# pkorus/neural-imaging

Measured on AMD Instinct MI355X. Metric: patches/s (fwd+bwd) ISP->JPEG->FAN @256^2, higher is better.
Workload: dtype bf16; 1 GPU; c4 = train_manipulation UNet->[native,sharpen:1,resample:50,gaussian:0.83,jpeg:80]->dJPEG(QF80,soft)->FAN, ds none, trainable nip+fan, lambda_nip 0.1; raw_patch=128, batch_per_gpu=64, global_batch=64, parallelism=dp1, world_size=1, hip_graph=False

## Files before the change

include/nimg.h:

```cpp
#ifndef NIMG_H
#define NIMG_H

#include <stddef.h>
#include <stdint.h>

#ifdef __cplusplus
extern "C" {
#endif

#define NIMG_OK 0
#define NIMG_ERR_ARG (-1)
#define NIMG_ERR_LAUNCH (-2)
#define NIMG_ERR_WORKSPACE (-3)

#define NIMG_BF16_IN 1
#define NIMG_BF16_OUT 2
#define NIMG_BF16_MASK 4
#define NIMG_BF16_DZ 8
#define NIMG_D2S_OUT 16
#define NIMG_MASK_CONV 128
#define NIMG_COPY_LRELU 64
#define NIMG_S2D_OUT 32
#define NIMG_UNPOOL_OUT 512
#define NIMG_D2S_CONVT 1024
#define NIMG_POOL_ALSO 256

#define NIMG_ABI_VERSION 7
int nimg_abi_version(void);

#define NIMG_ROUND_ROUND 0
#define NIMG_ROUND_SOFT 1
#define NIMG_ROUND_SIN 2
#define NIMG_ROUND_HARMONIC 3
#define NIMG_ROUND_IDENTITY 4

int nimg_djpeg_fwd(const float* x, float* y, const float* qtab, uint8_t* mask, int16_t* idx, float* xdq,
                   int n, int h, int w, int rounding, void* stream);
int nimg_djpeg_bwd(const float* x, const float* gy, const uint8_t* mask, const float* qtab, float* gx,
                   int n, int h, int w, int rounding, void* stream);
size_t nimg_djpeg_dq_workspace_bytes(int n, int h, int w);
int nimg_djpeg_bwd_dq(const float* x, const float* gy, const uint8_t* mask, const float* qtab, float* gx, float* dq,
                      int n, int h, int w, int rounding, int accumulate, void* workspace, size_t workspace_bytes,
                      void* stream);
int nimg_jpeg_qtable(int quality, int channel, float* out64);

int nimg_conv2d_fwd(const float* in1, int c1, const float* in2, int c2, const float* w, const float* bias,
                    float* out1, int o1, float* out2, int o2, const float* act_mask, int n, int h, int wd, int ks,
                    int stride, int pad_t, int pad_l, int pad_mode, int hout, int wout, int act, float alpha,
                    void* stream);
int nimg_conv_flip_weights(const float* w, float* wt, int ks_h, int ks_w, int cin, int cout, void* stream);
size_t nimg_conv2d_wgrad_workspace_bytes(int cin, int cout, int ks_h, int ks_w, int n, int hout, int wout);
int nimg_conv2d_wgrad(const float* in1, int c1, const float* in2, int c2, const float* dz, int cout, float* dw,
                      float* db, int n, int h, int wd, int ks, int stride, int pad_t, int pad_l, int pad_mode, int hout,
                      int wout, int accumulate, void* workspace, size_t workspace_bytes, void* stream);
size_t nimg_bias_grad_workspace_bytes(long npix, int cout);
int nimg_bias_grad(const float* dz, float* db, long npix, int cout, int accumulate, void* workspace,
                   size_t workspace_bytes, void* stream);
int nimg_bias_grad_ex(const float* dz, float* db, long npix, int cout, int accumulate, void* workspace,
                      size_t workspace_bytes, int flags, void* stream);
int nimg_convt2x2_fwd(const float* x, const float* w, const float* bias, float* y, int n, int h, int wd, int cin,
                      int cout, void* stream);

int nimg_maxpool2_fwd(const float* x, float* y, int n, int h, int w, int c, void* stream);
int nimg_maxpool2_bwd(const float* dp, const float* yact, const float* add, float* dz, int n, int h, int w, int c,
                      int apply_lrelu_mask, float alpha, void* stream);
int nimg_maxpool2_fwd_bf16(const void* x, void* y, int n, int h, int w, int c, void* stream);
int nimg_maxpool2_bwd_bf16(const void* dp, const void* yact, const void* add, void* dz, int n, int h, int w, int c,
                           int apply_lrelu_mask, float alpha, void* stream);
int nimg_conv2d_pool_fwd(const float* in, int cin, const float* w, const float* bias, float* pool_out,
                         unsigned char* pool_idx, int cout, int n, int h, int wd, int ks, int act, float alpha,
                         void* stream);
int nimg_conv2d_pool_fwd_bf16(const float* in, int cin, const float* w, const void* wb, const float* bias,
                              float* pool_out, unsigned char* pool_idx, int cout, int n, int h, int wd, int ks, int act,
                              float alpha, void* stream);
int nimg_maxpool2_unpool(const float* dp, const unsigned char* idx, const float* pooled, float* dz, int n, int ho, int wo,
                         int c, int apply_lrelu_mask, float alpha, void* stream);
int nimg_d2s_clip_fwd(const float* x, float* y, int n, int h, int w, int cout, float scale, float shift, int clip,
                      void* stream);
int nimg_d2s_clip_bwd(const float* dy, float* dx, int n, int h, int w, int cout, float scale, void* stream);
int nimg_lrelu_bwd(const float* dy, const float* yact, float* dz, long count, float alpha, void* stream);
int nimg_add(const float* a, const float* b, float* out, long count, void* stream);
int nimg_add_n(const float* const* inputs, int n_inputs, float* out, long count, void* stream);
int nimg_avgpool_fwd(const float* x, float* y, int n, int h, int w, int c, int factor, void* stream);
int nimg_avgpool_bwd(const float* dy, float* dx, int n, int h, int w, int c, int factor, void* stream);

size_t nimg_mse255_workspace_bytes(void);
int nimg_mse255(const float* a, const float* b, float* loss, float* grad_a, long count, float grad_scale,
                int accumulate, void* workspace, size_t workspace_bytes, void* stream);
size_t nimg_mae255_workspace_bytes(void);
int nimg_mae255(const float* a, const float* b, float* loss, float* grad_a, long count, float grad_scale,
                int accumulate, void* workspace, size_t workspace_bytes, void* stream);
size_t nimg_ssim_loss_workspace_bytes(int n, int h, int w, int c, int with_grad);
int nimg_ssim_loss(const float* y, const float* t, float* loss, float* grad_y, int n, int h, int w, int c,
                   float max_val, const float* gauss_win, float grad_scale, int accumulate, void* workspace,
                   size_t workspace_bytes, void* stream);
int nimg_mse255_sum_s2d3(const float* const* parts, int n_parts, const float* y, const float* target, float* loss, float* dz,
                         int n, int h, int w, float grad_scale, void* workspace, size_t workspace_bytes, void* stream);
size_t nimg_ssim_workspace_bytes(int n);
int nimg_ssim(const float* a, const float* b, float* out, int n, int h, int w, int c, int mode, float max_val,
              const float* gauss_win, void* workspace, size_t workspace_bytes, void* stream);
int nimg_fan_head_fwd(const float* act, const float* w, const float* b, const int* labels, float* gap, float* probs,
                      float* loss_per, float* dlogits, int n, int hw, int c, int k, float loss_scale, void* stream);
int nimg_fan_head_bwd(const float* act, const float* gap, const float* w, const float* dlogits,
                      const float* loss_per, float* dact, float* dw, float* db, float* loss, int n, int hw, int c,
                      int k, float loss_scale, float alpha, void* stream);
int nimg_adam_step(float* params, const float* grads, float* m, float* v, long count, float lr, float beta1,
                   float beta2, float eps, int step, float grad_scale, const int* skip_flag, void* stream);
int nimg_adam_step_dev(float* params, const float* grads, float* m, float* v, long count, const float* lr_t, float beta1,
                       float beta2, float eps, float grad_scale, const int* skip_flag, void* stream);
int nimg_nan_flag(const float* g, long count, int* flag, void* stream);
int nimg_int_words(int* dst, const int* src, long n, int value, int mode, void* stream);
int nimg_float_fill(float* dst, long n, float value, void* stream);

#define NIMG_TICKET_BYTES (64 * 1024)
#define NIMG_TICKET_STREAMS 16
int nimg_bind_tickets(void* stream, void* buf, size_t bytes);

int nimg_stream_create_cu_mask(int n_cus, void** stream);
int nimg_stream_destroy(void* stream);

int nimg_head_fused_ok(int hw, int c);
int nimg_head_fwd(const void* x, const void* wimg, const float* bias, unsigned* mask, unsigned* mask_p, float* gap, int n, int hw,
                  int c, float alpha, void* stream);
size_t nimg_head_wgrad_workspace_bytes(int n, int c);
int nimg_head_wgrad(const void* x, const unsigned* mask_p, const float* dlogits, const float* wdense, int k, float* dw, float* db,
                    int n, int hw, int c, float alpha, int accumulate, void* workspace, size_t workspace_bytes, void* stream);
int nimg_head_dgrad(const unsigned* mask, const float* dlogits, const float* wdense, int k, const void* wimg_t,
                    const void* in_mask, void* dx, int n, int hw, int c, float alpha, void* stream);
int nimg_head_dact(const unsigned* mask, const float* dlogits, const float* wdense, int k, void* dact, int n, int hw, int c,
                   float alpha, void* stream);
int nimg_fan_dense_fwd(const float* gap, const float* w, const float* b, const int* labels, float* probs, float* loss_per,
                       float* dlogits, int n, int c, int k, float loss_scale, void* stream);
int nimg_fan_dense_bwd(const float* gap, const float* dlogits, const float* loss_per, float* dw, float* db, float* loss, int n,
                       int c, int k, float loss_scale, void* stream);

int nimg_constrained_kernel_fwd(const float* kernel, float* nf, int ks, int channels, float strength, void* stream);
int nimg_constrained_kernel_bwd(const float* kernel, const float* dnf, float* dkernel, int ks, int channels,
                                float strength, void* stream);
int nimg_fold_pad(const float* dpad, float* dx, int n, int h, int w, int c, int pad, int pad_mode, void* stream);

int nimg_gaussian_fwd(const float* x, float* y, uint8_t* mask, const float* gk25, int n, int h, int w, int clip,
                      void* stream);
int nimg_gaussian_bwd(const float* dy, const uint8_t* mask, float* dx, const float* gk25, int n, int h, int w,
                      void* stream);
int nimg_dwfilter_fwd(const float* x, float* y, uint8_t* mask, const float* taps, int k, int pad_mode, int n, int h, int w,
                      int clip, void* stream);
int nimg_dwfilter_bwd(const float* dy, const uint8_t* mask, float* dx, const float* taps, int k, int pad_mode, int n, int h,
                      int w, void* stream);
int nimg_sharpen_fwd(const float* x, float* y, float* aux_hsv, uint8_t* mask, const float* gk9, int n, int h, int w,
                     void* stream);
int nimg_sharpen_bwd(const float* x, const float* dy, float* aux_hsv, const uint8_t* mask, float* dx,
                     const float* gk9, int n, int h, int w, void* stream);
int nimg_sparse_axis_apply(const float* in, float* out, const int* rowptr, const int* col, const float* val, int n,
                           int hin, int win, int c, int axis, int out_size, void* stream);

size_t nimg_ssim_planes_workspace_bytes(int n, int c);
int nimg_ssim_planes(const float* y, const float* t, int n, int h, int w, int c, float max_val, const float* gauss_win,
                     float* mean_ssim, float* mean_cs, float* maps, int which_maps, void* workspace,
                     size_t workspace_bytes, void* stream);
int nimg_msssim_combine(const float* values, const float* items, int scales, int planes, float* loss, float* coef,
                        void* stream);
int nimg_ssim_maps_grad(const float* y, const float* t, const float* maps, const float* coef, float* grad_y, int n,
                        int h, int w, int c, const float* gauss_win, float grad_scale, int accumulate, void* stream);

int nimg_patch_stats(const uint8_t* rgb, int n_images, int h, int w, const int* image_idx, const int* cand_xy, int b,
                     int attempts, int patch, double* var_out, double* mean_out, void* stream);
int nimg_patch_select(const int* cand_xy, const float* uniforms, const double* var, const double* mean, int b,
                      int attempts, int max_attempts, int mode, int* chosen_xy, int* attempts_used, void* stream);
int nimg_patch_gather(const uint16_t* raw, const uint8_t* rgb, int n_images, int h, int w, const int* image_idx,
                      const int* xy, int b, int patch, float* x_out, float* y_out, void* stream);

int nimg_affine(const float* x, float* y, long count, float a, float b, void* stream);
int nimg_lrelu_fwd(const float* x, float* y, long count, float alpha, void* stream);
int nimg_tanh_fwd(const float* x, float* y, long count, void* stream);
int nimg_tanh_bwd(const float* dy, const float* y, float* dx, long count, void* stream);
int nimg_clip01(const float* x, float* y, long count, void* stream);
int nimg_pad2d(const float* x, float* y, int n, int h, int w, int c, int pad, int pad_mode, void* stream);
int nimg_isp_residual_fwd(const float* x, const float* f, const float* alpha, float* y, long count, int clip,
                          void* stream);
long nimg_isp_residual_workspace_bytes(void);
int nimg_isp_residual_bwd(const float* dy, const float* f, const float* alpha, float* df, float* dalpha,
                          float* workspace, long count, int accumulate, void* stream);
int nimg_mask_scale(const float* x, const uint8_t* keep, float* y, long count, float scale, void* stream);
size_t nimg_conv5_dgrad_sparse_image_bytes(int cin, int cout);
int nimg_conv5_dgrad_sparse_weights(const float* w, void* image, int cin, int cout, void* stream);
int nimg_conv5_dgrad_sparse(const void* g, const unsigned char* idx, int cout, const void* image, void* out, int cin,
                            const void* act_mask, int n, int h, int wd, float alpha, int flags, void* stream);
int nimg_conv2d_fwd_bf16_res(const float* in1, int c1, const void* wb, const float* bias, float* out1, int o1,
                             const float* act_mask, const float* residual, void* out_bf16_copy, int n, int h, int wd, int ks,
                             int stride, int pad_t, int pad_l, int pad_mode, int hout, int wout, int act, float alpha, int flags,
                             void* stream);
int nimg_conv2d_fwd_bf16_unpool(const void* in_pooled, const unsigned char* in_idx, int c1, const void* wb, const float* bias,
                                float* out1, int o1, const float* act_mask, int n, int h, int w_, int ks, int pad_t, int pad_l,
// ... 12 lines not shown
size_t nimg_reduce_entry_bytes(void);
int nimg_reduce_batch_max(void);
int nimg_reduce_slabs_batch(const void* entries, int n, void* stream);

int nimg_conv5c3_bf16(const float* in, const float* w, float* out, int n, int h, int wd, void* stream);
int nimg_cconv3(const float* in, const float* w, float* out_f32, void* out_c4, int n, int h, int w_, int pad_mode,
                void* stream);
int nimg_cconv3_dgrad_border(const float* dc, const float* nf, float* dx, int n, int h, int w_, void* stream);
int nimg_conv1_pool_fwd_c4(const void* c4, const float* w, const float* bias, void* pooled, unsigned char* pool_idx, int n,
                           int h, int w_, float alpha, int out_bf16, void* stream);
size_t nimg_conv1_wgrad_c4_workspace_bytes(void);
int nimg_conv1_wgrad_c4(const void* c4, const void* g, const unsigned char* pool_idx, float* dw, float* db, int n, int h, int w_,
                        int g_bf16, int accumulate, void* workspace, size_t workspace_bytes, void* stream);
int nimg_conv1_dgrad_pooled(const void* g, const unsigned char* pool_idx, const float* w, float* dc, int n, int h, int w_,
                            int g_bf16, void* stream);
int nimg_confusion_accumulate(const float* probs, const int* labels, int* pred, unsigned long long* conf, int n, int k,
                              void* stream);
int nimg_sigmoid_fwd(const float* x, float* y, long count, void* stream);
int nimg_sigmoid_bwd(const float* dy, const float* y, float* dx, long count, void* stream);
int nimg_activation_fwd(const float* x, float* y, long count, int kind, float alpha, void* stream);
int nimg_activation_bwd(const float* dy, const float* y, float* dx, long count, int kind, float alpha, void* stream);
int nimg_gamma_ste_fwd(const float* x, float* y, long count, float lo, float hi, float exponent, void* stream);
int nimg_gamma_ste_bwd(const float* x, const float* dy, float* dx, long count, float lo, float hi, float exponent,
                       void* stream);
int nimg_s2d2_affine_bf16(const float* x, void* y, int n, int h, int w, int c, int cp, float a, float b, void* stream);
int nimg_s2d_conv_weights(const float* w5, float* w3, int cin, int cp, int cout, void* stream);
int nimg_s2d_conv_weights_bwd(const float* dw3, float* dw5, int cin, int cp, int cout, int accumulate, void* stream);
int nimg_d2s2_scale(const float* xs, float* x, int n, int h, int w, int c, int cp, float scale, void* stream);
int nimg_zero_insert2(const float* in, float* out, int n, int h, int w, int c, void* stream);
size_t nimg_latent_workspace_bytes(int codebook_size);
int nimg_latent_fwd(const float* z, const float* scale, const float* codebook, int codebook_size, float v,
                    float gamma, int soft_codebook, float* latent, float* entropy, long count, long count_global,
                    void* workspace, size_t workspace_bytes, int finalize, void* stream);
int nimg_latent_entropy_finalize(int codebook_size, long count_global, float* entropy, void* workspace, void* stream);
int nimg_latent_bwd(const float* z, const float* scale, const float* latent, const float* dlatent,
                    float entropy_coef, const float* codebook, int codebook_size, float v, float gamma,
                    int soft_codebook, float* dz, float* dscale, int accumulate_dscale, long count, void* workspace,
                    size_t workspace_bytes, void* stream);
size_t nimg_l2_loss_workspace_bytes(void);
int nimg_l2_loss(const float* target, const float* y, float* loss, float* grad_y, long count, float grad_scale,
                 int accumulate, void* workspace, size_t workspace_bytes, void* stream);

size_t nimg_conv_weights_bf16_bytes(int ks_h, int ks_w, int cin, int cout, int mode);
int nimg_conv_weights_bf16(const float* w, void* wb, int ks_h, int ks_w, int cin, int cout, int mode, void* stream);
int nimg_conv2d_wgrad_pooled_bf16(const float* in, int cin, const float* g, const unsigned char* idx, int cout,
                                  float* dw, float* db, int n, int h, int wd, int ks, int accumulate, void* workspace,
                                  size_t workspace_bytes, void* stream);
int nimg_conv2d_dgrad_fewin_pooled_bf16(const float* g, const unsigned char* idx, const float* w, float* out, int ci,
                                        int cz, int n, int h, int wd, int ks, void* stream);
int nimg_conv2d_fwd_bf16_ex(const float* in1, int c1, const float* in2, int c2, const void* wb, const float* bias,
                            float* out1, int o1, float* out2, int o2, const float* act_mask, int n, int h, int wd,
                            int ks, int stride, int pad_t, int pad_l, int pad_mode, int hout, int wout, int act,
                            float alpha, int flags, void* stream);
int nimg_conv2d_wgrad_bf16_ex(const float* in1, int c1, const float* in2, int c2, const float* dz, int cout, float* dw,
                              float* db, int n, int h, int wd, int ks, int stride, int pad_t, int pad_l, int pad_mode,
                              int hout, int wout, int accumulate, void* workspace, size_t workspace_bytes, int flags,
                              void* stream);
int nimg_conv2d_pool_fwd_bf16_ex(const float* in, int cin, const float* w, const void* wb, const float* bias,
                                 float* pool_out, unsigned char* pool_idx, int cout, int n, int h, int wd, int ks,
                                 int act, float alpha, int flags, void* stream);
int nimg_conv2d_fwd_pool_also_bf16(const float* in, int cin, const void* wb, const float* bias, float* out, float* pool_out,
                                   unsigned char* pool_idx, int cout, int n, int h, int wd, int act, float alpha, void* stream);
#define NIMG_ROWS_F32_OUT 1
int nimg_conv3_rows_bf16(const void* in1, int c1, const void* in2, int c2, const void* wb, const float* bias, const void* mask,
                         void* out, void* out2, void* pool_out, int n, int h, int wd, int cout, int act, float alpha, int flags,
                         void* stream);
int nimg_conv3_rows_d2s_bf16(const void* in, int c1, const void* wb, const float* bias, float* y, int n, int h, int wd, void* stream);
int nimg_conv3_rows_c4_bf16(const float* in, const float* w, const float* bias, void* out, int n, int h, int wd, int act, float alpha,
                            void* stream);

int nimg_conv2d_dgrad_unpool_out_bf16(const float* dz, int c1, const void* wb, const float* act, const float* skip, float* out,
                                      int cout, int n, int h, int wd, int apply_mask, float alpha, void* stream);
int nimg_conv2d_wgrad_pooled_bf16_ex(const float* in, int cin, const float* g, const unsigned char* idx, int cout,
                                     float* dw, float* db, int n, int h, int wd, int ks, int accumulate, void* workspace,
                                     size_t workspace_bytes, int flags, void* stream);
int nimg_conv2d_dgrad_fewin_pooled_bf16_ex(const float* g, const unsigned char* idx, const float* w, float* out, int ci,
                                           int cz, int n, int h, int wd, int ks, int flags, void* stream);
int nimg_maxpool2_unpool_ex(const float* dp, const unsigned char* idx, const float* pooled, float* dz, int n, int ho,
                            int wo, int c, int apply_lrelu_mask, float alpha, int flags, void* stream);
int nimg_convt2x2_fwd_bf16(const float* x, const void* wb, const float* bias, float* y, int n, int h, int wd, int cin,
                           int cout, void* stream);
int nimg_convt2x2_fwd_bf16_ex(const float* x, const void* wb, const float* bias, float* y, int n, int h, int wd, int cin,
                              int cout, int flags, void* stream);
int nimg_conv_weights_bf16_batch(const void* table, int n_entries, void* stream);
int nimg_conv2d_fwd_bf16(const float* in1, int c1, const float* in2, int c2, const void* wb, const float* bias,
                         float* out1, int o1, float* out2, int o2, const float* act_mask, int n, int h, int wd,
                         int ks, int stride, int pad_t, int pad_l, int pad_mode, int hout, int wout, int act,
                         float alpha, void* stream);
size_t nimg_conv2d_wgrad_bf16_workspace_bytes(int cin, int cout, int ks_h, int ks_w, int n, int hout, int wout);
int nimg_conv2d_wgrad_bf16(const float* in1, int c1, const float* in2, int c2, const float* dz, int cout, float* dw,
                           float* db, int n, int h, int wd, int ks, int stride, int pad_t, int pad_l, int pad_mode,
                           int hout, int wout, int accumulate, void* workspace, size_t workspace_bytes, void* stream);

int nimg_conv2d_fwd_smallc_bf16(const float* in, int cin, const float* w, const float* bias, float* out, int cout,
                                int n, int h, int wd, int ks, int pad_mode, int act, float alpha, void* stream);
int nimg_conv2d_fwd_smallc_bf16_ex(const float* in, int cin, const float* w, const float* bias, float* out, int cout,
                                   int n, int h, int wd, int ks, int pad_mode, int act, float alpha, int flags, void* stream);
int nimg_conv2d_dgrad_fewin_bf16(const float* dz, const float* w, float* out, int ci, int cz, int n, int h, int wd,
                                 int ks, void* stream);

int nimg_awgn_fwd(const float* x, const float* noise, float* y, uint8_t* mask, long count, float strength,
                  void* stream);
int nimg_awgn_bwd(const float* x, const float* noise, const float* dy, const uint8_t* mask, float* dx, long count,
                  float strength, void* stream);
int nimg_gamma_fwd(const float* x, float* y, long count, float gamma, void* stream);
int nimg_gamma_bwd(const float* x, const float* dy, float* dx, long count, float gamma, void* stream);
int nimg_median_fwd(const float* x, float* y, uint8_t* sel, int n, int h, int w, int kernel, void* stream);
int nimg_median_bwd(const float* dy, const uint8_t* sel, float* dx, int n, int h, int w, int kernel, void* stream);

#define NIMG_L3IC_E_READ 1
#define NIMG_L3IC_E_LANES 2
#define NIMG_L3IC_E_RANGE 4
#define NIMG_L3IC_E_SYMBOL 8
#define NIMG_L3IC_E_FREQ 16
#define NIMG_L3IC_E_VARINT 32
#define NIMG_L3IC_E_ODD 64
#define NIMG_L3IC_E_UNUSED 128
#define NIMG_L3IC_E_STATE 256
#define NIMG_L3IC_E_RLE 512
size_t nimg_l3ic_workspace_bytes(int n_streams, int n_sym);
int nimg_l3ic_quantise(const float* z, const float* codebook, int codebook_size, uint8_t* idx, int* err, int n, int h,
                       int w, int c, void* stream);
int nimg_l3ic_encode(const uint8_t* idx, int n_streams, int n_sym, uint8_t* out, uint32_t* lengths, uint32_t* hist,
                     uint32_t* freq, void* workspace, size_t workspace_bytes, void* stream);
int nimg_l3ic_decode(const uint8_t* data, const uint32_t* offsets, const uint32_t* lengths, const float* codebook,
                     int codebook_size, float* z, uint32_t* err, int n, int h, int w, int c, void* stream);

size_t nimg_jpeg_workspace_bytes(int n, int h, int w, int hs, int vs);
int nimg_jpeg_transform(const void* x, int is_u8, int n, int h, int w, int hs, int vs, int quality, int16_t* coef, void* workspace,
                        size_t workspace_bytes, void* stream);
int nimg_jpeg_encode(const int16_t* coef, int n, int h, int w, int hs, int vs, uint8_t* out, size_t out_capacity, uint32_t* lengths,
                     void* workspace, size_t workspace_bytes, void* stream);
int nimg_jpeg_reconstruct(const int16_t* coef, int n, int h, int w, int hs, int vs, int quality, float* y, void* workspace,
                          size_t workspace_bytes, void* stream);

#ifdef __cplusplus
}
#endif
#endif
```

neural-imaging_amd/_lib.py:

```python
import ctypes
import os
from ctypes import c_float, c_int, c_long, c_size_t, c_void_p

_HERE = os.path.dirname(os.path.abspath(__file__))
LIB_PATH = os.environ.get('NIMG_LIBPATH') or os.path.join(_HERE, 'libnimg.so')

P = c_void_p

PROTOTYPES = {
    'nimg_abi_version': (c_int, []),
    'nimg_djpeg_fwd': (c_int, [P, P, P, P, P, P, c_int, c_int, c_int, c_int, P]),
    'nimg_djpeg_bwd': (c_int, [P, P, P, P, P, c_int, c_int, c_int, c_int, P]),
    'nimg_djpeg_dq_workspace_bytes': (c_size_t, [c_int, c_int, c_int]),
    'nimg_djpeg_bwd_dq': (c_int, [P, P, P, P, P, P, c_int, c_int, c_int, c_int, c_int, P, c_size_t, P]),
    'nimg_jpeg_qtable': (c_int, [c_int, c_int, P]),
    'nimg_conv2d_fwd': (c_int, [P, c_int, P, c_int, P, P, P, c_int, P, c_int, P, c_int, c_int, c_int, c_int, c_int,
                                c_int, c_int, c_int, c_int, c_int, c_int, c_float, P]),
    'nimg_conv_flip_weights': (c_int, [P, P, c_int, c_int, c_int, c_int, P]),
    'nimg_conv2d_wgrad_workspace_bytes': (c_size_t, [c_int, c_int, c_int, c_int, c_int, c_int, c_int]),
    'nimg_conv2d_wgrad': (c_int, [P, c_int, P, c_int, P, c_int, P, P, c_int, c_int, c_int, c_int, c_int, c_int, c_int,
                                  c_int, c_int, c_int, c_int, P, c_size_t, P]),
    'nimg_bias_grad_workspace_bytes': (c_size_t, [c_long, c_int]),
    'nimg_bias_grad': (c_int, [P, P, c_long, c_int, c_int, P, c_size_t, P]),
    'nimg_bias_grad_ex': (c_int, [P, P, c_long, c_int, c_int, P, c_size_t, c_int, P]),
    'nimg_convt2x2_fwd': (c_int, [P, P, P, P, c_int, c_int, c_int, c_int, c_int, P]),
    'nimg_maxpool2_fwd': (c_int, [P, P, c_int, c_int, c_int, c_int, P]),
    'nimg_maxpool2_bwd': (c_int, [P, P, P, P, c_int, c_int, c_int, c_int, c_int, c_float, P]),
    'nimg_maxpool2_fwd_bf16': (c_int, [P, P, c_int, c_int, c_int, c_int, P]),
    'nimg_maxpool2_bwd_bf16': (c_int, [P, P, P, P, c_int, c_int, c_int, c_int, c_int, c_float, P]),
    'nimg_conv2d_pool_fwd': (c_int, [P, c_int, P, P, P, P, c_int, c_int, c_int, c_int, c_int, c_int, c_float, P]),
    'nimg_conv2d_pool_fwd_bf16': (c_int, [P, c_int, P, P, P, P, P, c_int, c_int, c_int, c_int, c_int, c_int, c_float,
                                          P]),
    'nimg_maxpool2_unpool': (c_int, [P, P, P, P, c_int, c_int, c_int, c_int, c_int, c_float, P]),
    'nimg_d2s_clip_fwd': (c_int, [P, P, c_int, c_int, c_int, c_int, c_float, c_float, c_int, P]),
    'nimg_d2s_clip_bwd': (c_int, [P, P, c_int, c_int, c_int, c_int, c_float, P]),
    'nimg_lrelu_bwd': (c_int, [P, P, P, c_long, c_float, P]),
    'nimg_add': (c_int, [P, P, P, c_long, P]),
    'nimg_add_n': (c_int, [P, c_int, P, c_long, P]),
    'nimg_avgpool_fwd': (c_int, [P, P, c_int, c_int, c_int, c_int, c_int, P]),
    'nimg_avgpool_bwd': (c_int, [P, P, c_int, c_int, c_int, c_int, c_int, P]),
    'nimg_mse255_workspace_bytes': (c_size_t, []),
    'nimg_mse255': (c_int, [P, P, P, P, c_long, c_float, c_int, P, c_size_t, P]),
    'nimg_mse255_sum_s2d3': (c_int, [P, c_int, P, P, P, P, c_int, c_int, c_int, c_float, P, c_size_t, P]),
    'nimg_fan_head_fwd': (c_int, [P, P, P, P, P, P, P, P, c_int, c_int, c_int, c_int, c_float, P]),
    'nimg_fan_head_bwd': (c_int, [P, P, P, P, P, P, P, P, P, c_int, c_int, c_int, c_int, c_float, c_float, P]),
    'nimg_adam_step': (c_int, [P, P, P, P, c_long, c_float, c_float, c_float, c_float, c_int, c_float, P, P]),
    'nimg_adam_step_dev': (c_int, [P, P, P, P, c_long, P, c_float, c_float, c_float, c_float, P, P]),
    'nimg_conv3_rows_bf16': (c_int, [P, c_int, P, c_int, P, P, P, P, P, P, c_int, c_int, c_int, c_int, c_int, c_float, c_int, P]),
    'nimg_conv3_rows_d2s_bf16': (c_int, [P, c_int, P, P, P, c_int, c_int, c_int, P]),
    'nimg_conv2d_wgrad_bf16_deferred': (c_int, [P, c_int, P, c_int, P, P, c_int, P, P, c_int, c_int, c_int, c_int, c_int, c_int, c_int,
                                                c_int, c_int, c_int, P, c_size_t, c_int, P, P]),
    'nimg_conv2d_wgrad_bf16_chained': (c_int, [P, c_int, P, c_int, P, P, c_int, P, P, c_int, c_int, c_int, c_int, c_int, c_int, c_int,
                                               c_int, c_int, c_int, P, c_size_t, c_int, P, P, P]),
    'nimg_reduce_entry_bytes': (c_size_t, []),
    'nimg_reduce_batch_max': (c_int, []),
    'nimg_reduce_slabs_batch': (c_int, [P, c_int, P]),
    'nimg_conv3_rows_c4_bf16': (c_int, [P, P, P, P, c_int, c_int, c_int, c_int, c_float, P]),
    'nimg_nan_flag': (c_int, [P, c_long, P, P]),
    'nimg_int_words': (c_int, [P, P, c_long, c_int, c_int, P]),
    'nimg_float_fill': (c_int, [P, c_long, c_float, P]),
    'nimg_bind_tickets': (c_int, [P, P, c_size_t]),
    'nimg_stream_create_cu_mask': (c_int, [c_int, P]),
    'nimg_stream_destroy': (c_int, [P]),
    'nimg_head_fused_ok': (c_int, [c_int, c_int]),
    'nimg_head_fwd': (c_int, [P, P, P, P, P, P, c_int, c_int, c_int, c_float, P]),
    'nimg_head_wgrad_workspace_bytes': (c_size_t, [c_int, c_int]),
    'nimg_head_wgrad': (c_int, [P, P, P, P, c_int, P, P, c_int, c_int, c_int, c_float, c_int, P, c_size_t, P]),
    'nimg_head_dgrad': (c_int, [P, P, P, c_int, P, P, P, c_int, c_int, c_int, c_float, P]),
    'nimg_head_dact': (c_int, [P, P, P, c_int, P, c_int, c_int, c_int, c_float, P]),
    'nimg_fan_dense_fwd': (c_int, [P, P, P, P, P, P, P, c_int, c_int, c_int, c_float, P]),
    'nimg_fan_dense_bwd': (c_int, [P, P, P, P, P, P, c_int, c_int, c_int, c_float, P]),
    'nimg_constrained_kernel_fwd': (c_int, [P, P, c_int, c_int, c_float, P]),
    'nimg_constrained_kernel_bwd': (c_int, [P, P, P, c_int, c_int, c_float, P]),
    'nimg_fold_pad': (c_int, [P, P, c_int, c_int, c_int, c_int, c_int, c_int, P]),
    'nimg_gaussian_fwd': (c_int, [P, P, P, P, c_int, c_int, c_int, c_int, P]),
    'nimg_gaussian_bwd': (c_int, [P, P, P, P, c_int, c_int, c_int, P]),
    'nimg_dwfilter_fwd': (c_int, [P, P, P, P, c_int, c_int, c_int, c_int, c_int, c_int, P]),
    'nimg_dwfilter_bwd': (c_int, [P, P, P, P, c_int, c_int, c_int, c_int, c_int, P]),
    'nimg_sharpen_fwd': (c_int, [P, P, P, P, P, c_int, c_int, c_int, P]),
    'nimg_sharpen_bwd': (c_int, [P, P, P, P, P, P, c_int, c_int, c_int, P]),
    'nimg_affine': (c_int, [P, P, c_long, c_float, c_float, P]),
    'nimg_lrelu_fwd': (c_int, [P, P, c_long, c_float, P]),
    'nimg_zero_insert2': (c_int, [P, P, c_int, c_int, c_int, c_int, P]),
    'nimg_s2d2_affine_bf16': (c_int, [P, P, c_int, c_int, c_int, c_int, c_int, c_float, c_float, P]),
    'nimg_s2d_conv_weights': (c_int, [P, P, c_int, c_int, c_int, P]),
    'nimg_s2d_conv_weights_bwd': (c_int, [P, P, c_int, c_int, c_int, c_int, P]),
    'nimg_d2s2_scale': (c_int, [P, P, c_int, c_int, c_int, c_int, c_int, c_float, P]),
    'nimg_latent_workspace_bytes': (c_size_t, [c_int]),
    'nimg_latent_fwd': (c_int, [P, P, P, c_int, c_float, c_float, c_int, P, P, c_long, c_long, P, c_size_t, c_int, P]),
    'nimg_latent_entropy_finalize': (c_int, [c_int, c_long, P, P, P]),
    'nimg_latent_bwd': (c_int, [P, P, P, P, c_float, P, c_int, c_float, c_float, c_int, P, P, c_int, c_long, P,
                                c_size_t, P]),
    'nimg_l2_loss_workspace_bytes': (c_size_t, []),
    'nimg_l2_loss': (c_int, [P, P, P, P, c_long, c_float, c_int, P, c_size_t, P]),
    'nimg_conv_weights_bf16_bytes': (c_size_t, [c_int, c_int, c_int, c_int, c_int]),
    'nimg_conv_weights_bf16': (c_int, [P, P, c_int, c_int, c_int, c_int, c_int, P]),
    'nimg_conv2d_fwd_bf16': (c_int, [P, c_int, P, c_int, P, P, P, c_int, P, c_int, P, c_int, c_int, c_int, c_int,
                                     c_int, c_int, c_int, c_int, c_int, c_int, c_int, c_float, P]),
    'nimg_conv2d_wgrad_bf16_workspace_bytes': (c_size_t, [c_int, c_int, c_int, c_int, c_int, c_int, c_int]),
    'nimg_conv2d_wgrad_bf16': (c_int, [P, c_int, P, c_int, P, c_int, P, P, c_int, c_int, c_int, c_int, c_int, c_int,
                                       c_int, c_int, c_int, c_int, c_int, P, c_size_t, P]),
    'nimg_conv2d_wgrad_pooled_bf16': (c_int, [P, c_int, P, P, c_int, P, P, c_int, c_int, c_int, c_int, c_int, P, c_size_t,
                                              P]),
    'nimg_conv2d_dgrad_fewin_pooled_bf16': (c_int, [P, P, P, P, c_int, c_int, c_int, c_int, c_int, c_int, P]),
    'nimg_ssim_workspace_bytes': (c_size_t, [c_int]),
    'nimg_ssim': (c_int, [P, P, P, c_int, c_int, c_int, c_int, c_int, c_float, P, P, c_size_t, P]),
    'nimg_tanh_fwd': (c_int, [P, P, c_long, P]),
    'nimg_tanh_bwd': (c_int, [P, P, P, c_long, P]),
    'nimg_clip01': (c_int, [P, P, c_long, P]),
    'nimg_isp_residual_fwd': (c_int, [P, P, P, P, c_long, c_int, P]),
    'nimg_isp_residual_workspace_bytes': (c_long, []),
    'nimg_isp_residual_bwd': (c_int, [P, P, P, P, P, P, c_long, c_int, P]),
    'nimg_activation_fwd': (c_int, [P, P, c_long, c_int, c_float, P]),
    'nimg_activation_bwd': (c_int, [P, P, P, c_long, c_int, c_float, P]),
    'nimg_sigmoid_fwd': (c_int, [P, P, c_long, P]),
    'nimg_sigmoid_bwd': (c_int, [P, P, P, c_long, P]),
    'nimg_gamma_ste_fwd': (c_int, [P, P, c_long, c_float, c_float, c_float, P]),
    'nimg_gamma_ste_bwd': (c_int, [P, P, P, c_long, c_float, c_float, c_float, P]),
    'nimg_mae255_workspace_bytes': (c_size_t, []),
    'nimg_mae255': (c_int, [P, P, P, P, c_long, c_float, c_int, P, c_size_t, P]),
    'nimg_ssim_loss_workspace_bytes': (c_size_t, [c_int, c_int, c_int, c_int, c_int]),
    'nimg_ssim_loss': (c_int, [P, P, P, P, c_int, c_int, c_int, c_int, c_float, P, c_float, c_int, P, c_size_t, P]),
    'nimg_patch_stats': (c_int, [P, c_int, c_int, c_int, P, P, c_int, c_int, c_int, P, P, P]),
    'nimg_patch_select': (c_int, [P, P, P, P, c_int, c_int, c_int, c_int, P, P, P]),
    'nimg_patch_gather': (c_int, [P, P, c_int, c_int, c_int, P, P, c_int, c_int, P, P, P]),
    'nimg_mask_scale': (c_int, [P, P, P, c_long, c_float, P]),
    'nimg_conv5_dgrad_sparse_image_bytes': (c_size_t, [c_int, c_int]),
    'nimg_conv5_dgrad_sparse_weights': (c_int, [P, P, c_int, c_int, P]),
    'nimg_conv5_dgrad_sparse': (c_int, [P, P, c_int, P, P, c_int, P, c_int, c_int, c_int, c_float, c_int, P]),
    'nimg_conv2d_fwd_bf16_res': (c_int, [P, c_int, P, P, P, c_int, P, P, P, c_int, c_int, c_int, c_int, c_int, c_int, c_int, c_int, c_int,
                                 c_int, c_int, c_float, c_int, P]),
    'nimg_conv2d_fwd_bf16_unpool': (c_int, [P, P, c_int, P, P, P, c_int, P, c_int, c_int, c_int, c_int, c_int, c_int, c_int,
                                            c_int, c_int, c_float, c_int, P]),
    'nimg_conv2d_wgrad_bf16_unpool': (c_int, [P, c_int, P, P, c_int, P, P, c_int, c_int, c_int, c_int, c_int, P, c_size_t, P]),
    'nimg_cconv3': (c_int, [P, P, P, P, c_int, c_int, c_int, c_int, P]),
    'nimg_conv5c3_bf16': (c_int, [P, P, P, c_int, c_int, c_int, P]),
    'nimg_cconv3_dgrad_border': (c_int, [P, P, P, c_int, c_int, c_int, P]),
    'nimg_conv1_pool_fwd_c4': (c_int, [P, P, P, P, P, c_int, c_int, c_int, c_float, c_int, P]),
    'nimg_conv1_wgrad_c4_workspace_bytes': (c_size_t, []),
    'nimg_conv1_wgrad_c4': (c_int, [P, P, P, P, P, c_int, c_int, c_int, c_int, c_int, P, c_size_t, P]),
    'nimg_conv1_dgrad_pooled': (c_int, [P, P, P, P, c_int, c_int, c_int, c_int, P]),
    'nimg_confusion_accumulate': (c_int, [P, P, P, P, c_int, c_int, P]),
    'nimg_ssim_planes_workspace_bytes': (c_size_t, [c_int, c_int]),
    'nimg_ssim_planes': (c_int, [P, P, c_int, c_int, c_int, c_int, c_float, P, P, P, P, c_int, P, c_size_t, P]),
    'nimg_msssim_combine': (c_int, [P, P, c_int, c_int, P, P, P]),
    'nimg_ssim_maps_grad': (c_int, [P, P, P, P, P, c_int, c_int, c_int, c_int, P, c_float, c_int, P]),
    'nimg_pad2d': (c_int, [P, P, c_int, c_int, c_int, c_int, c_int, c_int, P]),
    'nimg_conv2d_fwd_bf16_ex': (c_int, [P, c_int, P, c_int, P, P, P, c_int, P, c_int, P, c_int, c_int, c_int, c_int, c_int,
                                        c_int, c_int, c_int, c_int, c_int, c_int, c_float, c_int, P]),
    'nimg_conv2d_wgrad_bf16_ex': (c_int, [P, c_int, P, c_int, P, c_int, P, P, c_int, c_int, c_int, c_int, c_int, c_int,
                                          c_int, c_int, c_int, c_int, c_int, P, c_size_t, c_int, P]),
    'nimg_conv2d_pool_fwd_bf16_ex': (c_int, [P, c_int, P, P, P, P, P, c_int, c_int, c_int, c_int, c_int, c_int, c_float,
                                             c_int, P]),
    'nimg_conv2d_dgrad_unpool_out_bf16': (c_int, [P, c_int, P, P, P, P, c_int, c_int, c_int, c_int, c_int, c_float, P]),
    'nimg_conv2d_fwd_pool_also_bf16': (c_int, [P, c_int, P, P, P, P, P, c_int, c_int, c_int, c_int, c_int, c_float, P]),
    'nimg_conv2d_wgrad_pooled_bf16_ex': (c_int, [P, c_int, P, P, c_int, P, P, c_int, c_int, c_int, c_int, c_int, P,
                                                 c_size_t, c_int, P]),
    'nimg_conv2d_dgrad_fewin_pooled_bf16_ex': (c_int, [P, P, P, P, c_int, c_int, c_int, c_int, c_int, c_int, c_int, P]),
    'nimg_maxpool2_unpool_ex': (c_int, [P, P, P, P, c_int, c_int, c_int, c_int, c_int, c_float, c_int, P]),
    'nimg_conv_weights_bf16_batch': (c_int, [P, c_int, P]),
    'nimg_convt2x2_fwd_bf16': (c_int, [P, P, P, P, c_int, c_int, c_int, c_int, c_int, P]),
    'nimg_convt2x2_fwd_bf16_ex': (c_int, [P, P, P, P, c_int, c_int, c_int, c_int, c_int, c_int, P]),
    'nimg_conv2d_fwd_smallc_bf16': (c_int, [P, c_int, P, P, P, c_int, c_int, c_int, c_int, c_int, c_int, c_int,
                                            c_float, P]),
    'nimg_conv2d_fwd_smallc_bf16_ex': (c_int, [P, c_int, P, P, P, c_int, c_int, c_int, c_int, c_int, c_int, c_int,
                                               c_float, c_int, P]),
    'nimg_conv2d_dgrad_fewin_bf16': (c_int, [P, P, P, c_int, c_int, c_int, c_int, c_int, c_int, P]),
    'nimg_awgn_fwd': (c_int, [P, P, P, P, c_long, c_float, P]),
    'nimg_awgn_bwd': (c_int, [P, P, P, P, P, c_long, c_float, P]),
    'nimg_gamma_fwd': (c_int, [P, P, c_long, c_float, P]),
    'nimg_gamma_bwd': (c_int, [P, P, P, c_long, c_float, P]),
    'nimg_median_fwd': (c_int, [P, P, P, c_int, c_int, c_int, c_int, P]),
    'nimg_median_bwd': (c_int, [P, P, P, c_int, c_int, c_int, c_int, P]),
    'nimg_sparse_axis_apply': (c_int, [P, P, P, P, P, c_int, c_int, c_int, c_int, c_int, c_int, P]),
    'nimg_l3ic_workspace_bytes': (c_size_t, [c_int, c_int]),
    'nimg_l3ic_quantise': (c_int, [P, P, c_int, P, P, c_int, c_int, c_int, c_int, P]),
    'nimg_l3ic_encode': (c_int, [P, c_int, c_int, P, P, P, P, P, c_size_t, P]),
    'nimg_l3ic_decode': (c_int, [P, P, P, P, c_int, P, P, c_int, c_int, c_int, c_int, P]),
    'nimg_jpeg_workspace_bytes': (c_size_t, [c_int, c_int, c_int, c_int, c_int]),
    'nimg_jpeg_transform': (c_int, [P, c_int, c_int, c_int, c_int, c_int, c_int, c_int, P, P, c_size_t, P]),
    'nimg_jpeg_encode': (c_int, [P, c_int, c_int, c_int, c_int, c_int, P, c_size_t, P, P, c_size_t, P]),
    'nimg_jpeg_reconstruct': (c_int, [P, c_int, c_int, c_int, c_int, c_int, c_int, P, P, c_size_t, P]),
}

ERRORS = {-1: 'NIMG_ERR_ARG (invalid argument / unsupported configuration)',
          -2: 'NIMG_ERR_LAUNCH (HIP kernel launch failed)',
          -3: 'NIMG_ERR_WORKSPACE (workspace too small)'}

_lib = None


ABI_VERSION = 7
TICKET_BYTES = 64 * 1024


def load():
    global _lib
    if _lib is not None:
        return _lib
    if not os.path.isfile(LIB_PATH):
        raise RuntimeError('libnimg.so not found at {} - build it with neural-imaging_amd/csrc/build.sh '
                           '(or __graft_entry__.build()); there is no CPU fallback'.format(LIB_PATH))
    import torch
    lib = ctypes.CDLL(LIB_PATH)
    for name, (res, args) in PROTOTYPES.items():
        fn = getattr(lib, name)
        fn.restype = res
        fn.argtypes = args
    if lib.nimg_abi_version() != ABI_VERSION:
        raise RuntimeError('libnimg.so at {} has ABI version {}, this binding was written against {} - rebuild it '
                           '(neural-imaging_amd/csrc/build.sh)'.format(LIB_PATH, lib.nimg_abi_version(), ABI_VERSION))
    _lib = lib
    return lib


def call(name, *args):
    rc = getattr(load(), name)(*args)
    if rc != 0:
        raise RuntimeError('{} failed: {}'.format(name, ERRORS.get(rc, rc)))
    return rc
```

neural-imaging_amd/csrc/common.h:

```cpp
#pragma once
#include <hip/hip_runtime.h>
#include <stdint.h>
#include "../../include/nimg.h"

#define NIMG_CHECK_LAUNCH()                                   \
    do {                                                      \
        hipError_t e__ = hipGetLastError();                   \
        if (e__ != hipSuccess) return NIMG_ERR_LAUNCH;        \
    } while (0)

namespace nimg {

constexpr int WAVE = 64;

__device__ __forceinline__ float lrelu(float v, float alpha) { return v > 0.0f ? v : alpha * v; }

__device__ __forceinline__ float wave_sum(float v) {
#pragma unroll
    for (int o = 32; o > 0; o >>= 1) v += __shfl_xor(v, o, 64);
    return v;
}

__device__ __forceinline__ double wave_sum_d(double v) {
#pragma unroll
// ... 324 lines not shown
    e.blocks1 = 0;
    return e;
}

struct TicketJob {
    unsigned* cnt;
    float* slab[2];
    long stride[2];
    float* dst[2];
    int splits, group, accumulate;
};
struct TicketItem { int which; long off; };

__device__ __forceinline__ bool ticket_arrive(unsigned* cnt, unsigned expected, unsigned* flag_word) {
    asm volatile("s_waitcnt vmcnt(0)" ::: "memory");
    __syncthreads();
    if (threadIdx.x == 0) {
        __builtin_amdgcn_fence(__ATOMIC_RELEASE, "agent");
        asm volatile("s_waitcnt vmcnt(0)" ::: "memory");
        const unsigned t = __hip_atomic_fetch_add(cnt, 1u, __ATOMIC_RELAXED, __HIP_MEMORY_SCOPE_AGENT);
        const bool last = t + 1 == expected;
        if (last) {
            __hip_atomic_store(cnt, 0u, __ATOMIC_RELAXED, __HIP_MEMORY_SCOPE_AGENT);
            __builtin_amdgcn_fence(__ATOMIC_ACQUIRE, "agent");
        }
        *reinterpret_cast<volatile unsigned*>(flag_word) = last ? 1u : 0u;
    }
    __syncthreads();
    return *reinterpret_cast<volatile unsigned*>(flag_word) != 0u;
}

template <int NT, typename Map>
__device__ __forceinline__ void ticket_sum(const TicketJob& j, int k0, int kstep, int n, bool final, int items, Map map) {
    for (int it = threadIdx.x; it < items; it += NT) {
        const TicketItem m = map(it);
        const long stride = m.which ? j.stride[1] : j.stride[0];
        const long st = stride * kstep;
        float* src = (m.which ? j.slab[1] : j.slab[0]) + (long)k0 * stride + m.off;
        float4 a = *reinterpret_cast<const float4*>(src);
        int k = 1;
        for (; k + 8 <= n; k += 8) {
            float4 v[8];
#pragma unroll
            for (int u = 0; u < 8; ++u) v[u] = *reinterpret_cast<const float4*>(src + (long)(k + u) * st);
#pragma unroll
            for (int u = 0; u < 8; ++u) { a.x += v[u].x; a.y += v[u].y; a.z += v[u].z; a.w += v[u].w; }
        }
        for (; k < n; ++k) {
            const float4 v = *reinterpret_cast<const float4*>(src + (long)k * st);
            a.x += v.x; a.y += v.y; a.z += v.z; a.w += v.w;
        }
        if (final) {
            float4* d = reinterpret_cast<float4*>((m.which ? j.dst[1] : j.dst[0]) + m.off);
            if (j.accumulate) { const float4 o = *d; a.x += o.x; a.y += o.y; a.z += o.z; a.w += o.w; }
            *d = a;
        } else {
            *reinterpret_cast<float4*>(src) = a;
        }
    }
}

template <int NT, typename Map>
__device__ __forceinline__ void ticket_finish(const TicketJob& j, int split, int items, Map map, unsigned* flag_word) {
    const int G = j.group, NG = (j.splits + G - 1) / G, g = split / G;
    const int members = j.splits - g * G < G ? j.splits - g * G : G;
    if (!ticket_arrive(j.cnt + 1 + g, (unsigned)members, flag_word)) return;
    ticket_sum<NT>(j, g * G, 1, members, NG == 1, items, map);
    if (NG == 1) return;
    if (!ticket_arrive(j.cnt, (unsigned)NG, flag_word)) return;
    ticket_sum<NT>(j, 0, G, NG, true, items, map);
}

static inline int ticket_group(int splits) {
    if (splits <= 24) return splits < 1 ? 1 : splits;
    int g = 1;
    while (g * g < splits) ++g;
    return g;
}
__device__ __forceinline__ int ticket_words_per_tile_dev(int splits, int group) { return 1 + (splits + group - 1) / group; }
static inline int ticket_words_per_tile(int splits) { const int g = ticket_group(splits); return 1 + (splits + g - 1) / g; }

static inline int cdiv(long a, long b) { return (int)((a + b - 1) / b); }

}

extern "C" unsigned* nimg_internal_tickets(hipStream_t stream, size_t words);
int nimg_internal_wgrad5_alltaps(const void* in, int cin, const void* g, const unsigned char* idx, int cout, float* partial,
                                 float* db_partial, int n, int h, int wd, int max_slabs, hipStream_t stream);
int nimg_internal_wgrad3_alltaps(const void* in1, int c1, const void* in2, int c2, const void* dz, int cout, float* partial,
                                 float* db_partial, int n, int h, int wd, int max_slabs, hipStream_t stream, float* dw, float* db,
                                 int accumulate, const void* pre);
struct WgradArgsB;
int nimg_internal_wgrad_packed_splits(int cout, int n, int hout, int wout);
int nimg_internal_wgrad_packed(WgradArgsB* a, int ks, bool want_db, hipStream_t stream);
size_t nimg_internal_wgrad_tiny_bytes(int ks, int cin, int cout);
int nimg_internal_conv_wgrad_tiny(const float* in, const float* dz, float* dw, int cin, int cout, int n, int h, int wd,
                                  int ks, int pad, int pad_mode, int accumulate, void* workspace, hipStream_t s, bool bf16_ok);
int nimg_internal_conv_fewout(const float* in, int cin, const float* w, const float* bias, float* out, int cout, int n,
                              int h, int wd, int ks, int pad_t, int pad_l, int pad_mode, int hout, int wout,
                              hipStream_t s);
```

neural-imaging_amd/csrc/constrained.hip:

```cpp
#include "common.h"

namespace {

__device__ __forceinline__ bool centre_mask(int e, int ks, int c) {
    const int co = e % c, ci = (e / c) % c, kw = (e / (c * c)) % ks, kh = e / (c * c * ks);
    return kh == ks / 2 && kw == ks / 2 && ci == co;
}

__global__ __launch_bounds__(256) void constrained_fwd_kernel(const float* __restrict__ k, float* __restrict__ nf,
                                                              int ks, int c, float strength) {
    __shared__ float df[16];
    const int total = ks * ks * c * c, tid = threadIdx.x;
    if (tid < c) {
        float s = 0.f;
        for (int e = tid; e < total; e += c)
            if (!centre_mask(e, ks, c)) s += k[e];
        df[tid] = s;
    }
    __syncthreads();
    for (int e = tid; e < total; e += blockDim.x) {
        const bool m = centre_mask(e, ks, c);
        nf[e] = m ? -strength : strength * k[e] / df[e % c];
    }
}

__global__ __launch_bounds__(256) void constrained_bwd_kernel(const float* __restrict__ k,
                                                              const float* __restrict__ dnf, float* __restrict__ dk,
                                                              int ks, int c, float strength) {
    __shared__ float df[16], dot[16];
    const int total = ks * ks * c * c, tid = threadIdx.x;
    if (tid < c) {
        float s = 0.f, d = 0.f;
        for (int e = tid; e < total; e += c)
            if (!centre_mask(e, ks, c)) { s += k[e]; d += dnf[e] * k[e]; }
        df[tid] = s;
        dot[tid] = d;
    }
    __syncthreads();
    for (int e = tid; e < total; e += blockDim.x) {
        const int co = e % c;
        dk[e] = centre_mask(e, ks, c) ? 0.f : strength * (dnf[e] / df[co] - dot[co] / (df[co] * df[co]));
    }
}

}

extern "C" {

int nimg_constrained_kernel_fwd(const float* kernel, float* nf, int ks, int channels, float strength, void* stream) {
    if (!kernel || !nf || ks <= 0 || channels <= 0 || channels > 16) return NIMG_ERR_ARG;
    hipLaunchKernelGGL(constrained_fwd_kernel, dim3(1), dim3(256), 0, (hipStream_t)stream, kernel, nf, ks, channels,
                       strength);
    NIMG_CHECK_LAUNCH();
    return NIMG_OK;
}

int nimg_constrained_kernel_bwd(const float* kernel, const float* dnf, float* dkernel, int ks, int channels,
                                float strength, void* stream) {
    if (!kernel || !dnf || !dkernel || ks <= 0 || channels <= 0 || channels > 16) return NIMG_ERR_ARG;
    hipLaunchKernelGGL(constrained_bwd_kernel, dim3(1), dim3(256), 0, (hipStream_t)stream, kernel, dnf, dkernel, ks,
                       channels, strength);
    NIMG_CHECK_LAUNCH();
    return NIMG_OK;
}

}
```

neural-imaging_amd/csrc/conv_bf16.hip:

```cpp
#include "conv_bf16.h"

namespace {

__global__ void weights_bf16_kernel(const float* __restrict__ w, __bf16* __restrict__ wb, int taps, int cin, int cout,
                                    int mode) {
    const int rows = mode == 0 ? cout : cin, cols = mode == 0 ? cin : cout;
    const int cpad = (cols + 15) / 16 * 16;
    const long total = (long)taps * rows * cpad;
    for (long i = (long)blockIdx.x * blockDim.x + threadIdx.x; i < total; i += (long)gridDim.x * blockDim.x) {
        const int c = (int)(i % 16) + 16 * (int)(i / (16L * rows * taps)), r = (int)((i / 16) % rows);
        const int t = (int)((i / (16L * rows)) % taps);
        float v = 0.f;
        if (c < cols) v = mode == 0 ? w[((long)t * cin + c) * cout + r] : w[((long)(taps - 1 - t) * cin + r) * cout + c];
        wb[i] = (__bf16)v;
    }
}

__global__ __launch_bounds__(256) void weights_bf16_batch_kernel(const long long* __restrict__ table) {
    const long long* e = table + 4 * blockIdx.y;
    const float* w = reinterpret_cast<const float*>(e[0]);
    __bf16* wb = reinterpret_cast<__bf16*>(e[1]);
    const int taps = (int)(e[2] >> 32), mode = (int)(e[2] & 0xffffffffll);
    const int cin = (int)(e[3] >> 32), cout = (int)(e[3] & 0xffffffffll);
    const int rows = mode == 0 ? cout : cin, cols = mode == 0 ? cin : cout;
    const int chunks = (cols + 15) / 16, rblocks = (rows + 63) / 64;
    const int ntiles = chunks * taps * rblocks;
    __shared__ float tile[16][65];
    const int tid = threadIdx.x;
    for (int tl = blockIdx.x; tl < ntiles; tl += gridDim.x) {
        const int rb = tl % rblocks, ct = tl / rblocks, t = ct % taps, chunk = ct / taps;
        const int r0 = rb * 64, c0 = chunk * 16;
        __syncthreads();
        if (mode == 0) {
            const int cl = tid >> 4, rq = (tid & 15) * 4;
#pragma unroll
            for (int k = 0; k < 4; ++k) {
                const int c = c0 + cl, r = r0 + rq + k;
                tile[cl][rq + k] = (c < cols && r < rows) ? w[((long)t * cin + c) * cout + r] : 0.f;
            }
        } else {
            const int rl = tid >> 2, cq = (tid & 3) * 4;
#pragma unroll
            for (int k = 0; k < 4; ++k) {
                const int c = c0 + cq + k, r = r0 + rl;
                tile[cq + k][rl] = (c < cols && r < rows) ? w[((long)(taps - 1 - t) * cin + r) * cout + c] : 0.f;
            }
        }
        __syncthreads();
        const int rl = tid >> 2, kq = (tid & 3) * 4;
        if (r0 + rl < rows) {
            bf16x4 o;
#pragma unroll
            for (int k = 0; k < 4; ++k) o[k] = (__bf16)tile[kq + k][rl];
            *reinterpret_cast<bf16x4*>(wb + ((long)ct * rows + r0 + rl) * 16 + kq) = o;
        }
    }
}

template <int KS, int STRIDE>
int dispatch_b(const ConvParamsB& p, hipStream_t s) {
    if constexpr (STRIDE == 1) {
        if (p.flags & NIMG_BF16_IN) return conv_bf16_dispatch<KS, STRIDE, true>(p, s);
    } else if constexpr (KS == 2) {
        if (p.flags & NIMG_BF16_IN) return conv_bf16_dispatch<KS, STRIDE, true>(p, s);
    } else {
        if (p.flags & NIMG_BF16_IN) return NIMG_ERR_ARG;
    }
    return conv_bf16_dispatch<KS, STRIDE, false>(p, s);
}

}

extern "C" {

size_t nimg_conv_weights_bf16_bytes(int ks_h, int ks_w, int cin, int cout, int mode) {
    const long rows = mode == 0 ? cout : cin, cols = mode == 0 ? cin : cout;
    return (size_t)ks_h * ks_w * rows * ((cols + 15) / 16 * 16) * 2;
}

int nimg_conv_weights_bf16(const float* w, void* wb, int ks_h, int ks_w, int cin, int cout, int mode, void* stream) {
    if (!w || !wb || ks_h <= 0 || ks_w <= 0 || cin <= 0 || cout <= 0 || mode < 0 || mode > 1) return NIMG_ERR_ARG;
    const long total = (long)nimg_conv_weights_bf16_bytes(ks_h, ks_w, cin, cout, mode) / 2;
    const int grid = (int)((total + 255) / 256 > 2048 ? 2048 : (total + 255) / 256);
    hipLaunchKernelGGL(weights_bf16_kernel, dim3(grid), dim3(256), 0, (hipStream_t)stream, w, (__bf16*)wb,
                       ks_h * ks_w, cin, cout, mode);
    NIMG_CHECK_LAUNCH();
    return NIMG_OK;
}

int nimg_conv_weights_bf16_batch(const void* table, int n_entries, void* stream) {
    if (n_entries == 0) return NIMG_OK;
    if (!table || n_entries < 0) return NIMG_ERR_ARG;
    hipLaunchKernelGGL(weights_bf16_batch_kernel, dim3(384, (unsigned)n_entries), dim3(256), 0, (hipStream_t)stream,
                       (const long long*)table);
    NIMG_CHECK_LAUNCH();
    return NIMG_OK;
}

static int conv2d_fwd_bf16_impl(const float* in1, int c1, const float* in2, int c2, const void* wb, const float* bias,
                         float* out1, int o1, float* out2, int o2, const float* act_mask, int n, int h, int wd,
                         int ks, int stride, int pad_t, int pad_l, int pad_mode, int hout, int wout, int act,
                         float alpha, int flags, void* stream, const unsigned char* in_idx = nullptr,
                         const float* res = nullptr, void* out1b = nullptr, float* pool_out = nullptr,
                         unsigned char* pool_idx = nullptr) {
    if (n == 0) return NIMG_OK;
// ... 124 lines not shown
```

neural-imaging_amd/csrc/conv_bf16_wgrad.h:

```cpp
#pragma once
#include "conv_bf16.h"

struct WgradArgsB {
    const float* in1;
    const float* in2;
    const float* dz;
    const unsigned char* dz_idx;
    float* partial;
    float* db_partial;
    int C1, C2, Cout;
    int N, H, W, Hout, Wout, pad_t, pad_l;
    int tiles_y, tiles_x, splits, work_per_split, pad_mode;
    int flags;
    unsigned* tickets;
    float* dw;
    float* db;
    int group, accumulate;
    nimg::ReduceEntry pre;
};

namespace {

struct WgradParamsB : WgradArgsB {};

constexpr int B_TH = 8, B_TW = 16, B_CI = 32, B_CO = 64;

}
```

neural-imaging_amd/csrc/conv_bf16_wgrad.hip:

```cpp
#include "conv_bf16_wgrad.h"

namespace {

typedef short s16x4 __attribute__((ext_vector_type(4)));
typedef short s16x8 __attribute__((ext_vector_type(8)));

__device__ __forceinline__ bf16x8 tr_read8(const unsigned char* p0, const unsigned char* p1) {
    const s16x4 lo = __builtin_amdgcn_ds_read_tr16_b64_v4i16((s16x4 __attribute__((address_space(3)))*)p0);
    const s16x4 hi = __builtin_amdgcn_ds_read_tr16_b64_v4i16((s16x4 __attribute__((address_space(3)))*)p1);
    s16x8 r;
    r[0] = lo[0]; r[1] = lo[1]; r[2] = lo[2]; r[3] = lo[3]; r[4] = hi[0]; r[5] = hi[1]; r[6] = hi[2]; r[7] = hi[3];
    return *reinterpret_cast<bf16x8*>(&r);
}

constexpr int B_ZS = 192;

template <int KS, int STRIDE, int NW, bool INB, bool DZB, int TH, bool UNP = false, int NCO = 2, bool PAIR = false>
__global__ __launch_bounds__(NW * 64, 2) void conv_wgrad_bf16_kernel(const WgradParamsB p) {
    nimg::reduce_entry_inline(p.pre);
    constexpr int TCO = 32 * NCO, ZS = NCO == 2 ? B_ZS : 64, ZI = 4 * NCO;
    static_assert(NCO == 1 || NCO == 2, "one or two output fragments");
    static_assert(!UNP || NCO == 2, "un-pooling dz: 64-wide tile");
    static_assert(!UNP || (DZB && STRIDE == 1), "un-pooling dz: bf16-stored pooled gradient, stride 1");
    constexpr int TAPS = KS * KS, NT = (TAPS + NW - 1) / NW, NTHR = NW * 64;
    static_assert(!PAIR || (KS == 3 && STRIDE == 1 && TH == 8 && INB && DZB && !UNP), "image pairs: the 3x3 layers over 8 x 8 bf16 images");
    constexpr int THH = (TH - 1) * STRIDE + KS, TWH = PAIR ? 20 : (B_TW - 1) * STRIDE + KS;
    constexpr int NPIXH = THH * TWH, NPIX = TH * B_TW;
    static_assert(STRIDE == 1 || STRIDE == 2, "stride");
    extern __shared__ __attribute__((aligned(16))) unsigned char smem_raw[];
    unsigned char* sI = smem_raw;
    unsigned char* sZ = smem_raw + NPIXH * 64;
    const int tid = threadIdx.x, lane = tid & 63;
    const int wave = __builtin_amdgcn_readfirstlane(tid >> 6);
    const int Cin = p.C1 + p.C2;
    const int cib = (Cin + B_CI - 1) / B_CI, cob = (p.Cout + TCO - 1) / TCO;
    int bid = xcd_order(blockIdx.x);
    const int ci0 = (bid % cib) * B_CI;
    bid /= cib;
    const int co0 = (bid % cob) * TCO;
    const int split = bid / cob;
    const int half = lane >> 5, g = lane & 15, sub = (lane >> 4) & 1;

    f32x16 acc[NT][NCO];
#pragma unroll
    for (int t = 0; t < NT; ++t)
#pragma unroll
        for (int ni = 0; ni < NCO; ++ni)
#pragma unroll
            for (int j = 0; j < 16; ++j) acc[t][ni][j] = 0.0f;
    const int tiles = p.tiles_y * p.tiles_x;
    const int work_total = PAIR ? (p.N + 1) / 2 : p.N * tiles;
    const int w_begin = split * p.work_per_split;
    const int w_end = min(work_total, w_begin + p.work_per_split);
    const bool do_bias = p.db_partial && ci0 == 0;
    float bacc[8] = {0.f, 0.f, 0.f, 0.f, 0.f, 0.f, 0.f, 0.f};
    const int a_lane = ((half * (PAIR ? 10 : 8) + (g >> 2)) * STRIDE) * 64 + (sub * 16 + (g & 3) * 4) * 2;
    const int z_lane = (half * 8 + (g >> 2)) * ZS + (sub * 16 + (g & 3) * 4) * 2;
    constexpr int IP = (NPIXH * 4 + NTHR - 1) / NTHR, ZP = (NPIX * ZI) / NTHR;
    static_assert((NPIX * ZI) % NTHR == 0 && NTHR % ZI == 0, "dz tile must divide over the threads");
    float4 preI[IP][2], preZ[ZP][2];
    uint2 preZK[UNP ? ZP : 1];
    auto fetch = [&](int wk_) {
        const int n_ = (int)(wk_ / tiles), tile_ = (int)(wk_ % tiles);
        const int ty_ = (tile_ / p.tiles_x) * TH, tx_ = (tile_ % p.tiles_x) * B_TW;
        const int iy_ = ty_ * STRIDE - p.pad_t, ix_ = tx_ * STRIDE - p.pad_l;
#pragma unroll
        for (int q = 0; q < IP; ++q) {
            const int item = tid + q * NTHR;
            const int pix = item >> 2, c = ci0 + (item & 3) * 8;
            int gy = iy_ + pix / TWH, gx = ix_ + pix % TWH;
            int ni_ = n_;
            if constexpr (PAIR) {
                const int hx = pix % TWH;
                ni_ = 2 * wk_ + (hx >= 10 ? 1 : 0);
                gx = (hx >= 10 ? hx - 10 : hx) - 1;
                gy = pix / TWH - 1;
            }
            preI[q][0] = preI[q][1] = make_float4(0.f, 0.f, 0.f, 0.f);
            if (item < NPIXH * 4 && c < Cin && (!PAIR || ni_ < p.N) && map_coord(gy, p.H, p.pad_mode) && map_coord(gx, p.W, p.pad_mode)) {
                const long pixoff = ((long)ni_ * p.H + gy) * p.W + gx;
                if constexpr (INB) {
                    const __bf16* src = c < p.C1 ? reinterpret_cast<const __bf16*>(p.in1) + pixoff * p.C1 + c
                                                 : reinterpret_cast<const __bf16*>(p.in2) + pixoff * p.C2 + (c - p.C1);
                    preI[q][0] = *reinterpret_cast<const float4*>(src);
                } else {
                    const float* src = c < p.C1 ? p.in1 + pixoff * p.C1 + c : p.in2 + pixoff * p.C2 + (c - p.C1);
                    preI[q][0] = *reinterpret_cast<const float4*>(src);
                    if (c + 4 < Cin) preI[q][1] = *reinterpret_cast<const float4*>(src + 4);
                }
            }
        }
#pragma unroll
        for (int q = 0; q < ZP; ++q) {
            const int item = tid + q * NTHR;
            const int pix = item / ZI, c = co0 + (item % ZI) * 8;
            int oy = ty_ + pix / B_TW, ox = tx_ + pix % B_TW, nz_ = n_;
            if constexpr (PAIR) {
                nz_ = 2 * wk_ + ((pix % B_TW) >> 3);
                ox = pix & 7;
                oy = pix / B_TW;
            }
            preZ[q][0] = preZ[q][1] = make_float4(0.f, 0.f, 0.f, 0.f);
            if constexpr (UNP) preZK[q] = make_uint2(0xffffffffu, 0xffffffffu);
            if (oy < p.Hout && ox < p.Wout && c < p.Cout && (!PAIR || nz_ < p.N)) {
                const long zo = UNP ? (((long)n_ * (p.Hout >> 1) + (oy >> 1)) * (p.Wout >> 1) + (ox >> 1)) * p.Cout + c
                                    : (((long)nz_ * p.Hout + oy) * p.Wout + ox) * p.Cout + c;
                if constexpr (UNP) preZK[q] = *reinterpret_cast<const uint2*>(p.dz_idx + zo);
                if constexpr (DZB) {
                    preZ[q][0] = *reinterpret_cast<const float4*>(reinterpret_cast<const __bf16*>(p.dz) + zo);
                } else {
                    preZ[q][0] = *reinterpret_cast<const float4*>(p.dz + zo);
                    if (c + 4 < p.Cout) preZ[q][1] = *reinterpret_cast<const float4*>(p.dz + zo + 4);
                }
            }
        }
    };
    if (w_begin < w_end) fetch(w_begin);
    for (int wk = w_begin; wk < w_end; ++wk) {
        __syncthreads();
#pragma unroll
        for (int q = 0; q < IP; ++q) {
            const int item = tid + q * NTHR;
            if (item < NPIXH * 4) {
                uint4 packed;
                if constexpr (INB) {
                    packed = *reinterpret_cast<const uint4*>(&preI[q][0]);
                } else {
                    const float f[8] = {preI[q][0].x, preI[q][0].y, preI[q][0].z, preI[q][0].w,
                                        preI[q][1].x, preI[q][1].y, preI[q][1].z, preI[q][1].w};
                    const bf16x8 b = pack8(f);
                    packed = *reinterpret_cast<const uint4*>(&b);
                }
                *reinterpret_cast<uint4*>(sI + (item >> 2) * 64 + (item & 3) * 16) = packed;
            }
        }
#pragma unroll
        for (int q = 0; q < ZP; ++q) {
            const int item = tid + q * NTHR;
            float f[8];
            bf16x8 b;
            if constexpr (DZB) {
                if constexpr (UNP) {
                    const int pix_ = item / ZI;
                    const unsigned pos = (unsigned)((((pix_ / B_TW) & 1) << 1) | ((pix_ % B_TW) & 1));
                    const uint4 routed = unp_route(*reinterpret_cast<const uint4*>(&preZ[q][0]), preZK[q].x, preZK[q].y, pos);
                    b = *reinterpret_cast<const bf16x8*>(&routed);
                } else {
                    b = *reinterpret_cast<const bf16x8*>(&preZ[q][0]);
                }
#pragma unroll
                for (int e = 0; e < 8; ++e) f[e] = (float)b[e];
            } else {
                f[0] = preZ[q][0].x; f[1] = preZ[q][0].y; f[2] = preZ[q][0].z; f[3] = preZ[q][0].w;
                f[4] = preZ[q][1].x; f[5] = preZ[q][1].y; f[6] = preZ[q][1].z; f[7] = preZ[q][1].w;
                b = pack8(f);
            }
            if (do_bias) {
#pragma unroll
                for (int e = 0; e < 8; ++e) bacc[e] += f[e];
            }
            *reinterpret_cast<uint4*>(sZ + (item / ZI) * ZS + (item % ZI) * 16) = *reinterpret_cast<const uint4*>(&b);
        }
        __syncthreads();
        if (wk + 1 < w_end) fetch(wk + 1);
#pragma unroll 1
        for (int r = (KS == 1 ? wave : 0); r < TH; r += (KS == 1 ? NW : 1)) {
            const unsigned char* zr = sZ + (r * B_TW) * ZS + z_lane;
            bf16x8 bfr[NCO];
#pragma unroll
            for (int ni = 0; ni < NCO; ++ni) bfr[ni] = tr_read8(zr + 64 * ni, zr + 4 * ZS + 64 * ni);
#pragma unroll
            for (int t = 0; t < NT; ++t) {
                const int tap = KS == 1 ? 0 : wave + NW * t;
                if (tap < TAPS) {
                    const unsigned char* ir = sI + ((r * STRIDE + tap / KS) * TWH + (tap % KS)) * 64 + a_lane;
                    const bf16x8 a = tr_read8(ir, ir + 4 * STRIDE * 64);
#pragma unroll
                    for (int ni = 0; ni < NCO; ++ni)
                        acc[t][ni] = __builtin_amdgcn_mfma_f32_32x32x16_bf16(a, bfr[ni], acc[t][ni], 0, 0, 0);
                }
            }
        }
    }
    if (do_bias) {
        __syncthreads();
        float* red = reinterpret_cast<float*>(smem_raw);
#pragma unroll
        for (int e = 0; e < 8; ++e) red[tid * 8 + e] = bacc[e];
        __syncthreads();
        if (tid < TCO && co0 + tid < p.Cout) {
            float sum = 0.f;
            for (int o = 0; o < NTHR / ZI; ++o) sum += red[(o * ZI + (tid >> 3)) * 8 + (tid & 7)];
            p.db_partial[(long)split * p.Cout + co0 + tid] = sum;
        }
    }
    if constexpr (KS == 1) {
        static_assert(NCO == 2 && (NW - 1) * 2 * 16 * 64 * 4 <= NPIXH * 64 + NPIX * B_ZS, "fold scratch fits the tiles");
        __syncthreads();
        float* red = reinterpret_cast<float*>(smem_raw);
        if (wave > 0) {
#pragma unroll
            for (int ni = 0; ni < 2; ++ni)
#pragma unroll
                for (int j = 0; j < 16; ++j) red[(((wave - 1) * 2 + ni) * 16 + j) * 64 + lane] = acc[0][ni][j];
        }
        __syncthreads();
        if (wave == 0) {
#pragma unroll
            for (int w = 1; w < NW; ++w)
#pragma unroll
                for (int ni = 0; ni < 2; ++ni)
#pragma unroll
                    for (int j = 0; j < 16; ++j) acc[0][ni][j] += red[(((w - 1) * 2 + ni) * 16 + j) * 64 + lane];
        }
    }
    float* slab = p.partial + (long)split * TAPS * Cin * p.Cout;
#pragma unroll
    for (int t = 0; t < NT; ++t) {
        const int tap = KS == 1 ? 0 : wave + NW * t;
        if (tap >= TAPS || (KS == 1 && wave > 0)) continue;
#pragma unroll
        for (int ni = 0; ni < NCO; ++ni) {
            const int co = co0 + ni * 32 + (lane & 31);
            if (co >= p.Cout) continue;
#pragma unroll
            for (int j = 0; j < 16; ++j) {
                const int ci = ci0 + (j & 3) + 8 * (j >> 2) + 4 * half;
                if (ci < Cin) slab[((long)tap * Cin + ci) * p.Cout + co] = acc[t][ni][j];
            }
        }
    }
    if (p.tickets == nullptr) return;
    TicketJob job;
    job.cnt = p.tickets + (long)(xcd_order(blockIdx.x) % (cib * cob)) * ticket_words_per_tile_dev(p.splits, p.group);
    job.slab[0] = p.partial; job.stride[0] = (long)TAPS * Cin * p.Cout; job.dst[0] = p.dw;
    job.slab[1] = p.db_partial; job.stride[1] = p.Cout; job.dst[1] = p.db;
    job.splits = p.splits; job.group = p.group; job.accumulate = p.accumulate;
    const int rows = min(B_CI, Cin - ci0), c4n = min(TCO, p.Cout - co0) >> 2, Cout = p.Cout;
    const int witems = TAPS * rows * c4n;
    const int items = witems + ((p.db_partial && ci0 == 0) ? c4n : 0);
    ticket_finish<NTHR>(job, split, items, [=](int it) {
        TicketItem m;
        if (it >= witems) { m.which = 1; m.off = co0 + (it - witems) * 4; return m; }
        const int c4 = it % c4n, row = it / c4n;
        m.which = 0;
        m.off = ((long)(row / rows) * Cin + ci0 + row % rows) * Cout + co0 + c4 * 4;
        return m;
    }, reinterpret_cast<unsigned*>(smem_raw));
}

int splits_for(int cin, int cout, int n, int hout, int wout, int th = B_TH, int target_blocks = 512) {
    const long blocks_io = (long)cdiv(cin, B_CI) * cdiv(cout, B_CO);
    const long work = (long)n * cdiv(hout, th) * cdiv(wout, B_TW);
    long splits = (target_blocks + blocks_io - 1) / blocks_io;
    if (splits > work) splits = work;
    if (splits < 1) splits = 1;
    const long wps = (work + splits - 1) / splits;
    return (int)((work + wps - 1) / wps);
}

}

extern "C" {

size_t nimg_conv2d_wgrad_bf16_workspace_bytes(int cin, int cout, int ks_h, int ks_w, int n, int hout, int wout) {
    if (cin <= 0 || cout <= 0 || n <= 0) return 0;
    const size_t slab = (size_t)ks_h * ks_w * cin * cout * sizeof(float);
    const size_t generic = (slab + cout * sizeof(float)) * splits_for(cin, cout, n, hout, wout);
    const size_t packed = cin <= 4 ? (4 * slab + cout * sizeof(float)) * nimg_internal_wgrad_packed_splits(cout, n, hout, wout) : 0;
    const size_t tiny = (cin <= 4 && cout <= 4) ? nimg_internal_wgrad_tiny_bytes(ks_h, cin, cout) : 0;
    const size_t m = generic > packed ? generic : packed;
    return m > tiny ? m : tiny;
}

struct ReducePlan {
    nimg::ReduceEntry* defer = nullptr;
    const nimg::ReduceEntry* pre = nullptr;
};
static inline void finish_reduce2(const ReducePlan& plan, const float* p1, float* d1, long n1, int splits1, const float* p2,
                                  float* d2, long n2, int splits2, int accumulate, hipStream_t s) {
    if (plan.defer) nimg::fill_reduce_entry(plan.defer, p1, d1, n1, splits1, p2, d2, n2, splits2, accumulate);
    else launch_reduce2(p1, d1, n1, splits1, p2, d2, n2, splits2, accumulate, s);
}
struct OwedReduction {
    const nimg::ReduceEntry* e;
    hipStream_t s;
    void ran_in_kernel() { e = nullptr; }
    void now() {
        if (e && e->n1 > 0 && e->p1 && e->d1)
            launch_reduce2(e->p1, e->d1, e->n1, e->splits1, e->p2, e->d2, e->n2, e->splits2, e->accumulate, s);
        e = nullptr;
    }
    ~OwedReduction() { now(); }
};

static int wgrad_bf16_impl(const float* in1, int c1, const float* in2, int c2, const float* dz,
                           const unsigned char* dz_idx, int cout, float* dw, float* db, int n, int h, int wd, int ks,
                           int stride, int pad_t, int pad_l, int pad_mode, int hout, int wout, int accumulate,
                           void* workspace, size_t workspace_bytes, int flags, void* stream, const ReducePlan& plan) {
    OwedReduction owed{plan.pre, (hipStream_t)stream};
    if ((flags & NIMG_BF16_IN) && ((c1 & 7) || (c2 & 7))) return NIMG_ERR_ARG;
    if ((flags & NIMG_BF16_DZ) && (cout & 7)) return NIMG_ERR_ARG;
    if (flags && !dz_idx && c2 == 0 && c1 <= 4) return NIMG_ERR_ARG;
    if (dz_idx && c1 <= 4 && (flags & ~NIMG_BF16_DZ)) return NIMG_ERR_ARG;
    if (dz_idx && c1 > 4 && (flags != (NIMG_BF16_IN | NIMG_BF16_DZ) || stride != 1 || ks != 5 || (hout & 1) || (wout & 1)))
        return NIMG_ERR_ARG;
    if (!in1 || !dz || !dw || c1 <= 0 || c2 < 0 || cout <= 0 || n <= 0 || h <= 0 || wd <= 0) return NIMG_ERR_ARG;
    if ((c2 > 0 && !in2) || hout <= 0 || wout <= 0 || !workspace || pad_mode < 0 || pad_mode > 2) return NIMG_ERR_ARG;
    const int cin = c1 + c2;
    if (workspace_bytes < nimg_conv2d_wgrad_bf16_workspace_bytes(cin, cout, ks, ks, n, hout, wout)) return NIMG_ERR_WORKSPACE;
    WgradParamsB p;
    p.pre = nimg::empty_reduce_entry();
    p.in1 = in1; p.in2 = in2; p.dz = dz; p.dz_idx = dz_idx; p.partial = (float*)workspace; p.db_partial = nullptr;
    p.flags = flags;
    p.tickets = nullptr; p.dw = dw; p.db = db; p.group = 1; p.accumulate = accumulate;
    p.C1 = c1; p.C2 = c2; p.Cout = cout; p.N = n; p.H = h; p.W = wd; p.Hout = hout; p.Wout = wout;
    p.pad_t = pad_t; p.pad_l = pad_l; p.pad_mode = pad_mode;
    const long count = (long)ks * ks * cin * cout;
    hipStream_t s = (hipStream_t)stream;
    const bool tiny = c2 == 0 && c1 == 3 && cout == 3 && stride == 1 && (ks == 3 || ks == 5) && hout == h && wout == wd &&
                      pad_t == (ks - 1) / 2 && pad_l == pad_t && !db;
    const bool packed = c2 == 0 && (c1 == 3 || c1 == 4) && stride == 1 && (ks == 3 || ks == 5);
    const bool fan5 = dz_idx && ks == 5 && stride == 1 && c2 == 0 && pad_t == 2 && pad_l == 2 && hout == h && wout == wd && pad_mode == 0;
    if (tiny || packed || fan5) owed.now();
    if (tiny)
        return nimg_internal_conv_wgrad_tiny(in1, dz, dw, c1, cout, n, h, wd, ks, pad_t, pad_mode, accumulate, workspace, s,
                                             true);
    if (packed) {
        p.in2 = nullptr; p.dw = nullptr; p.db = nullptr;
        const int slabs = nimg_internal_wgrad_packed(&p, ks, db != nullptr, s);
        if (slabs < 0) return NIMG_ERR_LAUNCH;
        finish_reduce2(plan, (const float*)workspace, dw, count, slabs, p.db_partial, db, (long)cout, p.splits, accumulate, s);
        NIMG_CHECK_LAUNCH();
        return NIMG_OK;
    }
    if ((c1 % 4) || (c2 % 4) || (cout % 4) || (c2 > 0 && (c1 % 8))) return NIMG_ERR_ARG;
    auto want_tickets = [&](WgradParamsB& w) {
        if (plan.defer || (((uintptr_t)dw | (uintptr_t)db) & 15)) return;
        w.group = ticket_group(w.splits);
        w.tickets = nimg_internal_tickets((hipStream_t)stream, (size_t)cdiv(cin, B_CI) * cdiv(cout, B_CO) * ticket_words_per_tile(w.splits));
    };
    const int th = (stride == 1 && ks == 5) ? 16 : B_TH;
    p.tiles_y = cdiv(hout, th); p.tiles_x = cdiv(wout, B_TW);
    static const int wg5_env = getenv("NIMG_WGRAD5_BLOCKS") ? atoi(getenv("NIMG_WGRAD5_BLOCKS")) : 256;
    const int wg5 = wg5_env < 32 ? 32 : (wg5_env > 512 ? 512 : wg5_env);
    p.splits = splits_for(cin, cout, n, hout, wout, th, (stride == 1 && ks == 5) ? wg5 : 512);
    const long work = (long)n * p.tiles_y * p.tiles_x;
    p.work_per_split = (int)((work + p.splits - 1) / p.splits);
    if (fan5) {
        const int max_slabs = splits_for(cin, cout, n, hout, wout);
        float* dbp = db ? (float*)workspace + (size_t)max_slabs * count : nullptr;
        const int slabs = nimg_internal_wgrad5_alltaps(in1, cin, dz, dz_idx, cout, (float*)workspace, dbp, n, h, wd, max_slabs, s);
        if (slabs < 0) return NIMG_ERR_LAUNCH;
        if (slabs > 0) {
            finish_reduce2(plan, (const float*)workspace, dw, count, slabs, dbp, db, (long)cout, slabs, accumulate, s);
            NIMG_CHECK_LAUNCH();
            return NIMG_OK;
        }
    }
    if (!dz_idx && ks == 3 && stride == 1 && pad_t == 1 && pad_l == 1 && hout == h && wout == wd && pad_mode == 0 &&
        flags == (NIMG_BF16_IN | NIMG_BF16_DZ)) {
        const int max_slabs = splits_for(cin, cout, n, hout, wout);
        float* dbp = db ? (float*)workspace + (size_t)max_slabs * count : nullptr;
        const int slabs = nimg_internal_wgrad3_alltaps(in1, c1, in2, c2, dz, cout, (float*)workspace, dbp, n, h, wd, max_slabs, s,
                                                       plan.defer ? nullptr : dw, db, accumulate, owed.e);
        if (slabs != 0) owed.ran_in_kernel();
        if (slabs == -1) return NIMG_ERR_LAUNCH;
        if (slabs < -1) return NIMG_OK;
        if (slabs > 0) {
            finish_reduce2(plan, (const float*)workspace, dw, count, slabs, dbp, db, (long)cout, slabs, accumulate, s);
            NIMG_CHECK_LAUNCH();
            return NIMG_OK;
        }
    }
    static const bool no_pair = getenv("NIMG_NO_WGRAD_PAIR8") != nullptr;
    if (!no_pair && !dz_idx && ks == 3 && stride == 1 && h == 8 && wd == 8 && hout == 8 && wout == 8 && pad_t == 1 && pad_l == 1 &&
        pad_mode == 0 && flags == (NIMG_BF16_IN | NIMG_BF16_DZ) && n >= 2) {
        const long pairs = (n + 1) / 2;
        long sp = p.splits < pairs ? p.splits : pairs;
        const long wps = (pairs + sp - 1) / sp;
        sp = (pairs + wps - 1) / wps;
        p.splits = (int)sp; p.work_per_split = (int)wps; p.tiles_y = p.tiles_x = 1;
        if (db) p.db_partial = p.partial + (size_t)p.splits * count;
        const long pblocks = (long)cdiv(cin, B_CI) * cdiv(cout, B_CO) * p.splits;
        constexpr size_t lds = (size_t)10 * 20 * 64 + (size_t)B_TH * B_TW * B_ZS;
        auto k = conv_wgrad_bf16_kernel<3, 1, 4, true, true, B_TH, false, 2, true>;
        (void)hipFuncSetAttribute((const void*)k, hipFuncAttributeMaxDynamicSharedMemorySize, (int)lds);
        want_tickets(p);
        if (owed.e) p.pre = *owed.e;
        hipLaunchKernelGGL(k, dim3((unsigned)pblocks), dim3(256), lds, s, p);
        NIMG_CHECK_LAUNCH();
        owed.ran_in_kernel();
        if (p.tickets) return NIMG_OK;
        finish_reduce2(plan, (const float*)workspace, dw, count, p.splits, db ? (const float*)p.db_partial : nullptr, db, (long)cout,
                       p.splits, accumulate, s);
        NIMG_CHECK_LAUNCH();
        return NIMG_OK;
    }
    if (db) p.db_partial = p.partial + (size_t)p.splits * count;
    const long blocks = (long)cdiv(cin, B_CI) * cdiv(cout, B_CO) * p.splits;
    want_tickets(p);
    if (owed.e) p.pre = *owed.e;
#define NIMG_WGB1(KS_, ST_, NW_, INB_, DZB_, TH_)                                                               \
    do {                                                                                                      \
        constexpr int THH = (TH_ - 1) * ST_ + KS_, TWH = (B_TW - 1) * ST_ + KS_;                              \
        constexpr size_t lds_t = (size_t)THH * TWH * 64 + (size_t)TH_ * B_TW * B_ZS;                          \
        constexpr size_t lds = lds_t > (size_t)NW_ * 64 * 8 * 4 ? lds_t : (size_t)NW_ * 64 * 8 * 4;          \
        auto k = conv_wgrad_bf16_kernel<KS_, ST_, NW_, INB_, DZB_, TH_>;                                      \
        if constexpr (KS_ == 3 && ST_ == 1) {                              \
            static const bool no_narrow = getenv("NIMG_NO_NARROW_WGRAD") != nullptr;                          \
            if (!no_narrow && p.Cout <= 32 && !p.dz_idx) k = conv_wgrad_bf16_kernel<KS_, ST_, NW_, INB_, DZB_, TH_, false, 1>;  \
        }                                                                                                     \
        if (p.dz_idx) {                                                                                       \
            if constexpr (DZB_ && ST_ == 1 && KS_ == 5) k = conv_wgrad_bf16_kernel<KS_, ST_, NW_, INB_, true, TH_, true>;    \
            else return NIMG_ERR_ARG;                                                                         \
        }                                                                                                     \
        (void)hipFuncSetAttribute((const void*)k, hipFuncAttributeMaxDynamicSharedMemorySize, (int)lds);      \
        hipLaunchKernelGGL(k, dim3((unsigned)blocks), dim3(NW_ * 64), lds, s, p);                             \
    } while (0)
#define NIMG_WGB(KS_, ST_)                                                                                     \
    do {                                                                                                      \
        constexpr int NW = KS_ == 5 ? 8 : 4;                                                                  \
        constexpr int TH_ = (KS_ == 5 && ST_ == 1) ? 16 : B_TH;                                               \
         \
        constexpr bool BFOK = ST_ == 1 || KS_ == 2;                                                           \
        constexpr int S1 = BFOK ? ST_ : 1;                                                                    \
        constexpr int T1 = BFOK ? TH_ : B_TH;                                                                 \
        if (BFOK && (p.flags & NIMG_BF16_IN) && (p.flags & NIMG_BF16_DZ)) NIMG_WGB1(KS_, S1, NW, true, true, T1);    \
        else if (BFOK && (p.flags & NIMG_BF16_IN)) NIMG_WGB1(KS_, S1, NW, true, false, T1);                   \
        else if (BFOK && (p.flags & NIMG_BF16_DZ)) NIMG_WGB1(KS_, S1, NW, false, true, T1);                   \
        else if (p.flags) return NIMG_ERR_ARG;                                                                \
        else NIMG_WGB1(KS_, ST_, NW, false, false, TH_);                                                      \
    } while (0)
    if (stride == 1 && ks == 1) NIMG_WGB(1, 1);
    else if (stride == 1 && ks == 3) NIMG_WGB(3, 1);
    else if (stride == 1 && ks == 5) NIMG_WGB(5, 1);
    else if (stride == 2 && ks == 2) NIMG_WGB(2, 2);
    else if (stride == 2 && ks == 5) NIMG_WGB(5, 2);
    else return NIMG_ERR_ARG;
#undef NIMG_WGB
#undef NIMG_WGB1
    NIMG_CHECK_LAUNCH();
    owed.ran_in_kernel();
    if (p.tickets) return NIMG_OK;
    finish_reduce2(plan, (const float*)workspace, dw, count, p.splits, db ? (const float*)p.db_partial : nullptr, db, (long)cout,
                   p.splits, accumulate, s);
    NIMG_CHECK_LAUNCH();
    return NIMG_OK;
}

int nimg_conv2d_wgrad_bf16(const float* in1, int c1, const float* in2, int c2, const float* dz, int cout, float* dw,
                           float* db, int n, int h, int wd, int ks, int stride, int pad_t, int pad_l, int pad_mode,
                           int hout, int wout, int accumulate, void* workspace, size_t workspace_bytes, void* stream) {
    return wgrad_bf16_impl(in1, c1, in2, c2, dz, nullptr, cout, dw, db, n, h, wd, ks, stride, pad_t, pad_l, pad_mode, hout,
                           wout, accumulate, workspace, workspace_bytes, 0, stream, ReducePlan{});
}

int nimg_conv2d_wgrad_bf16_ex(const float* in1, int c1, const float* in2, int c2, const float* dz, int cout, float* dw,
                              float* db, int n, int h, int wd, int ks, int stride, int pad_t, int pad_l, int pad_mode,
                              int hout, int wout, int accumulate, void* workspace, size_t workspace_bytes, int flags,
                              void* stream) {
    return wgrad_bf16_impl(in1, c1, in2, c2, dz, nullptr, cout, dw, db, n, h, wd, ks, stride, pad_t, pad_l, pad_mode, hout,
                           wout, accumulate, workspace, workspace_bytes, flags, stream, ReducePlan{});
}

int nimg_conv2d_wgrad_bf16_unpool(const void* in, int cin, const void* g, const unsigned char* idx, int cout, float* dw, float* db,
                                  int n, int h, int wd, int ks, int accumulate, void* workspace, size_t workspace_bytes,
                                  void* stream) {
    if (!idx || ks != 5 || (h & 1) || (wd & 1)) return NIMG_ERR_ARG;
    return wgrad_bf16_impl((const float*)in, cin, nullptr, 0, (const float*)g, idx, cout, dw, db, n, h, wd, ks, 1, 2, 2, 0, h, wd,
                           accumulate, workspace, workspace_bytes, NIMG_BF16_IN | NIMG_BF16_DZ, stream, ReducePlan{});
}

int nimg_conv2d_wgrad_bf16_deferred(const void* in1, int c1, const void* in2, int c2, const void* dz, const unsigned char* idx,
                                    int cout, float* dw, float* db, int n, int h, int wd, int ks, int stride, int pad_t, int pad_l,
                                    int pad_mode, int hout, int wout, void* workspace, size_t workspace_bytes, int flags,
                                    void* entry, void* stream) {
    if (!entry) return NIMG_ERR_ARG;
    nimg::ReduceEntry* e = reinterpret_cast<nimg::ReduceEntry*>(entry);
    nimg::fill_reduce_entry(e, nullptr, nullptr, 0, 0, nullptr, nullptr, 0, 0, 0);
    e->blocks1 = 0;
    return wgrad_bf16_impl((const float*)in1, c1, (const float*)in2, c2, (const float*)dz, idx, cout, dw, db, n, h, wd, ks, stride,
                           pad_t, pad_l, pad_mode, hout, wout, 0, workspace, workspace_bytes, flags, stream, ReducePlan{e, nullptr});
}

int nimg_conv2d_wgrad_bf16_chained(const void* in1, int c1, const void* in2, int c2, const void* dz, const unsigned char* idx,
                                   int cout, float* dw, float* db, int n, int h, int wd, int ks, int stride, int pad_t, int pad_l,
                                   int pad_mode, int hout, int wout, void* workspace, size_t workspace_bytes, int flags,
                                   const void* pre_entry, void* entry, void* stream) {
    if (!entry) return NIMG_ERR_ARG;
    nimg::ReduceEntry pre_copy;
    if (pre_entry) pre_copy = *reinterpret_cast<const nimg::ReduceEntry*>(pre_entry);
    nimg::ReduceEntry* e = reinterpret_cast<nimg::ReduceEntry*>(entry);
    *e = nimg::empty_reduce_entry();
    return wgrad_bf16_impl((const float*)in1, c1, (const float*)in2, c2, (const float*)dz, idx, cout, dw, db, n, h, wd, ks, stride,
                           pad_t, pad_l, pad_mode, hout, wout, 0, workspace, workspace_bytes, flags, stream,
                           ReducePlan{e, pre_entry ? &pre_copy : nullptr});
}

size_t nimg_reduce_entry_bytes(void) { return sizeof(nimg::ReduceEntry); }
int nimg_reduce_batch_max(void) { return nimg::REDUCE_BATCH_MAX; }

int nimg_reduce_slabs_batch(const void* entries, int n, void* stream) {
    if (n == 0) return NIMG_OK;
    if (!entries || n < 0 || n > nimg::REDUCE_BATCH_MAX) return NIMG_ERR_ARG;
    const nimg::ReduceEntry* src = reinterpret_cast<const nimg::ReduceEntry*>(entries);
    nimg::ReduceBatch b;
    b.n = 0;
    int blocks = 0;
    for (int i = 0; i < n; ++i) {
        if (src[i].n1 <= 0 || !src[i].p1 || !src[i].d1) continue;
        b.e[b.n] = src[i];
        b.first_block[b.n] = blocks;
        blocks += src[i].blocks1 + ((src[i].p2 && src[i].d2) ? nimg::reduce_grid(src[i].n2) : 0);
        ++b.n;
    }
    b.first_block[b.n] = blocks;
    if (b.n == 0) return NIMG_OK;
    hipLaunchKernelGGL(nimg::reduce_slabs_batch_kernel, dim3((unsigned)blocks), dim3(256), 0, (hipStream_t)stream, b);
    NIMG_CHECK_LAUNCH();
    return NIMG_OK;
}

int nimg_conv2d_wgrad_pooled_bf16(const float* in, int cin, const float* g, const unsigned char* idx, int cout,
                                  float* dw, float* db, int n, int h, int wd, int ks, int accumulate, void* workspace,
                                  size_t workspace_bytes, void* stream) {
    return nimg_conv2d_wgrad_pooled_bf16_ex(in, cin, g, idx, cout, dw, db, n, h, wd, ks, accumulate, workspace,
                                            workspace_bytes, 0, stream);
}

int nimg_conv2d_wgrad_pooled_bf16_ex(const float* in, int cin, const float* g, const unsigned char* idx, int cout,
// ... 9 lines not shown
```

neural-imaging_amd/csrc/pointwise.hip:

```cpp
#include <stdlib.h>
#include <mutex>

#include "common.h"

namespace {

using namespace nimg;

inline int grid_for(long items) {
    long g = (items + 255) / 256;
    return (int)(g > 2048 ? 2048 : (g < 1 ? 1 : g));
}

template <int V>
__global__ void maxpool2_fwd_kernel(const float* __restrict__ x, float* __restrict__ y, int n, int h, int w, int c) {
    const int ho = h / 2, wo = w / 2, cv = c / V;
    const long total = (long)n * ho * wo * cv;
    for (long i = (long)blockIdx.x * blockDim.x + threadIdx.x; i < total; i += (long)gridDim.x * blockDim.x) {
        const int cc = (int)(i % cv) * V;
        long r = i / cv;
        const int ox = (int)(r % wo);
        r /= wo;
        const int oy = (int)(r % ho), im = (int)(r / ho);
        const float* p00 = x + (((long)im * h + 2 * oy) * w + 2 * ox) * c + cc;
// ... 802 lines not shown
#pragma unroll
    for (int k = 0; k < WIN; ++k) wsum += wt1[k];
    const double wnorm = mode == 0 ? 1.0 : 1.0 / wsum;
    double wt[WIN];
#pragma unroll
    for (int k = 0; k < WIN; ++k) wt[k] = wt1[k] * wnorm;
    double sum = 0.0;
    for (int t = blk; t < ntiles; t += blocks_per_image) {
        const int ch = t % c, tile = t / c, ty0 = (tile / tiles_x) * T, tx0 = (tile % tiles_x) * T;
        __syncthreads();
        for (int i = tid; i < HT * HT; i += 256) {
            const int gy = ty0 + i / HT, gx = tx0 + i % HT;
            const bool ok = gy < h && gx < w;
            const long o = (((long)n * h + (ok ? gy : 0)) * w + (ok ? gx : 0)) * c + ch;
            sa[i] = ok ? a[o] : 0.f;
            sb[i] = ok ? b[o] : 0.f;
        }
        __syncthreads();
        for (int i = tid; i < HT * T; i += 256) {
            const int r = i / T, cc = i % T;
            double ux = 0, uy = 0, uxx = 0, uyy = 0, uxy = 0;
#pragma unroll
            for (int dx = 0; dx < WIN; ++dx) {
                const double va = sa[r * HT + cc + dx], vb = sb[r * HT + cc + dx], wv = wt[dx];
                const double wa = wv * va, wb = wv * vb;
                ux += wa; uy += wb; uxx += wa * va; uyy += wb * vb; uxy += wa * vb;
            }
            hm[0][i] = ux; hm[1][i] = uy; hm[2][i] = uxx; hm[3][i] = uyy; hm[4][i] = uxy;
        }
        __syncthreads();
        const int oy = tid / T, ox = tid % T;
        if (ty0 + oy < ho && tx0 + ox < wo) {
            double ux = 0, uy = 0, uxx = 0, uyy = 0, uxy = 0;
#pragma unroll
            for (int dy = 0; dy < WIN; ++dy) {
                const int i = (oy + dy) * T + ox;
                const double wv = wt[dy];
                ux += wv * hm[0][i]; uy += wv * hm[1][i]; uxx += wv * hm[2][i]; uyy += wv * hm[3][i]; uxy += wv * hm[4][i];
            }
            const double vx = covn * (uxx - ux * ux), vy = covn * (uyy - uy * uy), vxy = covn * (uxy - ux * uy);
            sum += ((2 * ux * uy + c1) * (2 * vxy + c2)) / ((ux * ux + uy * uy + c1) * (vx + vy + c2));
        }
    }
    red[tid] = sum;
    __syncthreads();
    for (int st = 128; st > 0; st >>= 1) {
        if (tid < st) red[tid] += red[tid + st];
        __syncthreads();
    }
    if (tid == 0) partial[blockIdx.x] = red[0];
}

__global__ void ssim_final_kernel(const double* __restrict__ partial, float* __restrict__ out, int blocks_per_image,
                                  double inv_items) {
    const int n = blockIdx.x;
    double s = 0.0;
    for (int k = threadIdx.x; k < blocks_per_image; k += 64) s += partial[(long)n * blocks_per_image + k];
    s = wave_sum_d(s);
    if (threadIdx.x == 0) out[n] = (float)(s * inv_items);
}

__global__ void adam_kernel(float* __restrict__ p, const float* __restrict__ g, float* __restrict__ m,
                            float* __restrict__ v, long count, float lr_t, float b1, float b2, float eps,
                            float gscale, const int* __restrict__ skip_flag, const float* __restrict__ lr_t_dev) {
    if (skip_flag && skip_flag[0]) return;
    if (lr_t_dev) lr_t = lr_t_dev[0];
    for (long i = (long)blockIdx.x * blockDim.x + threadIdx.x; i < count; i += (long)gridDim.x * blockDim.x) {
        const float gi = gscale * g[i];
        const float mi = b1 * m[i] + (1.0f - b1) * gi;
        const float vi = b2 * v[i] + (1.0f - b2) * gi * gi;
        m[i] = mi;
        v[i] = vi;
        p[i] -= lr_t * mi / (sqrtf(vi) + eps);
    }
}

__global__ void nan_flag_kernel(const float* __restrict__ g, long count, int* flag) {
    bool bad = false;
    for (long i = (long)blockIdx.x * blockDim.x + threadIdx.x; i < count; i += (long)gridDim.x * blockDim.x)
        bad |= (g[i] != g[i]);
    if (__any(bad) && (threadIdx.x & 63) == 0) atomicOr(flag, 1);
}

}

extern "C" {

int nimg_maxpool2_fwd(const float* x, float* y, int n, int h, int w, int c, void* stream) {
    if (n == 0) return NIMG_OK;
    if (!x || !y || n < 0 || h < 2 || w < 2 || c <= 0) return NIMG_ERR_ARG;
    if (n == 0) return NIMG_OK;
    hipStream_t s = (hipStream_t)stream;
    if (c % 4 == 0)
        hipLaunchKernelGGL(maxpool2_fwd_kernel<4>, dim3(grid_for((long)n * (h / 2) * (w / 2) * (c / 4))), dim3(256),
                           0, s, x, y, n, h, w, c);
    else
        hipLaunchKernelGGL(maxpool2_fwd_kernel<1>, dim3(grid_for((long)n * (h / 2) * (w / 2) * c)), dim3(256), 0, s,
                           x, y, n, h, w, c);
    NIMG_CHECK_LAUNCH();
    return NIMG_OK;
}

int nimg_maxpool2_bwd(const float* dp, const float* yact, const float* add, float* dz, int n, int h, int w, int c,
                      int apply_lrelu_mask, float alpha, void* stream) {
    if (n == 0) return NIMG_OK;
    if (!dp || !yact || !dz || n < 0 || h < 2 || w < 2 || c <= 0) return NIMG_ERR_ARG;
    if (n == 0) return NIMG_OK;
    hipStream_t s = (hipStream_t)stream;
    if ((h & 1) || (w & 1)) {
        if (add && add != dz) return NIMG_ERR_ARG;
        if (!add && hipMemsetAsync(dz, 0, (size_t)n * h * w * c * sizeof(float), s) != hipSuccess) return NIMG_ERR_LAUNCH;
        if (add && apply_lrelu_mask) {
            const long border = (long)n * (((h & 1) ? (long)w * c : 0) + ((w & 1) ? (long)(h & ~1) * c : 0));
            hipLaunchKernelGGL(maxpool2_bwd_border_kernel, dim3(grid_for(border)), dim3(256), 0, s, yact, dz, n, h, w, c, alpha);
            NIMG_CHECK_LAUNCH();
        }
    }
    if (c % 4 == 0)
        hipLaunchKernelGGL(maxpool2_bwd_kernel<4>, dim3(grid_for((long)n * (h / 2) * (w / 2) * (c / 4))), dim3(256),
                           0, s, dp, yact, add, dz, n, h, w, c, apply_lrelu_mask, alpha);
    else
        hipLaunchKernelGGL(maxpool2_bwd_kernel<1>, dim3(grid_for((long)n * (h / 2) * (w / 2) * c)), dim3(256), 0, s,
                           dp, yact, add, dz, n, h, w, c, apply_lrelu_mask, alpha);
    NIMG_CHECK_LAUNCH();
    return NIMG_OK;
}

int nimg_maxpool2_fwd_bf16(const void* x, void* y, int n, int h, int w, int c, void* stream) {
    if (n == 0) return NIMG_OK;
    if (!x || !y || n < 0 || h < 2 || w < 2 || c <= 0 || (h & 1) || (w & 1) || (c & 7)) return NIMG_ERR_ARG;
    hipLaunchKernelGGL(maxpool2_fwd_bf16_kernel, dim3(grid_for((long)n * (h / 2) * (w / 2) * (c / 8))), dim3(256), 0,
                       (hipStream_t)stream, (const __bf16*)x, (__bf16*)y, n, h, w, c);
    NIMG_CHECK_LAUNCH();
    return NIMG_OK;
}

int nimg_maxpool2_bwd_bf16(const void* dp, const void* yact, const void* add, void* dz, int n, int h, int w, int c,
                           int apply_lrelu_mask, float alpha, void* stream) {
    if (n == 0) return NIMG_OK;
    if (!dp || !yact || !dz || n < 0 || h < 2 || w < 2 || c <= 0 || (h & 1) || (w & 1) || (c & 7)) return NIMG_ERR_ARG;
    hipLaunchKernelGGL(maxpool2_bwd_bf16_kernel, dim3(grid_for((long)n * (h / 2) * (w / 2) * (c / 8))), dim3(256), 0,
                       (hipStream_t)stream, (const __bf16*)dp, (const __bf16*)yact, (const __bf16*)add, (__bf16*)dz, n, h, w, c,
                       apply_lrelu_mask, alpha);
    NIMG_CHECK_LAUNCH();
    return NIMG_OK;
}

int nimg_maxpool2_unpool(const float* dp, const unsigned char* idx, const float* pooled, float* dz, int n, int ho, int wo,
                         int c, int apply_lrelu_mask, float alpha, void* stream) {
    if (n == 0) return NIMG_OK;
    if (!dp || !idx || !dz || n < 0 || ho <= 0 || wo <= 0 || c <= 0 || (c & 3)) return NIMG_ERR_ARG;
    if (apply_lrelu_mask && !pooled) return NIMG_ERR_ARG;
    if (n == 0) return NIMG_OK;
    return nimg_maxpool2_unpool_ex(dp, idx, pooled, dz, n, ho, wo, c, apply_lrelu_mask, alpha, 0, stream);
}

int nimg_maxpool2_unpool_ex(const float* dp, const unsigned char* idx, const float* pooled, float* dz, int n, int ho,
                            int wo, int c, int apply_lrelu_mask, float alpha, int flags, void* stream) {
    if (n == 0) return NIMG_OK;
    if (!dp || !idx || !dz || n < 0 || ho <= 0 || wo <= 0 || c <= 0 || (c & 3)) return NIMG_ERR_ARG;
    if (apply_lrelu_mask && !pooled) return NIMG_ERR_ARG;
    const dim3 grid(grid_for((long)n * ho * wo * (c / 4)));
    hipStream_t s = (hipStream_t)stream;
    if ((flags & NIMG_BF16_IN) && (flags & NIMG_BF16_OUT) && !apply_lrelu_mask && (c & 7) == 0) {
        hipLaunchKernelGGL(maxpool2_unpool_bf16x8_kernel, dim3(grid_for((long)n * ho * wo * (c / 8))), dim3(256), 0, s,
                           (const uint4*)dp, (const uint2*)idx, (uint4*)dz, n, ho, wo, c / 8);
// ... 185 lines not shown
    NIMG_CHECK_LAUNCH();
    if (k > 16)
        hipLaunchKernelGGL(dense_softmax_ce_wide_kernel, dim3(n), dim3(64), 0, s, gap, w, b, labels, probs, loss_per, dlogits, n,
                           c, k, loss_scale);
    else
    hipLaunchKernelGGL(dense_softmax_ce_kernel, dim3(n), dim3(64), 0, s, gap, w, b, labels, probs, loss_per, dlogits, n, c,
                       k, loss_scale);
    NIMG_CHECK_LAUNCH();
    return NIMG_OK;
}

int nimg_fan_head_bwd(const float* act, const float* gap, const float* w, const float* dlogits,
                      const float* loss_per, float* dact, float* dw, float* db, float* loss, int n, int hw, int c,
                      int k, float loss_scale, float alpha, void* stream) {
    if (!act || !gap || !w || !dlogits || !loss_per || !dact || !dw || !db || !loss) return NIMG_ERR_ARG;
    if (n <= 0 || hw <= 0 || c <= 0 || k <= 0 || k > 256) return NIMG_ERR_ARG;
    hipStream_t s = (hipStream_t)stream;
    if (k > 16)
        hipLaunchKernelGGL(dense_bwd_params_wide_kernel, dim3(c + 2), dim3(64), 0, s, gap, dlogits, loss_per, dw, db, loss, n, c,
                           k, loss_scale);
    else
    hipLaunchKernelGGL(dense_bwd_params_kernel, dim3(c + 2), dim3(64), 0, s, gap, dlogits, loss_per, dw, db, loss, n, c, k,
                       loss_scale);
    NIMG_CHECK_LAUNCH();
    const int parts = n >= 1024 ? 1 : (n >= 256 ? 4 : 16);
    hipLaunchKernelGGL(gap_bwd_kernel, dim3((unsigned)(n * parts)), dim3(256), 0, s, dlogits, w, act, dact, hw, c, k, alpha,
                       parts);
    NIMG_CHECK_LAUNCH();
    return NIMG_OK;
}

int nimg_fan_dense_fwd(const float* gap, const float* w, const float* b, const int* labels, float* probs, float* loss_per,
                       float* dlogits, int n, int c, int k, float loss_scale, void* stream) {
    if (n == 0) return NIMG_OK;
    if (!gap || !w || !b || !probs || n < 0 || c <= 0 || k <= 0 || k > 256) return NIMG_ERR_ARG;
    if (labels && (!loss_per || !dlogits)) return NIMG_ERR_ARG;
    hipStream_t s = (hipStream_t)stream;
    if (k > 16)
        hipLaunchKernelGGL(dense_softmax_ce_wide_kernel, dim3(n), dim3(64), 0, s, gap, w, b, labels, probs, loss_per, dlogits, n,
                           c, k, loss_scale);
    else
        hipLaunchKernelGGL(dense_softmax_ce_kernel, dim3(n), dim3(64), 0, s, gap, w, b, labels, probs, loss_per, dlogits, n, c,
                           k, loss_scale);
    NIMG_CHECK_LAUNCH();
    return NIMG_OK;
}

int nimg_fan_dense_bwd(const float* gap, const float* dlogits, const float* loss_per, float* dw, float* db, float* loss, int n,
                       int c, int k, float loss_scale, void* stream) {
    if (!gap || !dlogits || !loss_per || !dw || !db || !loss || n <= 0 || c <= 0 || k <= 0 || k > 256) return NIMG_ERR_ARG;
    hipStream_t s = (hipStream_t)stream;
    if (k > 16)
        hipLaunchKernelGGL(dense_bwd_params_wide_kernel, dim3(c + 2), dim3(64), 0, s, gap, dlogits, loss_per, dw, db, loss, n, c,
                           k, loss_scale);
    else
        hipLaunchKernelGGL(dense_bwd_params_kernel, dim3(c + 2), dim3(64), 0, s, gap, dlogits, loss_per, dw, db, loss, n, c, k,
                           loss_scale);
    NIMG_CHECK_LAUNCH();
    return NIMG_OK;
}

int nimg_adam_step(float* params, const float* grads, float* m, float* v, long count, float lr, float beta1,
                   float beta2, float eps, int step, float grad_scale, const int* skip_flag, void* stream) {
    if (!params || !grads || !m || !v || count < 0 || step < 1) return NIMG_ERR_ARG;
    if (count == 0) return NIMG_OK;
    const double lr_t = (double)lr * __builtin_sqrt(1.0 - __builtin_pow((double)beta2, (double)step)) /
                        (1.0 - __builtin_pow((double)beta1, (double)step));
    hipLaunchKernelGGL(adam_kernel, dim3(grid_for(count)), dim3(256), 0, (hipStream_t)stream, params, grads, m, v,
                       count, (float)lr_t, beta1, beta2, eps, grad_scale, skip_flag, (const float*)nullptr);
    NIMG_CHECK_LAUNCH();
    return NIMG_OK;
}

int nimg_adam_step_dev(float* params, const float* grads, float* m, float* v, long count, const float* lr_t, float beta1,
                       float beta2, float eps, float grad_scale, const int* skip_flag, void* stream) {
    if (!params || !grads || !m || !v || !lr_t || count < 0) return NIMG_ERR_ARG;
    if (count == 0) return NIMG_OK;
    hipLaunchKernelGGL(adam_kernel, dim3(grid_for(count)), dim3(256), 0, (hipStream_t)stream, params, grads, m, v,
                       count, 0.f, beta1, beta2, eps, grad_scale, skip_flag, lr_t);
    NIMG_CHECK_LAUNCH();
    return NIMG_OK;
}

int nimg_int_words(int* dst, const int* src, long n, int value, int mode, void* stream) {
    if (n == 0) return NIMG_OK;
    if (!dst || n < 0 || mode < 0 || mode > 1 || (mode == 1 && !src)) return NIMG_ERR_ARG;
    hipLaunchKernelGGL(int_words_kernel, dim3(grid_for(n)), dim3(256), 0, (hipStream_t)stream, dst, src, n, value, mode);
    NIMG_CHECK_LAUNCH();
    return NIMG_OK;
}

namespace {
struct TicketBinding { hipStream_t stream; unsigned* buf; size_t words; bool used; };
TicketBinding g_tickets[NIMG_TICKET_STREAMS];
std::mutex g_tickets_mutex;
}

int nimg_bind_tickets(void* stream, void* buf, size_t bytes) {
    if ((buf && (bytes < 4 || (bytes & 3))) || ((uintptr_t)buf & 3)) return NIMG_ERR_ARG;
    std::lock_guard<std::mutex> lock(g_tickets_mutex);
    int free_slot = -1;
    for (int i = 0; i < NIMG_TICKET_STREAMS; ++i) {
        if (g_tickets[i].used && g_tickets[i].stream == (hipStream_t)stream) {
            if (buf) { g_tickets[i].buf = (unsigned*)buf; g_tickets[i].words = bytes / 4; }
            else g_tickets[i].used = false;
            return NIMG_OK;
        }
        if (!g_tickets[i].used && free_slot < 0) free_slot = i;
    }
    if (!buf) return NIMG_OK;
    if (free_slot < 0) return NIMG_ERR_ARG;
    g_tickets[free_slot] = TicketBinding{(hipStream_t)stream, (unsigned*)buf, bytes / 4, true};
    return NIMG_OK;
}

int nimg_stream_create_cu_mask(int n_cus, void** stream) {
    if (!stream || n_cus < 1 || n_cus > 1024) return NIMG_ERR_ARG;
    uint32_t mask[32] = {0};
    for (int i = 0; i < n_cus; ++i) mask[i >> 5] |= 1u << (i & 31);
    hipStream_t s = nullptr;
    if (hipExtStreamCreateWithCUMask(&s, (uint32_t)((n_cus + 31) / 32), mask) != hipSuccess) return NIMG_ERR_LAUNCH;
    *stream = (void*)s;
    return NIMG_OK;
}

int nimg_stream_destroy(void* stream) {
    if (!stream) return NIMG_ERR_ARG;
    return hipStreamDestroy((hipStream_t)stream) == hipSuccess ? NIMG_OK : NIMG_ERR_LAUNCH;
}

unsigned* nimg_internal_tickets(hipStream_t stream, size_t words) {
    static const bool off = getenv("NIMG_NO_TICKETS") != nullptr;
    if (off) return nullptr;
    std::lock_guard<std::mutex> lock(g_tickets_mutex);
    for (int i = 0; i < NIMG_TICKET_STREAMS; ++i)
        if (g_tickets[i].used && g_tickets[i].stream == stream) return g_tickets[i].words >= words ? g_tickets[i].buf : nullptr;
    return nullptr;
}

int nimg_float_fill(float* dst, long n, float value, void* stream) {
    if (n == 0) return NIMG_OK;
    if (!dst || n < 0) return NIMG_ERR_ARG;
    hipLaunchKernelGGL(float_fill_kernel, dim3(grid_for(n)), dim3(256), 0, (hipStream_t)stream, dst, n, value);
    NIMG_CHECK_LAUNCH();
    return NIMG_OK;
}

int nimg_nan_flag(const float* g, long count, int* flag, void* stream) {
    if (!g || !flag || count < 0) return NIMG_ERR_ARG;
    if (count == 0) return NIMG_OK;
    hipLaunchKernelGGL(nan_flag_kernel, dim3(grid_for(count)), dim3(256), 0, (hipStream_t)stream, g, count, flag);
    NIMG_CHECK_LAUNCH();
    return NIMG_OK;
}

}
```

neural-imaging_amd/models/forensics.py:

```python
import os
from collections import OrderedDict

import numpy as np

import torch

from .. import ops, parallel
from ..device import DeviceArray, to_device
from ..helpers import paramspec
from .layers import ConstrainedConv2D, Conv2D
from .tfmodel import ParamStore, TFModel, glorot_uniform_


LATE_PARAMS = os.environ.get('NIMG_NO_LATE_PARAMS') is None
LATE_MIN_IMAGES = int(os.environ.get('NIMG_LATE_MIN_IMAGES', '160'))
DEFER_MASK = int(os.environ.get('NIMG_PIPELINE_FAN_MASK', '255'))
LATE_MASK = int(os.environ.get('NIMG_LATE_MASK', '255'))


class FAN(TFModel):

    def __init__(self, n_classes, patch_size=None, n_filters=32, n_fscale=2, n_convolutions=4, kernel=5, dropout=0.0,
                 use_gap=True, n_dense=0, activation='leaky_relu', device=None, seed=4321):
        super().__init__(device=device)
        self._h = paramspec.ParamSpec({
            'n_classes': (7, int, (2, 256)),
            'n_filters': (32, int, (4, 128)),
            'n_fscale': (2, float, (0.25, 4)),
            'n_convolutions': (4, int, (1, 32)),
            'kernel': (5, int, (3, 11)),
            'dropout': (0, float, (0, 1)),
            'use_gap': (False, bool, None),
            'n_dense': (2, int, (0, 16)),
            'activation': ('leaky_relu', str, set(ops.ACTIVATIONS)),
        })
        params = locals()
        self._h.update(**{k: params[k] for k in self._h.keys()})
        if not 0 <= float(dropout) < 1:
            raise ValueError('dropout rate must be in [0, 1)')
        self._dropout_gen, self._dropout_seed = None, int(seed) + 17
        self.dropout_masks = None
        if not use_gap and patch_size is None:
            raise ValueError('the Flatten head (use_gap=False) needs a fixed patch_size')
        self.patch_size = patch_size
        self.x = _Shape((None, patch_size, patch_size, 3))
        self.y = _Shape((None, n_classes))

        self._constrained = ConstrainedConv2D('constrained')
        self._convs = []
        cin, nf = 3, n_filters
        for i in range(self._h.n_convolutions):
            self._convs.append(Conv2D('conv{}'.format(i + 1), self._h.kernel, cin, nf, self._h.activation,
                                      mask_activation=self._h.activation))
            cin, nf = nf, int(nf * self._h.n_fscale)
        nf = int(nf // self._h.n_fscale)
        self._conv1x1 = Conv2D('conv1x1', 1, cin, nf, self._h.activation, mask_activation=self._h.activation)
        self._generic_act = self._h.activation != 'leaky_relu'
        self._use_gap = bool(use_gap)
        feat = nf if use_gap else nf * (patch_size // 2 ** self._h.n_convolutions) ** 2
        self._hidden = []
        for i in range(self._h.n_dense):
            nf = int(nf // self._h.n_fscale)
            self._hidden.append(Conv2D('dense' if i == 0 else 'dense_{}'.format(i), 1, feat, nf, self._h.activation))
            feat = nf
        self._cls = 'dense' if self._h.n_dense == 0 else 'dense_{}'.format(self._h.n_dense)
        self._n_features = feat
        specs = self._constrained.specs()
        for c in self._convs:
            specs += c.specs()
        specs += self._conv1x1.specs()
        for d in self._hidden:
            specs += [(d.name + '/kernel', (d.cin, d.cout)), (d.name + '/bias', (d.cout,))]
        specs += [(self._cls + '/kernel', (feat, n_classes)), (self._cls + '/bias', (n_classes,))]
        self._model = ParamStore(specs, self.device)
        gen = torch.Generator().manual_seed(seed)
        self._constrained.init(self._model)
        for c in self._convs:
            c.init(self._model, gen)
        self._conv1x1.init(self._model, gen)
        for d in self._hidden + [None]:
            name, fi, fo = (d.name, d.cin, d.cout) if d is not None else (self._cls, feat, n_classes)
            k = torch.empty((fi, fo), dtype=torch.float32)
            glorot_uniform_(k, fi, fo, gen)
            self._model.p[name + '/kernel'].copy_(k)
            self._model.p[name + '/bias'].zero_()
        self.learning_rate = 1e-3
        self.loss = self._loss

    def reset_performance_stats(self):
        self.performance = {'loss': {'training': [], 'validation': []}, 'accuracy': {'validation': []},
                            'confusion': []}

    def forward(self, x, labels=None, training=False, loss_scale=None):
        self._model.refresh_images()
        P = self._model
        t = OrderedDict()
        t['x'] = x
        c1 = self._convs[0]
        front = ops.front_end_ok(c1.cin, c1.cout, c1.ks, x.shape[1], x.shape[2], n=x.shape[0] if training else None) and \
            c1.activation == 'leaky_relu'
        net, nf = self._constrained.forward(P, x, c4_only=front)
        t['constrained'], t['nf'] = net, nf
        for i, c in enumerate(self._convs):
            if i == 0 and front:
                nxt = self._convs[1] if len(self._convs) > 1 else self._conv1x1
                as_bf16 = ops.STORE_BF16 and nxt.cout >= 8
                net, idx = ops.conv1_pool_c4(net, P.p[c.name + '/kernel'], P.p[c.name + '/bias'], want_idx=training,
                                             out_bf16=as_bf16)
                t['idx1'], t['front'] = idx, True
            elif c.can_pool(net):
                nxt = self._convs[i + 1] if i + 1 < len(self._convs) else self._conv1x1
                as_bf16 = ops.COMPUTE == 'bf16' and ops.STORE_BF16 and c.cout % 8 == 0 and nxt.cout >= 8
                net, idx = c.forward_pool(P, net, want_idx=training, out_bf16=as_bf16)
                t['idx{}'.format(i + 1)] = idx
            else:
                a = c.forward(P, net)
                t['conv{}'.format(i + 1)] = a
                net = ops.maxpool2(a)
            t['pool{}'.format(i + 1)] = net
        n = x.shape[0]
        ls = (1.0 / n) if loss_scale is None else loss_scale
        c5 = self._conv1x1
        if self._use_gap and not self._hidden and not self._generic_act and c5.cin == c5.cout and ops.head_fused_ok(net, c5.cout):
            gap, mask, mask_p = ops.head_fwd(net, P.p[c5.name + '/kernel'], P.p[c5.name + '/bias'], want_mask=training)
            t['head_mask_p'] = mask_p
            probs, loss_per, dlogits = ops.fan_dense_fwd(gap, P.p[self._cls + '/kernel'], P.p[self._cls + '/bias'], labels, ls)
            t['head_mask'], t['gap'], t['probs'], t['loss_per'], t['dlogits'], t['loss_scale'] = mask, gap, probs, loss_per, dlogits, ls
            return probs, (t if training else None)
        a = self._conv1x1.forward(P, net)
        t['conv1x1'] = a
        head_in = a
        if self._hidden or not self._use_gap:
            if self._use_gap:
                if a.shape[1] != a.shape[2]:
                    raise ValueError('the hidden-Dense head pools square feature maps')
                head_in = ops.avgpool(a, a.shape[1])
            else:
                head_in = a.reshape(n, 1, 1, -1)
            t['feat'] = head_in
            rate = float(self._h.dropout)
            for li, d in enumerate(self._hidden):
                w4 = P.p[d.name + '/kernel'].view(1, 1, d.cin, d.cout)
                if self._generic_act:
                    head_in = ops.conv2d(head_in, w4, P.p[d.name + '/bias'])
                    ops.activation(head_in, self._h.activation, out=head_in)
                else:
                    head_in = ops.conv2d(head_in, w4, P.p[d.name + '/bias'], act='leaky_relu')
                t[d.name] = head_in
                if training and rate > 0:
                    if self.dropout_masks is not None:
                        keep = self.dropout_masks[li].to(device=x.device, dtype=torch.uint8).reshape(head_in.shape).contiguous()
                    else:
                        if self._dropout_gen is None:
                            self._dropout_gen = parallel.rank_generator(self._dropout_seed, x.device)
                        keep = (torch.rand(head_in.shape, device=x.device, generator=self._dropout_gen) >= rate).to(torch.uint8)
                    head_in = ops.mask_scale(head_in, keep, 1.0 / (1.0 - rate))
                    t[d.name + '/keep'], t[d.name + '/dropped'] = keep, head_in
            if training:
                self.dropout_masks = None
# ... 166 lines not shown
```

neural-imaging_amd/models/layers.py:

```python
import numpy as np
import torch

from .. import ops
from ..helpers import kernels as hk


FUSED_ACTIVATIONS = (None, 'leaky_relu')


def act_forward(y, activation):
    if isinstance(y, tuple):
        raise RuntimeError('a bf16 copy cannot be combined with activation {}'.format(activation))
    return ops.activation(y, activation, out=y)


class Conv2D(object):

    def __init__(self, name, ks, cin, cout, activation=None, stride=1, cin2=0, mask_activation='leaky_relu'):
        self.name, self.ks, self.cin, self.cin2, self.cout = name, ks, cin, cin2, cout
        self.activation, self.stride = activation, stride
        self.mask_activation = mask_activation

    def specs(self):
        return [(self.name + '/kernel', (self.ks, self.ks, self.cin + self.cin2, self.cout)),
# ... 42 lines not shown
    def forward_s2d(self, store, xs, bf16_copy=False, copy_lrelu=False):
        w3 = ops.s2d_conv_weights(store.p[self.name + '/kernel'])
        fused = self.activation in FUSED_ACTIVATIONS
        y = ops.conv2d(xs, w3, store.p[self.name + '/bias'], act=self.activation if fused else None, bf16_copy=bf16_copy,
                       copy_lrelu=copy_lrelu)
        return y if fused else act_forward(y, self.activation)

    def backward_params_s2d(self, store, xs, dz):
        with ops.side_stream(xs, dz, key=store.g[self.name + '/kernel'].data_ptr()):
            dw3 = ops.conv2d_wgrad(xs, dz, 3, db=store.g[self.name + '/bias'])
            ops.s2d_conv_weights_bwd(dw3, store.g[self.name + '/kernel'])

    def backward_input(self, store, dz, in_hw, act_mask=None, out=None, out2=None, out_bf16=False, residual=None,
                       bf16_copy=False, s2d_out=False, mask_s2d=False, mask_activation=None):
        kind = mask_activation or self.mask_activation
        if act_mask is not None and kind not in FUSED_ACTIVATIONS:
            if out2 is not None or mask_s2d:
                raise NotImplementedError('split / space-to-depth-stored masks with activation {}'.format(kind))
            d = self.backward_input(store, dz, in_hw, out=out)
            ops.activation_bwd(d, act_mask, kind, out=d)
            if residual is not None:
                ops.add(residual, d, out=d)
            if s2d_out:
                d = ops.d2s_clip_bwd(d, 1.0)
            return (d, None) if bf16_copy else d
        if self.stride == 2:
            d = ops.conv2d_dgrad_strided2(dz, store.p[self.name + '/kernel'], in_hw, act_mask=act_mask, out_bf16=out_bf16,
                                          mask_s2d=mask_s2d)
            d = d if residual is None else ops.add(residual, d, out=d)
            return (d, None) if bf16_copy else d
        return ops.conv2d_dgrad(dz, store.p[self.name + '/kernel'], in_hw, stride=self.stride, act_mask=act_mask,
                                out=out, out2=out2, out_bf16=out_bf16, residual=residual, bf16_copy=bf16_copy,
                                s2d_out=s2d_out)


class Conv5x5Stride2Image(Conv2D):

    def s2d_ok(self, x):
        return ops.s2d_conv_ok(self.ks, self.stride, x.shape[1], x.shape[2], self.cin) and self.cin2 == 0 and 4 * self.cin <= 16

    def forward_image(self, store, x, a, b, s2d_out=False):
        if not self.s2d_ok(x):
            if s2d_out:
                raise RuntimeError('s2d_out needs the space-to-depth form of the layer')
            x0 = ops.affine(x, a, b)
            return self.forward(store, x0), x0
        xs = ops.s2d2_affine(x, a, b, cp=16)
        w3 = ops.s2d_conv_weights(store.p[self.name + '/kernel'], cp=16)
        fused = self.activation in FUSED_ACTIVATIONS
        y = ops.conv2d(xs, w3, store.p[self.name + '/bias'], act=self.activation if fused else None, s2d_out=s2d_out,
                       out_bf16=s2d_out)
        return (y if fused else act_forward(y, self.activation)), xs

    def backward_params_image(self, store, ctx, dz):
        if ctx.dtype != torch.bfloat16:
            return self.backward_params(store, ctx, dz)
        with ops.side_stream(ctx, dz, key=store.g[self.name + '/kernel'].data_ptr()):
            dw3 = ops.conv2d_wgrad(ctx, dz, 3, db=store.g[self.name + '/bias'])
            ops.s2d_conv_weights_bwd(dw3, store.g[self.name + '/kernel'])

    def backward_input_image(self, store, dz, in_hw, a):
        return ops.conv2d_dgrad_strided2(dz, store.p[self.name + '/kernel'], in_hw, scale=a)


class Conv2DTranspose2x2(object):

    def __init__(self, name, cin, cout):
        self.name, self.cin, self.cout = name, cin, cout

    def specs(self):
        return [(self.name + '/kernel', (2, 2, self.cout, self.cin)), (self.name + '/bias', (self.cout,))]

    def init(self, store, gen):
        from .tfmodel import glorot_uniform_
        k = torch.empty((2, 2, self.cout, self.cin), dtype=torch.float32)
        glorot_uniform_(k, self.cin * 4, self.cout * 4, gen)
        store.p[self.name + '/kernel'].copy_(k)
        store.p[self.name + '/bias'].zero_()

    def forward(self, store, x, out_bf16=False):
        return ops.convt2x2(x, store.p[self.name + '/kernel'], store.p[self.name + '/bias'], out_bf16=out_bf16)

    def backward_params(self, store, x, dy):
        ops.convt2x2_wgrad(x, dy, dw=store.g[self.name + '/kernel'], side=True)
        ops.bias_grad(dy, db=store.g[self.name + '/bias'], side=True)

    def backward_input(self, store, dy, act_mask=None, out_bf16=False, mask_activation='leaky_relu'):
        if act_mask is not None and mask_activation not in FUSED_ACTIVATIONS:
            d = ops.convt2x2_dgrad(dy, store.p[self.name + '/kernel'])
            return ops.activation_bwd(d, act_mask, mask_activation, out=d)
        return ops.convt2x2_dgrad(dy, store.p[self.name + '/kernel'], act_mask=act_mask, out_bf16=out_bf16)


class ConstrainedConv2D(object):

    def __init__(self, name='constrained', filter_strength=100.0):
        self.name, self.strength = name, float(filter_strength)

    def specs(self):
        return [(self.name + '/kernel', (5, 5, 3, 3))]

    def init(self, store, gen=None):
        store.p[self.name + '/kernel'].copy_(torch.from_numpy(hk.residual_init_filter().astype(np.float32)))

    def forward(self, store, x, c4_only=False):
        nf = ops.constrained_kernel(store.p[self.name + '/kernel'], self.strength)
        y, c4 = ops.cconv3(x, nf, pad_mode=1, want_f32=not c4_only, want_c4=c4_only)
        return (c4 if c4_only else y), nf

    def backward_params(self, store, x, dy):
        with ops.side_stream(x, dy, key=store.g[self.name + '/kernel'].data_ptr()):
            dnf = ops.conv2d_wgrad(x, dy, 5, pads=(2, 2), pad_mode=1)
            ops.constrained_kernel_bwd(store.p[self.name + '/kernel'], dnf, store.g[self.name + '/kernel'], self.strength)

    def backward_input(self, nf, dy):
        n, h, w, _ = dy.shape
        if h < 4 or w < 4:
            dpad = ops.conv2d(dy, ops.flip_weights(nf), None, pads=(4, 4), out_hw=(h + 4, w + 4))
            return ops.fold_pad(dpad, 2, 1)
        return ops.cconv3_dgrad(dy, nf)
```

neural-imaging_amd/models/tfmodel.py:

```python
import json
import os
from collections import OrderedDict
from pathlib import Path

import numpy as np
import torch

from ..device import DeviceArray, default_device
from ..helpers import utils
from .. import ops


class ParamStore(object):

    def __init__(self, specs, device):
        self.specs = OrderedDict(specs)
        self.device = device
        align = 64
        sizes = [int(np.prod(s)) if len(s) else 1 for s in self.specs.values()]
        total = int(sum(-(-n // align) * align for n in sizes))
        self.flat = torch.zeros(total, dtype=torch.float32, device=device)
        self.flat_grad = torch.zeros(total, dtype=torch.float32, device=device)
        self.p, self.g, self.offsets = OrderedDict(), OrderedDict(), OrderedDict()
        off = 0
        for (name, shape), n in zip(self.specs.items(), sizes):
            self.p[name] = self.flat[off:off + n].view(shape)
            self.g[name] = self.flat_grad[off:off + n].view(shape)
            self.offsets[name] = off
            off += -(-n // align) * align
        self.m = self.v = None
        self.step = 0
        self.lr_t_dev = None
        self.images = ops.WeightImages([t for t in self.p.values() if t.dim() == 4 and min(t.shape) > 0], device) \
            if torch.device(device).type == 'cuda' else None

    def grad_range(self, first=None, before=None):
        lo = 0 if first is None else self.offsets[first]
        hi = self.flat_grad.numel() if before is None else self.offsets[before]
        return self.flat_grad[lo:hi]

    def refresh_images(self):
        if self.images is not None:
            self.images.refresh()

    def ensure_adam(self):
        if self.m is None:
            self.m = torch.zeros_like(self.flat)
            self.v = torch.zeros_like(self.flat)

    def adam(self, lr, step=None, grad_scale=1.0, skip_flag=None, lr_t_dev=None):
        self.ensure_adam()
        ops.join_side_stream()
        self.grads_pending = False
        if step is None:
            self.step += 1
            step = self.step
        ops.adam_step(self.flat, self.flat_grad, self.m, self.v, lr, step, grad_scale=grad_scale, skip_flag=skip_flag,
                      lr_t_dev=lr_t_dev if lr_t_dev is not None else self.lr_t_dev)


def glorot_uniform_(t, fan_in, fan_out, gen):
    limit = float(np.sqrt(6.0 / (fan_in + fan_out)))
    vals = (torch.rand(t.shape, generator=gen, dtype=torch.float64) * 2 - 1) * limit
    t.copy_(vals.to(torch.float32))


class TFModel(object):

    def __init__(self, device=None, **kwargs):
        self.device = torch.device(device) if device is not None else default_device()
        self._model = None
        self.reset_performance_stats()

    @staticmethod
    def _reset_performance(metrics):
        return {k: {'training': [], 'validation': []} for k in metrics}

    def reset_performance_stats(self):
        self.performance = self._reset_performance(['loss'])

    def log_metric(self, metric, scope, value, raw=False):
        if not raw:
            if isinstance(value, DeviceArray):
                value = float(np.mean(value.numpy()))
            elif utils.is_number(value):
                value = float(value)
            else:
                value = float(np.mean([float(v) for v in value]))
        self.performance[metric][scope].append(value)

    def pop_metric(self, metric, scope):
        return self.performance[metric][scope][-1]

    @property
    def parameters(self):
        return [] if self._model is None else list(self._model.p.values())

    @property
    def variables(self):
        return self.parameters

    @property
    def parameter_names(self):
        return [] if self._model is None else list(self._model.p.keys())

    def count_parameters(self):
        return int(sum(int(p.numel()) for p in self.parameters))

    def count_parameters_breakdown(self):
        import pandas as pd
        total = max(self.count_parameters(), 1)
        rows = [(k, tuple(v.shape), int(v.numel()), round(100 * int(v.numel()) / total, 1)) for k, v in self._model.p.items()]
        return pd.DataFrame(rows, columns=['name', 'shape', 'parameters', 'total'])

    def state_dict(self):
        return OrderedDict((k, v.detach().cpu().numpy()) for k, v in self._model.p.items())

    def load_state_dict(self, state):
        for k, v in self._model.p.items():
            if k not in state:
                raise KeyError('missing parameter {} in checkpoint'.format(k))
            a = np.asarray(state[k], np.float32)
            if tuple(a.shape) != tuple(v.shape):
                raise ValueError('shape mismatch for {}: {} vs {}'.format(k, a.shape, tuple(v.shape)))
            v.copy_(torch.from_numpy(a))

    _h5_skip = ()

    def keras_layers(self):
        layers = []
        for k, v in self.state_dict().items():
            if k in self._h5_skip:
                continue
            prefix, _, leaf = k.rpartition('/')
            lname = (prefix or leaf).replace('/', '_')
            if not layers or layers[-1][0] != lname:
                layers.append((lname, []))
            layers[-1][1].append(('{}/{}:0'.format(lname, leaf), v))
        return layers

    def load_keras_weights(self, filename):
# ... 108 lines not shown
```

neural-imaging_amd/ops.py:

```python
import math
import os

import numpy as np
import torch

from . import _lib

LRELU_ALPHA = 0.2

COMPUTE = 'f32'


STORE_BF16 = True


def set_compute(mode):
    global COMPUTE
    if mode not in ('f32', 'bf16'):
        raise ValueError('compute mode must be f32 or bf16')
    COMPUTE = mode


_WB_REGISTRY = {}


class WeightImages(object):

    def __init__(self, weights, device):
        lib = _lib.load()
        self.entries, sizes = [], []
        for w in weights:
            kh, kw, cin, cout = w.shape
            for mode in (0, 1):
                sizes.append(int(lib.nimg_conv_weights_bf16_bytes(kh, kw, cin, cout, mode)))
                self.entries.append((w, mode))
        offs = np.concatenate([[0], np.cumsum([-(-s // 256) * 256 for s in sizes])]).astype(np.int64)
        self.buf = torch.empty(int(offs[-1]) or 256, dtype=torch.uint8, device=device)
        table = np.zeros((len(self.entries), 4), np.int64)
        for i, (w, mode) in enumerate(self.entries):
            kh, kw, cin, cout = w.shape
            view = self.buf[int(offs[i]):int(offs[i]) + sizes[i]]
            table[i] = (w.data_ptr(), view.data_ptr(), ((kh * kw) << 32) | mode, (cin << 32) | cout)
            if _WB_REGISTRY.get(w.data_ptr(), {}).get('shape') != tuple(w.shape):
                _WB_REGISTRY[w.data_ptr()] = {'shape': tuple(w.shape)}
            _WB_REGISTRY[w.data_ptr()][mode] = view
        self.table = torch.from_numpy(table).to(device)
        import weakref
        keys = [(w.data_ptr(), tuple(w.shape)) for w in weights]
        weakref.finalize(self, WeightImages._forget, keys, self.buf.data_ptr(), self.buf.numel())

    @staticmethod
    def _forget(keys, base, size):
        for ptr, shape in keys:
            reg = _WB_REGISTRY.get(ptr)
            if reg is not None and reg['shape'] == shape and \
                    all(base <= reg[m].data_ptr() < base + size for m in (0, 1) if m in reg):
                del _WB_REGISTRY[ptr]

    def refresh(self):
        if COMPUTE == 'bf16' and len(self.entries):
            _lib.call('nimg_conv_weights_bf16_batch', _p(self.table), len(self.entries), _stream())


def weights_bf16(w, mode):
    reg = _WB_REGISTRY.get(w.data_ptr())
    if reg is not None and reg['shape'] == tuple(w.shape) and mode in reg:
        return reg[mode]
    kh, kw, cin, cout = w.shape
    nbytes = int(_lib.load().nimg_conv_weights_bf16_bytes(kh, kw, cin, cout, mode))
    wb = torch.empty(nbytes, dtype=torch.uint8, device=w.device)
    _lib.call('nimg_conv_weights_bf16', _p(w), _p(wb), kh, kw, cin, cout, mode, _stream())
    return wb


_raw_stream = getattr(torch._C, '_cuda_getCurrentRawStream', None)
_raw_device = getattr(torch._C, '_cuda_getDevice', None)


def _stream():
    if _raw_stream is not None and _raw_device is not None:
        return _raw_stream(_raw_device())
    return torch.cuda.current_stream().cuda_stream


def _p(t):
    return None if t is None else t.data_ptr()


def _chk(*ts):
    for t in ts:
        if t is None:
            continue
        if not (t.is_cuda and t.is_contiguous()):
            raise RuntimeError('nimg ops need contiguous device tensors (got device={}, contiguous={})'.format(
                t.device, t.is_contiguous()))


def _f32(*ts):
    for t in ts:
        if t is not None and t.dtype != torch.float32:
            raise RuntimeError('nimg ops need float32 tensors, got {}'.format(t.dtype))
    _chk(*ts)


D2S_EPILOGUE = os.environ.get('NIMG_NO_D2S_OUT') is None
BF16_IN, BF16_OUT, BF16_MASK, BF16_DZ, D2S_OUT, S2D_OUT, COPY_LRELU, MASK_CONV = 1, 2, 4, 8, 16, 32, 64, 128


def _fb(*ts):
    for t in ts:
        if t is not None and t.dtype not in (torch.float32, torch.bfloat16):
            raise RuntimeError('nimg ops need float32 / bfloat16 tensors, got {}'.format(t.dtype))
    _chk(*ts)


def _is_bf16(t):
    return t is not None and t.dtype == torch.bfloat16


def same_pads(size, k, s):
    out = -(-size // s)
    total = max((out - 1) * s + k - size, 0)
    return out, total // 2


_PIN_LOG = None


def begin_pin_log():
    global _PIN_LOG
    _PIN_LOG = []


def end_pin_log():
    global _PIN_LOG
    log, _PIN_LOG = _PIN_LOG or [], None
    seen, out = set(), []
    for t in log:
        if id(t) not in seen:
            seen.add(id(t))
            out.append(t)
    return out


# ... 553 lines not shown
            return dw
        if _defer_k is not None and CHAIN_REDUCE:
            _flush_chain_here(_defer_k)
        if _defer_k is not None:
            _flush_deferred(_defer_k, on_its_stream=False)
        ws = _ws_current(x.device).get(need, x.device)
        _lib.call('nimg_conv2d_wgrad_bf16_ex', _p(x), c1, _p(x2), c2, _p(dz), cout, _p(dw), _p(db), n, h, wd, ks, stride,
                  pt, pl, pad_mode, ho, wo, 1 if accumulate else 0, _p(ws), ws.numel(), flags, _stream())
        return dw
    if _is_bf16(x) or _is_bf16(dz):
        raise RuntimeError('bf16-stored tensor reached a float32 weight-gradient path')
    need = _lib.load().nimg_conv2d_wgrad_workspace_bytes(c1 + c2, cout, ks, ks, n, ho, wo)
    ws = _ws_current(x.device).get(need, x.device)
    _lib.call('nimg_conv2d_wgrad', _p(x), c1, _p(x2), c2, _p(dz), cout, _p(dw), _p(db), n, h, wd, ks, stride, pt, pl,
              pad_mode, ho, wo, 1 if accumulate else 0, _p(ws), ws.numel(), _stream())
    return dw


def _flush_chain_here(k):
    entry = _CHAIN.pop(k, None)
    if entry is not None:
        _lib.call('nimg_reduce_slabs_batch', entry, 1, _stream())


def _wgrad_carried(k, carrier, device, need, flags, *operands):
    import ctypes
    if carrier == 'defer':
        st = _defer_state(k)
        if st['n'] == st['cap']:
            _flush_deferred(k, on_its_stream=False)
        entry = ctypes.byref(st['buf'], st['n'] * st['nb'])
    else:
        entry = (ctypes.c_char * int(_lib.load().nimg_reduce_entry_bytes()))()
    ws = _SIDE['ws'][k].claim(need, device)
    name, pre = ('nimg_conv2d_wgrad_bf16_chained', (_CHAIN.get(k),)) if carrier == 'chain' else ('nimg_conv2d_wgrad_bf16_deferred', ())
    _lib.call(name, *operands, _p(ws), ws.numel(), flags, *pre, entry, _stream())
    if carrier == 'defer':
        st['n'] += 1
    elif carrier == 'chain':
        _CHAIN[k] = entry
    else:
        _reduce_behind(k, entry, device)


def bias_grad(dz, db=None, accumulate=False, side=False):
    if side and _SIDE['enabled'] and db is not None:
        with _on_side_stream(dz, key=db.data_ptr()):
            return bias_grad(dz, db=db, accumulate=accumulate, side=False)
    _f32(db)
    _fb(dz)
    cout = dz.shape[-1]
    npix = dz.numel() // cout
    if db is None:
        db = torch.empty((cout,), dtype=torch.float32, device=dz.device)
    need = _lib.load().nimg_bias_grad_workspace_bytes(npix, cout)
    ws = _ws_current(dz.device).get(need, dz.device)
    _lib.call('nimg_bias_grad_ex', _p(dz), _p(db), npix, cout, 1 if accumulate else 0, _p(ws), ws.numel(),
              BF16_DZ if _is_bf16(dz) else 0, _stream())
    return db


def convt2x2(x, w, bias, out_bf16=False):
    _f32(w, bias)
    _fb(x)
    n, h, wd, cin = x.shape
    cout = w.shape[2]
    y = torch.empty((n, 2 * h, 2 * wd, cout), dtype=torch.bfloat16 if out_bf16 else torch.float32, device=x.device)
    if COMPUTE == 'bf16' and cin % 8 == 0 and cout >= 8:
        wb = weights_bf16(w, 1)
        _lib.call('nimg_convt2x2_fwd_bf16_ex', _p(x), _p(wb), _p(bias), _p(y), n, h, wd, cin, cout,
                  (BF16_IN if _is_bf16(x) else 0) | (BF16_OUT if out_bf16 else 0), _stream())
        return y
    if _is_bf16(x) or out_bf16:
        raise RuntimeError('bf16-stored tensor reached a float32 transposed-convolution path')
    _lib.call('nimg_convt2x2_fwd', _p(x), _p(w), _p(bias), _p(y), n, h, wd, cin, cout, _stream())
    return y


def convt2x2_dgrad(dy, w, act_mask=None, out_bf16=False):
    n, h2, w2, _ = dy.shape
    return conv2d(dy, w, None, stride=2, pads=(0, 0), out_hw=(h2 // 2, w2 // 2), act_mask=act_mask, out_bf16=out_bf16)


def convt2x2_wgrad(x, dy, dw=None, side=False):
    return conv2d_wgrad(dy, x, 2, stride=2, pads=(0, 0), dw=dw, side=side)


def maxpool2(x):
    _fb(x)
    n, h, w, c = x.shape
    y = torch.empty((n, h // 2, w // 2, c), dtype=x.dtype, device=x.device)
    if _is_bf16(x):
        _lib.call('nimg_maxpool2_fwd_bf16', _p(x), _p(y), n, h, w, c, _stream())
        return y
    _lib.call('nimg_maxpool2_fwd', _p(x), _p(y), n, h, w, c, _stream())
    return y


def maxpool2_bwd(dp, yact, add=None, apply_mask=True, out=None, alpha=None):
    a = LRELU_ALPHA if alpha is None else float(alpha)
    _fb(dp, yact, add, out)
    n, h, w, c = yact.shape
    dz = torch.empty_like(yact) if out is None else out
    if _is_bf16(yact):
        if any(t is not None and not _is_bf16(t) for t in (dp, add, dz)):
            raise RuntimeError('maxpool2_bwd on a bf16-stored activation needs bf16-stored gradients')
        _lib.call('nimg_maxpool2_bwd_bf16', _p(dp), _p(yact), _p(add), _p(dz), n, h, w, c, 1 if apply_mask else 0,
                  a, _stream())
        return dz
    _f32(dp, add, dz)
    _lib.call('nimg_maxpool2_bwd', _p(dp), _p(yact), _p(add), _p(dz), n, h, w, c, 1 if apply_mask else 0,
              a, _stream())
    return dz


def conv2d_pool(x, w, bias=None, act='leaky_relu', want_idx=True, out_bf16=False):
    _f32(w, bias)
    _fb(x)
    n, h, wd, cin = x.shape
    ks, cout = w.shape[0], w.shape[3]
    if w.shape[2] != cin or (h & 1) or (wd & 1) or (cout & 3) or ks not in (3, 5):
        raise ValueError('conv2d_pool: unsupported shape')
    bf16_path = COMPUTE == 'bf16' and (cin in (3, 4) or cin % 8 == 0)
    if (out_bf16 or _is_bf16(x)) and not bf16_path:
        raise RuntimeError('bf16 storage needs the throughput-mode convolution path')
    pooled = torch.empty((n, h // 2, wd // 2, cout), dtype=torch.bfloat16 if out_bf16 else torch.float32, device=x.device)
    idx = torch.empty((n, h // 2, wd // 2, cout), dtype=torch.uint8, device=x.device) if want_idx else None
    a = 1 if act == 'leaky_relu' else 0
    if bf16_path:
        wb = None if cin in (3, 4) else weights_bf16(w, 0)
        flags = (BF16_IN if _is_bf16(x) else 0) | (BF16_OUT if out_bf16 else 0)
        _lib.call('nimg_conv2d_pool_fwd_bf16_ex', _p(x), cin, _p(w), _p(wb), _p(bias), _p(pooled), _p(idx), cout, n, h, wd,
                  ks, a, LRELU_ALPHA, flags, _stream())
    else:
        _lib.call('nimg_conv2d_pool_fwd', _p(x), cin, _p(w), _p(bias), _p(pooled), _p(idx), cout, n, h, wd, ks, a,
                  LRELU_ALPHA, _stream())
    return pooled, idx


POOL_ALSO = _os.environ.get('NIMG_NO_POOL_ALSO') is None


_EPI8 = {}


def _epi8_built(entry):
    if entry not in _EPI8:
        lib = _lib.load()
        if entry == 'nimg_conv2d_fwd_pool_also_bf16':
            rc = lib.nimg_conv2d_fwd_pool_also_bf16(None, 8, None, None, None, None, None, 8, 0, 16, 16, 1, LRELU_ALPHA, None)
        else:
            rc = lib.nimg_conv2d_dgrad_unpool_out_bf16(None, 8, None, None, None, None, 8, 0, 16, 16, 1, LRELU_ALPHA, None)
        _EPI8[entry] = rc == 0
    return _EPI8[entry]


def conv2d_and_pool_ok(x, w):
    n, h, wd, cin = x.shape
    return POOL_ALSO and _epi8_built('nimg_conv2d_fwd_pool_also_bf16') and COMPUTE == 'bf16' and _is_bf16(x) and w.shape[0] == 3 and w.shape[1] == 3 and cin % 8 == 0 and \
        w.shape[3] % 8 == 0 and h % 2 == 0 and wd % 2 == 0 and h > 8 and wd > 8


def conv2d_and_pool(x, w, bias=None, act='leaky_relu'):
    _f32(w, bias)
    if not conv2d_and_pool_ok(x, w):
        raise ValueError('conv2d_and_pool: unsupported shape / mode')
    n, h, wd, cin = x.shape
    cout = w.shape[3]
# ... 309 lines not shown
        if labels.dtype != torch.int32:
            raise RuntimeError('labels must be int32')
        loss_per = torch.empty((n,), dtype=torch.float32, device=gap.device)
        dlogits = torch.empty((n, k), dtype=torch.float32, device=gap.device)
    _lib.call('nimg_fan_dense_fwd', _p(gap), _p(w), _p(b), _p(labels), _p(probs), _p(loss_per), _p(dlogits), n, c, k,
              float(loss_scale), _stream())
    return probs, loss_per, dlogits


def fan_dense_bwd(gap, dlogits, loss_per, loss_scale, dw, db):
    _f32(gap, dlogits, loss_per, dw, db)
    n, c = gap.shape
    loss = torch.empty((1,), dtype=torch.float32, device=gap.device)
    _lib.call('nimg_fan_dense_bwd', _p(gap), _p(dlogits), _p(loss_per), _p(dw), _p(db), _p(loss), n, c, dlogits.shape[1],
              float(loss_scale), _stream())
    return loss


def head_dgrad(mask, dlogits, wdense, w, in_mask, shape, alpha=None):
    _chk(mask, dlogits, wdense, w, in_mask)
    n, h, wd, c = shape
    dx = torch.empty((n, h, wd, c), dtype=torch.bfloat16, device=mask.device)
    if in_mask is not None and (not _is_bf16(in_mask) or tuple(in_mask.shape) != tuple(shape)):
        raise RuntimeError('head_dgrad: the mask tensor is the bf16-stored input of the 1x1 layer')
    _lib.call('nimg_head_dgrad', _p(mask), _p(dlogits), _p(wdense), dlogits.shape[1], _p(weights_bf16(w, 1)), _p(in_mask), _p(dx),
              n, h * wd, c, LRELU_ALPHA if alpha is None else float(alpha), _stream())
    return dx


def head_dact(mask, dlogits, wdense, shape, alpha=None):
    _chk(mask, dlogits, wdense)
    n, h, wd, c = shape
    dact = torch.empty((n, h, wd, c), dtype=torch.bfloat16, device=mask.device)
    _lib.call('nimg_head_dact', _p(mask), _p(dlogits), _p(wdense), dlogits.shape[1], _p(dact), n, h * wd, c,
              LRELU_ALPHA if alpha is None else float(alpha), _stream())
    return dact


def adam_lr_t(lr, step, beta1=0.9, beta2=0.999):
    lr, beta1, beta2 = (float(np.float32(v)) for v in (lr, beta1, beta2))
    return lr * math.sqrt(1.0 - math.pow(beta2, float(int(step)))) / (1.0 - math.pow(beta1, float(int(step))))


def adam_step(params, grads, m, v, lr, step, beta1=0.9, beta2=0.999, eps=1e-7, grad_scale=1.0, skip_flag=None,
              lr_t_dev=None):
    join_side_stream()
    _f32(params, grads, m, v, lr_t_dev)
    if lr_t_dev is not None:
        _lib.call('nimg_adam_step_dev', _p(params), _p(grads), _p(m), _p(v), params.numel(), _p(lr_t_dev), float(beta1),
                  float(beta2), float(eps), float(grad_scale), _p(skip_flag), _stream())
        return
    _lib.call('nimg_adam_step', _p(params), _p(grads), _p(m), _p(v), params.numel(), float(lr), float(beta1),
              float(beta2), float(eps), int(step), float(grad_scale), _p(skip_flag), _stream())


def int_fill(t, value=0):
    _chk(t)
    if t.dtype != torch.int32 or not t.is_contiguous():
        raise ValueError('int_fill: contiguous int32 tensor expected')
    _lib.call('nimg_int_words', _p(t), None, t.numel(), int(value), 0, _stream())
    return t


def int_max_(dst, src):
    _chk(dst, src)
    if dst.dtype != torch.int32 or src.dtype != torch.int32 or dst.numel() != src.numel():
        raise ValueError('int_max_: two int32 tensors of one size expected')
    _lib.call('nimg_int_words', _p(dst), _p(src), dst.numel(), 0, 1, _stream())
    return dst


def float_fill(t, value):
    _f32(t)
    _lib.call('nimg_float_fill', _p(t), t.numel(), float(value), _stream())
    return t


def nan_flag(g, flag):
    join_side_stream()
    _f32(g)
    _lib.call('nimg_nan_flag', _p(g), g.numel(), _p(flag), _stream())


def constrained_kernel(kernel, strength=100.0):
    _f32(kernel)
    nf = torch.empty_like(kernel)
    _lib.call('nimg_constrained_kernel_fwd', _p(kernel), _p(nf), kernel.shape[0], kernel.shape[2], float(strength),
              _stream())
    return nf


def constrained_kernel_bwd(kernel, dnf, dk, strength=100.0):
    _f32(kernel, dnf, dk)
    _lib.call('nimg_constrained_kernel_bwd', _p(kernel), _p(dnf), _p(dk), kernel.shape[0], kernel.shape[2],
              float(strength), _stream())
    return dk


def cconv3(x, w, pad_mode=1, out=None, want_f32=True, want_c4=False):
    _f32(x, w, out)
    n, h, wd, c = x.shape
    if c != 3 or tuple(w.shape) != (5, 5, 3, 3):
        raise ValueError('cconv3: (N,H,W,3) input and a (5,5,3,3) kernel expected')
    y = (torch.empty_like(x) if out is None else out) if want_f32 else None
    c4 = torch.empty((n, h, wd, 4), dtype=torch.bfloat16, device=x.device) if want_c4 else None
    _lib.call('nimg_cconv3', _p(x), _p(w), _p(y), _p(c4), n, h, wd, int(pad_mode), _stream())
    return y, c4


FRONT_END = _os.environ.get('NIMG_OLD_FRONTEND') is None
CCONV_DGRAD_MFMA = _os.environ.get('NIMG_NO_CCONV_DGRAD_MFMA') is None
S2D_CONV = _os.environ.get('NIMG_NO_S2D_CONV') is None
SPARSE_DGRAD = _os.environ.get('NIMG_SPARSE_DGRAD') is not None


def front_end_ok(cin, cout, ks, h, w, n=None):
    small = n is None or n * h * w * 16 < (1 << 31) - 65536
    return FRONT_END and COMPUTE == 'bf16' and cin == 3 and cout == 32 and ks == 5 and h % 2 == 0 and w % 2 == 0 and \
        h >= 4 and w >= 4 and small


def conv1_pool_c4(c4, w, bias, act='leaky_relu', want_idx=True, out_bf16=True):
    _f32(w, bias)
    _chk(c4)
    n, h, wd, c = c4.shape
    if c4.dtype != torch.bfloat16 or c != 4 or tuple(w.shape) != (5, 5, 3, 32) or (h & 1) or (wd & 1):
        raise ValueError('conv1_pool_c4: (N,H,W,4) bf16 pixels, a (5,5,3,32) kernel and even sizes expected')
    pooled = torch.empty((n, h // 2, wd // 2, 32), dtype=torch.bfloat16 if out_bf16 else torch.float32, device=c4.device)
    idx = torch.empty((n, h // 2, wd // 2, 8), dtype=torch.uint8, device=c4.device) if want_idx else None
    _lib.call('nimg_conv1_pool_fwd_c4', _p(c4), _p(w), _p(bias), _p(pooled), _p(idx), n, h, wd,
              LRELU_ALPHA if act == 'leaky_relu' else 1.0, 1 if out_bf16 else 0, _stream())
    return pooled, idx


def conv1_wgrad_c4(c4, g, idx, dw=None, db=None, accumulate=False, side=False):
    if side and _SIDE['enabled'] and dw is not None:
        with _on_side_stream(c4, g, idx, key=dw.data_ptr()):
            return conv1_wgrad_c4(c4, g, idx, dw=dw, db=db, accumulate=accumulate, side=False)
    _f32(dw, db)
    _fb(g)
    _chk(c4, idx)
    n, h, wd, _ = c4.shape
    if c4.dtype != torch.bfloat16 or tuple(g.shape) != (n, h // 2, wd // 2, 32) or tuple(idx.shape) != (n, h // 2, wd // 2, 8) or \
            idx.dtype != torch.uint8:
        raise ValueError('conv1_wgrad_c4: (N,H,W,4) bf16 pixels, a (N,H/2,W/2,32) gradient and (N,H/2,W/2,8) arg-max codes expected')
    if dw is None:
        dw = torch.empty((5, 5, 3, 32), dtype=torch.float32, device=c4.device)
    need = _lib.load().nimg_conv1_wgrad_c4_workspace_bytes()
    ws = _ws_current(c4.device).get(need, c4.device)
    _lib.call('nimg_conv1_wgrad_c4', _p(c4), _p(g), _p(idx), _p(dw), _p(db), n, h, wd, 1 if _is_bf16(g) else 0,
              1 if accumulate else 0, _p(ws), ws.numel(), _stream())
    return dw


def conv1_dgrad_pooled(g, idx, w, out=None):
    _f32(w, out)
    _fb(g)
    _chk(idx)
    n, hp, wp, c = g.shape
    if c != 32 or tuple(w.shape) != (5, 5, 3, 32) or tuple(idx.shape) != (n, hp, wp, 8) or idx.dtype != torch.uint8:
        raise ValueError('conv1_dgrad_pooled: a (N,H/2,W/2,32) gradient, (N,H/2,W/2,8) arg-max codes and a (5,5,3,32) kernel expected')
    if out is None:
        out = torch.empty((n, 2 * hp, 2 * wp, 3), dtype=torch.float32, device=g.device)
    _lib.call('nimg_conv1_dgrad_pooled', _p(g), _p(idx), _p(w), _p(out), n, 2 * hp, 2 * wp, 1 if _is_bf16(g) else 0, _stream())
    return out


def cconv3_dgrad(dy, nf):
    _f32(dy, nf)
    n, h, wd, _ = dy.shape
    if COMPUTE == 'bf16' and wd % 64 == 0 and CCONV_DGRAD_MFMA:
        dx = torch.empty_like(dy)
        _lib.call('nimg_conv5c3_bf16', _p(dy), _p(flip_weights(nf)), _p(dx), n, h, wd, _stream())
    else:
        dx, _ = cconv3(dy, flip_weights(nf), pad_mode=0)
    _lib.call('nimg_cconv3_dgrad_border', _p(dy), _p(nf), _p(dx), n, h, wd, _stream())
    return dx


def fold_pad(dpad, pad, pad_mode):
    _f32(dpad)
    n, hp, wp, c = dpad.shape
    dx = torch.empty((n, hp - 2 * pad, wp - 2 * pad, c), dtype=torch.float32, device=dpad.device)
    _lib.call('nimg_fold_pad', _p(dpad), _p(dx), n, hp - 2 * pad, wp - 2 * pad, c, pad, pad_mode, _stream())
    return dx


def gaussian_fwd(x, gk25, out=None, clip=True, want_mask=True):
    _f32(x, gk25, out)
    n, h, w, _ = x.shape
    y = torch.empty_like(x) if out is None else out
    mask = torch.empty((n, h, w), dtype=torch.uint8, device=x.device) if want_mask else None
    _lib.call('nimg_gaussian_fwd', _p(x), _p(y), _p(mask), _p(gk25), n, h, w, 1 if clip else 0, _stream())
    return y, mask


def gaussian_bwd(dy, mask, gk25):
    _f32(dy, gk25)
    n, h, w, _ = dy.shape
    dx = torch.empty_like(dy)
    _lib.call('nimg_gaussian_bwd', _p(dy), _p(mask), _p(dx), _p(gk25), n, h, w, _stream())
    return dx


def dwfilter_fwd(x, taps, k, pad_mode, out=None, clip=True, want_mask=True):
    _f32(x, taps, out)
    n, h, w, _ = x.shape
    if taps.numel() != k * k:
        raise ValueError('taps: k*k floats')
    y = torch.empty_like(x) if out is None else out
    mask = torch.empty((n, h, w), dtype=torch.uint8, device=x.device) if want_mask else None
    _lib.call('nimg_dwfilter_fwd', _p(x), _p(y), _p(mask), _p(taps), int(k), PAD_MODES[pad_mode], n, h, w,
              1 if clip else 0, _stream())
    return y, mask


def dwfilter_bwd(dy, mask, taps, k, pad_mode):
    _f32(dy, taps)
    n, h, w, _ = dy.shape
    dx = torch.empty_like(dy)
    _lib.call('nimg_dwfilter_bwd', _p(dy), _p(mask), _p(dx), _p(taps), int(k), PAD_MODES[pad_mode], n, h, w, _stream())
    return dx


def sharpen_fwd(x, gk9, out=None, want_aux=True):
    _f32(x, gk9, out)
    n, h, w, _ = x.shape
    y = torch.empty_like(x) if out is None else out
    aux = torch.empty_like(x) if want_aux else None
    mask = torch.empty((n, h, w), dtype=torch.uint8, device=x.device) if want_aux else None
    _lib.call('nimg_sharpen_fwd', _p(x), _p(y), _p(aux), _p(mask), _p(gk9), n, h, w, _stream())
    return y, aux, mask


def sharpen_bwd(x, dy, aux, mask, gk9):
    _f32(x, dy, aux, gk9)
    n, h, w, _ = x.shape
    dx = torch.empty_like(x)
    _lib.call('nimg_sharpen_bwd', _p(x), _p(dy), _p(aux), _p(mask), _p(dx), _p(gk9), n, h, w, _stream())
    return dx


class AxisOperator(object):

    def __init__(self, dense, device):
        dense = np.asarray(dense, np.float64)
        self.out_size, self.in_size = dense.shape
        self.fwd = self._csr(dense, device)
        self.bwd = self._csr(dense.T, device)

    @staticmethod
    def _csr(m, device):
        rowptr, col, val = [0], [], []
        for r in range(m.shape[0]):
            nz = np.nonzero(m[r])[0]
            col.extend(nz.tolist())
            val.extend(m[r, nz].tolist())
            rowptr.append(len(col))
# ... 594 lines not shown
```

neural-imaging_amd/workflows/manipulation_classification.py:

```python
from collections import OrderedDict

import os

import numpy as np
import torch

from .. import ops, parallel
from ..device import DeviceArray, to_device
from ..helpers import tf_helpers
from ..models import forensics, jpeg, pipelines


class ManipulationClassification(object):

    def __init__(self, nip_model, manipulations=None, distribution=None, fan_args=None, trainable=None,
                 raw_patch_size=128, loss_metric='L2', device=None, nan_check='eager', pipeline_fan_update=None):
        if raw_patch_size < 16 or raw_patch_size > 512:
            raise ValueError('The patch size ({}) looks incorrect, typical values should be >= 16 and <= 512'.format(
                raw_patch_size))
        self._trainable = set() if trainable is None else set(trainable)
        self._trainable.add('fan')
        if distribution is None:
            self._distribution = {'downsampling': 'pool:2', 'compression': 'jpeg',
                                  'compression_params': {'quality': 50, 'codec': 'soft'}}
# ... 142 lines not shown
        from ..helpers import kernels as hk
        key = (size, factor, str(device))
        cache = self.__dict__.setdefault('_bilinear_cache', {})
        if key not in cache:
            cache[key] = ops.AxisOperator(hk.bilinear_axis_matrix(size, size // factor), device)
        return cache[key]

    def _downsampling_bwd(self, dc):
        mode = self._distribution['downsampling']
        if mode.startswith('pool'):
            return ops.avgpool_bwd(dc, self.downsampling_factor)
        if mode == 'bilinear':
            op = self._bilinear_operator(dc.shape[1] * self.downsampling_factor, self.downsampling_factor, dc.device)
            tmp = ops.sparse_axis_apply(dc, op.bwd, 0, op.in_size)
            return ops.sparse_axis_apply(tmp, op.bwd, 1, op.in_size)
        return dc

    def run_workflow(self, batch_x, augment=False, training=False):
        self.finish_pending()
        x = to_device(batch_x, self.device)
        Y = self.nip.forward(x)[0]
        m, _ = self._manipulations(Y, augment)
        c = self._downsampling(m)
        C, ent, _ = self._codec_forward(c)
        entropy = np.nan if ent is None else DeviceArray(ent)
        probs = self.fan.forward(C)[0]
        return DeviceArray(Y), DeviceArray(c), DeviceArray(C), entropy, DeviceArray(probs)

    def run_workflow_to_decisions(self, batch_x):
        return self.run_workflow(batch_x)[-1].numpy().argmax(axis=1)

    def run_manipulations(self, batch_y, randomize=False, override=None):
        return DeviceArray(self._manipulations(to_device(batch_y, self.device), randomize, override)[0])

    def manipulations_timing(self, batch_y):
        from datetime import datetime
        Y = to_device(batch_y, self.device)
        times = {}
        for name, op in self._operations.items():
            torch.cuda.synchronize(self.device)
            d1 = datetime.now()
            op.forward(Y, self._strengths[name])
            torch.cuda.synchronize(self.device)
            times[name] = (datetime.now() - d1).total_seconds()
        return times

    def run_downsampling(self, batch_y):
        return DeviceArray(self._downsampling(to_device(batch_y, self.device)))

    def run_compression(self, batch_y, return_entropy=False):
        y = to_device(batch_y, self.device)
        C, ent, _ = self._codec_forward(y)
        return (DeviceArray(C), np.nan if ent is None else DeviceArray(ent)) if return_entropy else DeviceArray(C)

    def run_rgb_to_fan(self, batch_Y):
        m = self._manipulations(to_device(batch_Y, self.device))[0]
        c = self._downsampling(m)
        return self._codec_forward(c)[0].cpu().numpy()

    def run_rgb_to_probabilities(self, batch_Y):
        self.finish_pending()
        C = torch.from_numpy(self.run_rgb_to_fan(batch_Y)).to(self.device)
        return self.fan.forward(C)[0].cpu().numpy()

    def _codec_forward(self, c, training=False):
        if self.codec is None:
            return c, None, None
        if self._is_dcn:
            return self.codec.forward(c, training=training)
        C, ctx = self.codec.forward(c, training=training)
        return C, None, ctx

    def training_step(self, batch_x, batch_y, lambda_nip=0, lambda_dcn=0, augment=False, learning_rate=1e-4):
        x = to_device(batch_x, self.device)
        target = to_device(batch_y, self.device)
        b = x.shape[0]
        train_nip = 'nip' in self._trainable and self.nip.count_parameters() > 0
        train_dcn = 'dcn' in self._trainable
        need_upstream = train_nip or train_dcn
        world = parallel.world_size()

        self._launch_pending_fan()

        m = None
        if getattr(self.nip, 'writes_into', False):
            b = x.shape[0]
            m = torch.empty((self.n_classes * b, 2 * x.shape[1], 2 * x.shape[2], 3), dtype=torch.float32, device=x.device)
            Y, nctx = self.nip.forward(x, training=train_nip, out=m[:b])
        else:
            Y, nctx = self.nip.forward(x, training=train_nip)
        m, mctxs = self._manipulations(Y, augment, training=train_nip, m=m)
        c = self._downsampling(m)
        C, entropy, cctx = self._codec_forward(c, training=need_upstream)
        self._finish_pending_fan()
        _, fctx = self.fan.forward(C, self._device_labels(b), training=True)

        ops.int_fill(self._nan_flag, 0)
        late_fan = forensics.LATE_PARAMS and need_upstream and not parallel.is_distributed() and \
            C.shape[0] >= forensics.LATE_MIN_IMAGES
        pipelined = self._pipeline_fan and need_upstream and not parallel.is_distributed() and self._nan_check == 'deferred' and \
            self._lr_t_dev is None
        deferred = [] if pipelined else None
        if pipelined:
            late_fan = True
        loss_ce, dC = self.fan.backward(fctx, need_input_grad=need_upstream, join=not late_fan, defer=deferred)
        if not late_fan:
            ops.nan_flag(self.fan._model.flat_grad, self._nan_flag)
            self._bucket.launch(self.fan._model.flat_grad)
        loss_dcn = None
        dc = None
        if need_upstream:
            if self.codec is None:
                dc = dC
            elif self._is_dcn:
                lam = float(lambda_dcn) * world if train_dcn else 0.0
                dc_direct = None
                if train_dcn:
                    l2, _ = ops.l2_loss(c, C, grad_scale=lam, grad_out=dC, accumulate=True)
                    if train_nip:
                        dc_direct = torch.empty_like(c)
                        ops.l2_loss(C, c, grad_scale=lam, grad_out=dc_direct, accumulate=False)
                    loss_dcn = (l2, entropy)
                dc = self.codec.backward(cctx, dC, entropy_coef=lam * self.codec._h.entropy_weight,
                                         need_input_grad=train_nip)
                if train_nip and dc_direct is not None:
                    ops.add(dc, dc_direct, out=dc)
                if train_dcn:
                    ops.nan_flag(self.codec._model.flat_grad, self._nan_flag)
                    self._bucket.launch(self.codec._model.flat_grad)
            else:
                dc_direct = None
                if train_dcn:
                    lam = float(lambda_dcn) / (255.0 * 255.0)
                    mse, _ = ops.mse255(C, c, grad_scale=lam, grad_out=dC, accumulate=True)
                    if train_nip:
                        dc_direct = torch.empty_like(c)
                        ops.mse255(c, C, grad_scale=lam, grad_out=dc_direct, accumulate=False)
                    loss_dcn = (mse, None)
                dc = self.codec.backward(cctx, dC)
                if dc_direct is not None:
                    ops.add(dc, dc_direct, out=dc)
                if train_dcn:
                    ops.nan_flag(self.codec._model.flat_grad, self._nan_flag)
                    self._bucket.launch(self.codec._model.flat_grad)
        if train_nip:
            dm = self._downsampling_bwd(dc)
            parts_dY = [dm[:b]] + [op.backward(mctxs[k], dm[(k + 1) * b:(k + 2) * b])
                                   for k, (name, op) in enumerate(self._operations.items())]
            dY = dm[:b]
            head = self.nip.head_gradient(parts_dY, Y, target, float(lambda_nip)) if hasattr(self.nip, 'head_gradient') else None
            nip_kw = {}
            if head is not None:
                loss_nip, nip_kw['dz_head'] = head
            else:
                for i in range(0, len(parts_dY) - 1, 5):
                    chunk = ([dY] if i else [parts_dY[0]]) + parts_dY[i + 1:i + 6]
                    ops.add_n(chunk, out=dY)
                loss_nip, _ = self.nip.loss_and_grad(Y, target, grad_scale=float(lambda_nip), grad_out=dY, accumulate=True)
            if parallel.is_distributed() and hasattr(self.nip, 'decoder_grads'):
                dec, enc = self.nip.decoder_grads()
                def decoder_done():
                    ops.nan_flag(dec, self._nan_flag)
                    self._bucket.launch(dec)
                self.nip.backward(nctx, dY, on_decoder_done=decoder_done, **nip_kw)
                ops.nan_flag(enc, self._nan_flag)
                self._bucket.launch(enc)
            else:
                self.nip.backward(nctx, dY, **nip_kw)
                ops.nan_flag(self.nip._model.flat_grad, self._nan_flag)
                self._bucket.launch(self.nip._model.flat_grad)
        else:
            loss_nip, _ = self.nip._loss_fn(Y, target)
        if late_fan and not pipelined:
            ops.nan_flag(self.fan._model.flat_grad, self._nan_flag)
            self._bucket.launch(self.fan._model.flat_grad)
        parallel.all_reduce_flag(self._nan_flag)
        ops.int_max_(self._nan_seen, self._nan_flag)
        if self._nan_check == 'eager' and int(self._nan_flag.item()) != 0:
            self._nan_seen.zero_()
            self._bucket.wait()
            raise RuntimeError('gradient NaNs in the workflow step')
        self._bucket.wait()

        self._step += 1
        gscale = 1.0 / world
        rate = self._lr_t_dev
        if pipelined:
            self._pending_fan = (deferred, learning_rate, self._step, gscale)
        else:
            self.fan._model.adam(learning_rate, self._step, gscale, skip_flag=self._nan_flag, lr_t_dev=rate)
        if train_nip:
            self.nip._model.adam(learning_rate, self._step, gscale, skip_flag=self._nan_flag, lr_t_dev=rate)
        if train_dcn:
            self.codec._model.adam(learning_rate, self._step, gscale, skip_flag=self._nan_flag, lr_t_dev=rate)

        dcn_value = np.nan
        if loss_dcn is not None and loss_dcn[1] is None:
            dcn_value = _LazySum(torch.zeros_like(loss_dcn[0]), loss_dcn[0], 1.0 / (255.0 * 255.0))
        elif loss_dcn is not None:
            dcn_value = _LazySum(loss_dcn[0], loss_dcn[1], self.codec._h.entropy_weight)
        loss = _LazyLoss(loss_ce, loss_nip, float(lambda_nip) if 'nip' in self._trainable else 0.0,
                         dcn_value if loss_dcn is not None else None, float(lambda_dcn))
        return loss, {'ce': DeviceArray(loss_ce), 'nip': DeviceArray(loss_nip), 'dcn': dcn_value}

    def _launch_pending_fan(self):
        if self._pending_fan is not None and self._pending_fan[0] is not None:
            with ops.one_fork():
                for fn in self._pending_fan[0]:
                    fn()
            self._pending_fan = (None,) + self._pending_fan[1:]

    def _finish_pending_fan(self):
        if self._pending_fan is None:
            return
        self._launch_pending_fan()
        _, lr, step, gscale = self._pending_fan
        self._pending_fan = None
        ops.nan_flag(self.fan._model.flat_grad, self._nan_flag)
        ops.int_max_(self._nan_seen, self._nan_flag)
        self.fan._model.adam(lr, step, gscale, skip_flag=self._nan_flag)

    def finish_pending(self):
        self._finish_pending_fan()

    def check_nan(self):
        self.finish_pending()
        """Deferred NaN guard (nan_check='deferred'): raises if any step since the last check produced NaN grads (those
        steps' Adam updates were skipped on the device)."""
        seen = int(self._nan_seen.item())
        self._nan_seen.zero_()
        if seen != 0:
            raise RuntimeError('gradient NaNs in the workflow step')

    def summary_compact(self):
        return '{class_name}[{trainables}]: {nip} -> [{manips}] {pool}{codec}-> {fan}'.format(
            class_name=type(self).__name__, nip=self.nip.class_name,
            manips=''.join([x[0] for x in self._forensics_classes]),
            trainables=''.join([x[0] for x in self.trainable_models]),
            pool='' if self._distribution['downsampling'] == 'none' else '-> {} '.format(
                self._distribution['downsampling']),
            codec='' if self.codec is None else '-> {} '.format(self.codec.summary_compact()), fan='FAN')

    def summary(self):
        return '{class_name}[opt={trainables}]: {input} -> {nip} -> {n_ops} manipulations [{manips}] {pool}{codec}-> {fan}'.format(
            class_name=type(self).__name__, input='(rgb)' if self.nip.x.shape[-1] == 3 else '(raw)',
            nip=self.nip.class_name, n_ops=self.n_classes - 1,
            manips=''.join([x[0] for x in self._forensics_classes]),
            trainables=''.join([x[0] for x in self.trainable_models]),
            pool='' if self._distribution['downsampling'] == 'none' else '-> {} '.format(
                self._distribution['downsampling']),
            codec='' if self.codec is None else '-> {} '.format(self.codec.summary_compact()),
            fan='FAN -> (prob. {} classes)'.format(self.n_classes))

    def details(self):
        out = [self.summary()]
        out.append('Input         : {} {}'.format(self.nip.x.shape, '(rgb)' if self.nip.x.shape[-1] == 3 else '(raw)'))
        out.append('Camera ISP    : {}'.format(self.nip.summary()))
        out.append('Manipulations : {} -> {}'.format(self.n_classes, self._forensics_classes))
        out.append('Downsampling  : {}'.format(self._distribution['downsampling']))
        out.append('Codec         : {}'.format('' if self.codec is None else self.codec.summary()))
        out.append('Forensics     : {}'.format(self.fan.summary()))
        out.append('Output        : {}'.format(self.fan.y.shape))
        return '\n'.join(out)

    def is_trainable(self, model):
        return model in self._trainable

    @property
    def trainable_models(self):
        return tuple(x for x in self._trainable)


class _JpegManipulation(object):

    def __init__(self, codec):
        self.codec = codec

# ... 36 lines not shown
```

Baseline: 8242 patches/s.

## Batch Adam and NaN checks into table kernels and fuse convT wgrad bias

Replaces the per-model NaN-flag and Adam launches with single table-driven kernels that walk several parameter ranges in one launch. Folds the constrained-kernel normalisation and its flipped copy into the batched weight-conversion kernel and caches the flip. Adds a transposed-conv 2x2 weight-gradient path that computes the bias gradient as input sums inside the wgrad kernel. Weight images are refreshed once per step for all models. The aim is fewer small kernel launches and fewer separate reduction passes, at the cost of pointer-table caching keyed on data_ptr, which could go stale if buffers are reallocated.

```diff
diff --git a/include/nimg.h b/include/nimg.h
--- a/include/nimg.h
+++ b/include/nimg.h
@@ -25,7 +25,7 @@
 #define NIMG_D2S_CONVT 1024
 #define NIMG_POOL_ALSO 256
 
-#define NIMG_ABI_VERSION 7
+#define NIMG_ABI_VERSION 8
 int nimg_abi_version(void);
 
 #define NIMG_ROUND_ROUND 0
@@ -109,6 +109,9 @@
 int nimg_adam_step_dev(float* params, const float* grads, float* m, float* v, long count, const float* lr_t, float beta1,
                        float beta2, float eps, float grad_scale, const int* skip_flag, void* stream);
 int nimg_nan_flag(const float* g, long count, int* flag, void* stream);
+int nimg_adam_step_table(const void* table, int n_ranges, long max_count, float lr, float beta1, float beta2, float eps,
+                         int step, float grad_scale, const int* skip_flag, const float* lr_t, void* stream);
+int nimg_nan_flag_table(const void* table, int n_ranges, long max_count, int* flag, int* seen, void* stream);
 int nimg_int_words(int* dst, const int* src, long n, int value, int mode, void* stream);
 int nimg_float_fill(float* dst, long n, float value, void* stream);
 
@@ -287,6 +290,10 @@
                            int cout, void* stream);
 int nimg_convt2x2_fwd_bf16_ex(const float* x, const void* wb, const float* bias, float* y, int n, int h, int wd, int cin,
                               int cout, int flags, void* stream);
+size_t nimg_conv2d_wgrad_bf16_isum_workspace_bytes(int cin, int cout, int ks_h, int ks_w, int n, int hout, int wout);
+int nimg_convt2x2_wgrad_bias_bf16(const void* dy, int c_dy, const void* x, int c_x, float* dw, float* db, int n, int ho, int wo,
+                                  int accumulate, void* workspace, size_t workspace_bytes, int flags, void* stream);
+#define NIMG_CONSTRAINED_FLIP_OFFSET 256
 int nimg_conv_weights_bf16_batch(const void* table, int n_entries, void* stream);
 int nimg_conv2d_fwd_bf16(const float* in1, int c1, const float* in2, int c2, const void* wb, const float* bias,
                          float* out1, int o1, float* out2, int o2, const float* act_mask, int n, int h, int wd,
diff --git a/neural-imaging_amd/_lib.py b/neural-imaging_amd/_lib.py
--- a/neural-imaging_amd/_lib.py
+++ b/neural-imaging_amd/_lib.py
@@ -57,6 +57,8 @@
     'nimg_reduce_slabs_batch': (c_int, [P, c_int, P]),
     'nimg_conv3_rows_c4_bf16': (c_int, [P, P, P, P, c_int, c_int, c_int, c_int, c_float, P]),
     'nimg_nan_flag': (c_int, [P, c_long, P, P]),
+    'nimg_adam_step_table': (c_int, [P, c_int, c_long, c_float, c_float, c_float, c_float, c_int, c_float, P, P, P]),
+    'nimg_nan_flag_table': (c_int, [P, c_int, c_long, P, P, P]),
     'nimg_int_words': (c_int, [P, P, c_long, c_int, c_int, P]),
     'nimg_float_fill': (c_int, [P, c_long, c_float, P]),
     'nimg_bind_tickets': (c_int, [P, P, c_size_t]),
@@ -159,6 +161,8 @@
     'nimg_conv2d_dgrad_fewin_pooled_bf16_ex': (c_int, [P, P, P, P, c_int, c_int, c_int, c_int, c_int, c_int, c_int, P]),
     'nimg_maxpool2_unpool_ex': (c_int, [P, P, P, P, c_int, c_int, c_int, c_int, c_int, c_float, c_int, P]),
     'nimg_conv_weights_bf16_batch': (c_int, [P, c_int, P]),
+    'nimg_conv2d_wgrad_bf16_isum_workspace_bytes': (c_size_t, [c_int, c_int, c_int, c_int, c_int, c_int, c_int]),
+    'nimg_convt2x2_wgrad_bias_bf16': (c_int, [P, c_int, P, c_int, P, P, c_int, c_int, c_int, c_int, P, c_size_t, c_int, P]),
     'nimg_convt2x2_fwd_bf16': (c_int, [P, P, P, P, c_int, c_int, c_int, c_int, c_int, P]),
     'nimg_convt2x2_fwd_bf16_ex': (c_int, [P, P, P, P, c_int, c_int, c_int, c_int, c_int, c_int, P]),
     'nimg_conv2d_fwd_smallc_bf16': (c_int, [P, c_int, P, P, P, c_int, c_int, c_int, c_int, c_int, c_int, c_int,
@@ -190,7 +194,7 @@
 _lib = None
 
 
-ABI_VERSION = 7
+ABI_VERSION = 8
 TICKET_BYTES = 64 * 1024
 
 
diff --git a/neural-imaging_amd/csrc/common.h b/neural-imaging_amd/csrc/common.h
--- a/neural-imaging_amd/csrc/common.h
+++ b/neural-imaging_amd/csrc/common.h
@@ -430,6 +430,30 @@
 
 static inline int cdiv(long a, long b) { return (int)((a + b - 1) / b); }
 
+__device__ __forceinline__ bool constrained_centre(int e, int ks, int c) {
+    const int co = e % c, ci = (e / c) % c, kw = (e / (c * c)) % ks, kh = e / (c * c * ks);
+    return kh == ks / 2 && kw == ks / 2 && ci == co;
+}
+__device__ __forceinline__ void constrained_normalise(const float* __restrict__ k, float* __restrict__ nf,
+                                                      float* __restrict__ flip, int ks, int c, float strength, float* df) {
+    const int total = ks * ks * c * c, tid = threadIdx.x;
+    if (tid < c) {
+        float s = 0.f;
+        for (int e = tid; e < total; e += c)
+            if (!constrained_centre(e, ks, c)) s += k[e];
+        df[tid] = s;
+    }
+    __syncthreads();
+    for (int e = tid; e < total; e += blockDim.x) {
+        const float v = constrained_centre(e, ks, c) ? -strength : strength * k[e] / df[e % c];
+        nf[e] = v;
+        if (flip) {
+            const int co = e % c, ci = (e / c) % c, t = e / (c * c);
+            flip[((ks * ks - 1 - t) * c + co) * c + ci] = v;
+        }
+    }
+}
+
 }
 
 extern "C" unsigned* nimg_internal_tickets(hipStream_t stream, size_t words);
diff --git a/neural-imaging_amd/csrc/constrained.hip b/neural-imaging_amd/csrc/constrained.hip
--- a/neural-imaging_amd/csrc/constrained.hip
+++ b/neural-imaging_amd/csrc/constrained.hip
@@ -10,18 +10,7 @@
 __global__ __launch_bounds__(256) void constrained_fwd_kernel(const float* __restrict__ k, float* __restrict__ nf,
                                                               int ks, int c, float strength) {
     __shared__ float df[16];
-    const int total = ks * ks * c * c, tid = threadIdx.x;
-    if (tid < c) {
-        float s = 0.f;
-        for (int e = tid; e < total; e += c)
-            if (!centre_mask(e, ks, c)) s += k[e];
-        df[tid] = s;
-    }
-    __syncthreads();
-    for (int e = tid; e < total; e += blockDim.x) {
-        const bool m = centre_mask(e, ks, c);
-        nf[e] = m ? -strength : strength * k[e] / df[e % c];
-    }
+    nimg::constrained_normalise(k, nf, nullptr, ks, c, strength, df);
 }
 
 __global__ __launch_bounds__(256) void constrained_bwd_kernel(const float* __restrict__ k,
diff --git a/neural-imaging_amd/csrc/conv_bf16.hip b/neural-imaging_amd/csrc/conv_bf16.hip
--- a/neural-imaging_amd/csrc/conv_bf16.hip
+++ b/neural-imaging_amd/csrc/conv_bf16.hip
@@ -21,6 +21,16 @@
     const float* w = reinterpret_cast<const float*>(e[0]);
     __bf16* wb = reinterpret_cast<__bf16*>(e[1]);
     const int taps = (int)(e[2] >> 32), mode = (int)(e[2] & 0xffffffffll);
+    if (mode == 2) {
+        __shared__ float df[16];
+        if (blockIdx.x != 0 || (int)(e[3] & 0xffffffffll) > 16) return;
+        int ks = 1;
+        while (ks * ks < taps) ++ks;
+        float* nf = reinterpret_cast<float*>(e[1]);
+        nimg::constrained_normalise(w, nf, nf + NIMG_CONSTRAINED_FLIP_OFFSET, ks, (int)(e[3] & 0xffffffffll),
+                                    __uint_as_float((unsigned)(e[3] >> 32)), df);
+        return;
+    }
     const int cin = (int)(e[3] >> 32), cout = (int)(e[3] & 0xffffffffll);
     const int rows = mode == 0 ? cout : cin, cols = mode == 0 ? cin : cout;
     const int chunks = (cols + 15) / 16, rblocks = (rows + 63) / 64;
diff --git a/neural-imaging_amd/csrc/conv_bf16_wgrad.h b/neural-imaging_amd/csrc/conv_bf16_wgrad.h
--- a/neural-imaging_amd/csrc/conv_bf16_wgrad.h
+++ b/neural-imaging_amd/csrc/conv_bf16_wgrad.h
@@ -8,6 +8,7 @@
     const unsigned char* dz_idx;
     float* partial;
     float* db_partial;
+    float* isum_partial;
     int C1, C2, Cout;
     int N, H, W, Hout, Wout, pad_t, pad_l;
     int tiles_y, tiles_x, splits, work_per_split, pad_mode;
diff --git a/neural-imaging_amd/csrc/conv_bf16_wgrad.hip b/neural-imaging_amd/csrc/conv_bf16_wgrad.hip
--- a/neural-imaging_amd/csrc/conv_bf16_wgrad.hip
+++ b/neural-imaging_amd/csrc/conv_bf16_wgrad.hip
@@ -15,7 +15,7 @@
 
 constexpr int B_ZS = 192;
 
-template <int KS, int STRIDE, int NW, bool INB, bool DZB, int TH, bool UNP = false, int NCO = 2, bool PAIR = false>
+template <int KS, int STRIDE, int NW, bool INB, bool DZB, int TH, bool UNP = false, int NCO = 2, bool PAIR = false, bool ISUM = false>
 __global__ __launch_bounds__(NW * 64, 2) void conv_wgrad_bf16_kernel(const WgradParamsB p) {
     nimg::reduce_entry_inline(p.pre);
     constexpr int TCO = 32 * NCO, ZS = NCO == 2 ? B_ZS : 64, ZI = 4 * NCO;
@@ -27,6 +27,7 @@
     constexpr int THH = (TH - 1) * STRIDE + KS, TWH = PAIR ? 20 : (B_TW - 1) * STRIDE + KS;
     constexpr int NPIXH = THH * TWH, NPIX = TH * B_TW;
     static_assert(STRIDE == 1 || STRIDE == 2, "stride");
+    static_assert(!ISUM || (KS == 2 && STRIDE == 2 && !PAIR && !UNP && NW * 64 * 8 * 4 <= NPIXH * 64), "input sums: disjoint tiles");
     extern __shared__ __attribute__((aligned(16))) unsigned char smem_raw[];
     unsigned char* sI = smem_raw;
     unsigned char* sZ = smem_raw + NPIXH * 64;
@@ -54,6 +55,8 @@
     const int w_end = min(work_total, w_begin + p.work_per_split);
     const bool do_bias = p.db_partial && ci0 == 0;
     float bacc[8] = {0.f, 0.f, 0.f, 0.f, 0.f, 0.f, 0.f, 0.f};
+    const bool do_isum = ISUM && p.isum_partial && co0 == 0;
+    float iacc[8] = {0.f, 0.f, 0.f, 0.f, 0.f, 0.f, 0.f, 0.f};
     const int a_lane = ((half * (PAIR ? 10 : 8) + (g >> 2)) * STRIDE) * 64 + (sub * 16 + (g & 3) * 4) * 2;
     const int z_lane = (half * 8 + (g >> 2)) * ZS + (sub * 16 + (g & 3) * 4) * 2;
     constexpr int IP = (NPIXH * 4 + NTHR - 1) / NTHR, ZP = (NPIX * ZI) / NTHR;
@@ -125,9 +128,22 @@
                 uint4 packed;
                 if constexpr (INB) {
                     packed = *reinterpret_cast<const uint4*>(&preI[q][0]);
+                    if constexpr (ISUM) {
+                        if (do_isum) {
+                            const bf16x8 b = *reinterpret_cast<const bf16x8*>(&preI[q][0]);
+#pragma unroll
+                            for (int e = 0; e < 8; ++e) iacc[e] += (float)b[e];
+                        }
+                    }
                 } else {
                     const float f[8] = {preI[q][0].x, preI[q][0].y, preI[q][0].z, preI[q][0].w,
                                         preI[q][1].x, preI[q][1].y, preI[q][1].z, preI[q][1].w};
+                    if constexpr (ISUM) {
+                        if (do_isum) {
+#pragma unroll
+                            for (int e = 0; e < 8; ++e) iacc[e] += f[e];
+                        }
+                    }
                     const bf16x8 b = pack8(f);
                     packed = *reinterpret_cast<const uint4*>(&b);
                 }
@@ -192,6 +208,20 @@
             float sum = 0.f;
             for (int o = 0; o < NTHR / ZI; ++o) sum += red[(o * ZI + (tid >> 3)) * 8 + (tid & 7)];
             p.db_partial[(long)split * p.Cout + co0 + tid] = sum;
+        }
+    }
+    if constexpr (ISUM) {
+        if (do_isum) {
+            __syncthreads();
+            float* red = reinterpret_cast<float*>(smem_raw);
+#pragma unroll
+            for (int e = 0; e < 8; ++e) red[tid * 8 + e] = iacc[e];
+            __syncthreads();
+            if (tid < B_CI && ci0 + tid < Cin) {
+                float sum = 0.f;
+                for (int o = 0; o < NTHR / 4; ++o) sum += red[(o * 4 + (tid >> 3)) * 8 + (tid & 7)];
+                p.isum_partial[(long)split * Cin + ci0 + tid] = sum;
+            }
         }
     }
     if constexpr (KS == 1) {
@@ -297,8 +327,12 @@
 static int wgrad_bf16_impl(const float* in1, int c1, const float* in2, int c2, const float* dz,
                            const unsigned char* dz_idx, int cout, float* dw, float* db, int n, int h, int wd, int ks,
                            int stride, int pad_t, int pad_l, int pad_mode, int hout, int wout, int accumulate,
-                           void* workspace, size_t workspace_bytes, int flags, void* stream, const ReducePlan& plan) {
+                           void* workspace, size_t workspace_bytes, int flags, void* stream, const ReducePlan& plan,
+                           float* isum = nullptr) {
     OwedReduction owed{plan.pre, (hipStream_t)stream};
+    if (isum && (ks != 2 || stride != 2 || pad_t || pad_l || pad_mode || c2 || db || dz_idx || h != 2 * hout || wd != 2 * wout ||
+                 (c1 % 4) || (cout % 4)))
+        return NIMG_ERR_ARG;
     if ((flags & NIMG_BF16_IN) && ((c1 & 7) || (c2 & 7))) return NIMG_ERR_ARG;
     if ((flags & NIMG_BF16_DZ) && (cout & 7)) return NIMG_ERR_ARG;
     if (flags && !dz_idx && c2 == 0 && c1 <= 4) return NIMG_ERR_ARG;
@@ -309,9 +343,11 @@
     if ((c2 > 0 && !in2) || hout <= 0 || wout <= 0 || !workspace || pad_mode < 0 || pad_mode > 2) return NIMG_ERR_ARG;
     const int cin = c1 + c2;
     if (workspace_bytes < nimg_conv2d_wgrad_bf16_workspace_bytes(cin, cout, ks, ks, n, hout, wout)) return NIMG_ERR_WORKSPACE;
+    if (isum && workspace_bytes < nimg_conv2d_wgrad_bf16_isum_workspace_bytes(cin, cout, ks, ks, n, hout, wout)) return NIMG_ERR_WORKSPACE;
     WgradParamsB p;
     p.pre = nimg::empty_reduce_entry();
     p.in1 = in1; p.in2 = in2; p.dz = dz; p.dz_idx = dz_idx; p.partial = (float*)workspace; p.db_partial = nullptr;
+    p.isum_partial = nullptr;
     p.flags = flags;
     p.tickets = nullptr; p.dw = dw; p.db = db; p.group = 1; p.accumulate = accumulate;
     p.C1 = c1; p.C2 = c2; p.Cout = cout; p.N = n; p.H = h; p.W = wd; p.Hout = hout; p.Wout = wout;
@@ -398,8 +434,9 @@
         return NIMG_OK;
     }
     if (db) p.db_partial = p.partial + (size_t)p.splits * count;
+    if (isum) p.isum_partial = p.partial + (size_t)p.splits * count;
     const long blocks = (long)cdiv(cin, B_CI) * cdiv(cout, B_CO) * p.splits;
-    want_tickets(p);
+    if (!isum) want_tickets(p);
     if (owed.e) p.pre = *owed.e;
 #define NIMG_WGB1(KS_, ST_, NW_, INB_, DZB_, TH_)                                                               \
     do {                                                                                                      \
@@ -414,6 +451,9 @@
         if (p.dz_idx) {                                                                                       \
             if constexpr (DZB_ && ST_ == 1 && KS_ == 5) k = conv_wgrad_bf16_kernel<KS_, ST_, NW_, INB_, true, TH_, true>;    \
             else return NIMG_ERR_ARG;                                                                         \
+        }                                                                                                     \
+        if constexpr (KS_ == 2 && ST_ == 2) {                   \
+            if (p.isum_partial) k = conv_wgrad_bf16_kernel<KS_, ST_, NW_, INB_, DZB_, TH_, false, 2, false, true>;  \
         }                                                                                                     \
         (void)hipFuncSetAttribute((const void*)k, hipFuncAttributeMaxDynamicSharedMemorySize, (int)lds);      \
         hipLaunchKernelGGL(k, dim3((unsigned)blocks), dim3(NW_ * 64), lds, s, p);                             \
@@ -443,10 +483,27 @@
     NIMG_CHECK_LAUNCH();
     owed.ran_in_kernel();
     if (p.tickets) return NIMG_OK;
-    finish_reduce2(plan, (const float*)workspace, dw, count, p.splits, db ? (const float*)p.db_partial : nullptr, db, (long)cout,
-                   p.splits, accumulate, s);
+    if (isum)
+        finish_reduce2(plan, (const float*)workspace, dw, count, p.splits, (const float*)p.isum_partial, isum, (long)cin, p.splits,
+                       accumulate, s);
+    else
+        finish_reduce2(plan, (const float*)workspace, dw, count, p.splits, db ? (const float*)p.db_partial : nullptr, db, (long)cout,
+                       p.splits, accumulate, s);
     NIMG_CHECK_LAUNCH();
     return NIMG_OK;
+}
+
+size_t nimg_conv2d_wgrad_bf16_isum_workspace_bytes(int cin, int cout, int ks_h, int ks_w, int n, int hout, int wout) {
+    if (cin <= 0 || cout <= 0 || n <= 0) return 0;
+    const size_t base = nimg_conv2d_wgrad_bf16_workspace_bytes(cin, cout, ks_h, ks_w, n, hout, wout);
+    return base + (size_t)cin * sizeof(float) * splits_for(cin, cout, n, hout, wout);
+}
+
+int nimg_convt2x2_wgrad_bias_bf16(const void* dy, int c_dy, const void* x, int c_x, float* dw, float* db, int n, int ho, int wo,
+                                  int accumulate, void* workspace, size_t workspace_bytes, int flags, void* stream) {
+    if (!db || c_dy < 8) return NIMG_ERR_ARG;
+    return wgrad_bf16_impl((const float*)dy, c_dy, nullptr, 0, (const float*)x, nullptr, c_x, dw, nullptr, n, 2 * ho, 2 * wo, 2, 2, 0,
+                           0, 0, ho, wo, accumulate, workspace, workspace_bytes, flags, stream, ReducePlan{}, db);
 }
 
 int nimg_conv2d_wgrad_bf16(const float* in1, int c1, const float* in2, int c2, const float* dz, int cout, float* dw,
diff --git a/neural-imaging_amd/csrc/pointwise.hip b/neural-imaging_amd/csrc/pointwise.hip
--- a/neural-imaging_amd/csrc/pointwise.hip
+++ b/neural-imaging_amd/csrc/pointwise.hip
@@ -908,6 +908,39 @@
     if (__any(bad) && (threadIdx.x & 63) == 0) atomicOr(flag, 1);
 }
 
+__global__ void adam_table_kernel(const long long* __restrict__ table, float lr_t, float b1, float b2, float eps,
+                                  float gscale, const int* __restrict__ skip_flag, const float* __restrict__ lr_t_dev) {
+    if (skip_flag && skip_flag[0]) return;
+    if (lr_t_dev) lr_t = lr_t_dev[0];
+    const long long* e = table + 5 * blockIdx.y;
+    float* __restrict__ p = reinterpret_cast<float*>(e[0]);
+    const float* __restrict__ g = reinterpret_cast<const float*>(e[1]);
+    float* __restrict__ m = reinterpret_cast<float*>(e[2]);
+    float* __restrict__ v = reinterpret_cast<float*>(e[3]);
+    const long count = (long)e[4];
+    for (long i = (long)blockIdx.x * blockDim.x + threadIdx.x; i < count; i += (long)gridDim.x * blockDim.x) {
+        const float gi = gscale * g[i];
+        const float mi = b1 * m[i] + (1.0f - b1) * gi;
+        const float vi = b2 * v[i] + (1.0f - b2) * gi * gi;
+        m[i] = mi;
+        v[i] = vi;
+        p[i] -= lr_t * mi / (sqrtf(vi) + eps);
+    }
+}
+
+__global__ void nan_flag_table_kernel(const long long* __restrict__ table, int* flag, int* seen) {
+    const long long* e = table + 2 * blockIdx.y;
+    const float* __restrict__ g = reinterpret_cast<const float*>(e[0]);
+    const long count = (long)e[1];
+    bool bad = false;
+    for (long i = (long)blockIdx.x * blockDim.x + threadIdx.x; i < count; i += (long)gridDim.x * blockDim.x)
+        bad |= (g[i] != g[i]);
+    if (__any(bad) && (threadIdx.x & 63) == 0) {
+        atomicOr(flag, 1);
+        if (seen) atomicOr(seen, 1);
+    }
+}
+
 }
 
 extern "C" {
@@ -1259,6 +1292,27 @@
     return NIMG_OK;
 }
 
+int nimg_adam_step_table(const void* table, int n_ranges, long max_count, float lr, float beta1, float beta2, float eps,
+                         int step, float grad_scale, const int* skip_flag, const float* lr_t, void* stream) {
+    if (!table || n_ranges < 0 || n_ranges > 65535 || max_count < 0 || (!lr_t && step < 1)) return NIMG_ERR_ARG;
+    if (n_ranges == 0 || max_count == 0) return NIMG_OK;
+    const double lr_host = lr_t ? 0.0 : (double)lr * __builtin_sqrt(1.0 - __builtin_pow((double)beta2, (double)step)) /
+                                            (1.0 - __builtin_pow((double)beta1, (double)step));
+    hipLaunchKernelGGL(adam_table_kernel, dim3(grid_for(max_count), (unsigned)n_ranges), dim3(256), 0, (hipStream_t)stream,
+                       (const long long*)table, (float)lr_host, beta1, beta2, eps, grad_scale, skip_flag, lr_t);
+    NIMG_CHECK_LAUNCH();
+    return NIMG_OK;
+}
+
+int nimg_nan_flag_table(const void* table, int n_ranges, long max_count, int* flag, int* seen, void* stream) {
+    if (!table || !flag || n_ranges < 0 || n_ranges > 65535 || max_count < 0) return NIMG_ERR_ARG;
+    if (n_ranges == 0 || max_count == 0) return NIMG_OK;
+    hipLaunchKernelGGL(nan_flag_table_kernel, dim3(grid_for(max_count), (unsigned)n_ranges), dim3(256), 0, (hipStream_t)stream,
+                       (const long long*)table, flag, seen);
+    NIMG_CHECK_LAUNCH();
+    return NIMG_OK;
+}
+
 int nimg_int_words(int* dst, const int* src, long n, int value, int mode, void* stream) {
     if (n == 0) return NIMG_OK;
     if (!dst || n < 0 || mode < 0 || mode > 1 || (mode == 1 && !src)) return NIMG_ERR_ARG;
diff --git a/neural-imaging_amd/models/forensics.py b/neural-imaging_amd/models/forensics.py
--- a/neural-imaging_amd/models/forensics.py
+++ b/neural-imaging_amd/models/forensics.py
@@ -75,6 +75,7 @@
         self._model = ParamStore(specs, self.device)
         gen = torch.Generator().manual_seed(seed)
         self._constrained.init(self._model)
+        self._constrained.attach(self._model)
         for c in self._convs:
             c.init(self._model, gen)
         self._conv1x1.init(self._model, gen)
diff --git a/neural-imaging_amd/models/layers.py b/neural-imaging_amd/models/layers.py
--- a/neural-imaging_amd/models/layers.py
+++ b/neural-imaging_amd/models/layers.py
@@ -148,8 +148,7 @@
         return ops.convt2x2(x, store.p[self.name + '/kernel'], store.p[self.name + '/bias'], out_bf16=out_bf16)
 
     def backward_params(self, store, x, dy):
-        ops.convt2x2_wgrad(x, dy, dw=store.g[self.name + '/kernel'], side=True)
-        ops.bias_grad(dy, db=store.g[self.name + '/bias'], side=True)
+        ops.convt2x2_wgrad(x, dy, dw=store.g[self.name + '/kernel'], side=True, db=store.g[self.name + '/bias'])
 
     def backward_input(self, store, dy, act_mask=None, out_bf16=False, mask_activation='leaky_relu'):
         if act_mask is not None and mask_activation not in FUSED_ACTIVATIONS:
@@ -169,8 +168,14 @@
     def init(self, store, gen=None):
         store.p[self.name + '/kernel'].copy_(torch.from_numpy(hk.residual_init_filter().astype(np.float32)))
 
+    def attach(self, store):
+        if store.images is not None:
+            store.images.add_constrained(store.p[self.name + '/kernel'], self.strength)
+
     def forward(self, store, x, c4_only=False):
-        nf = ops.constrained_kernel(store.p[self.name + '/kernel'], self.strength)
+        nf = ops.constrained_kernel_prebuilt(store.p[self.name + '/kernel'], self.strength)
+        if nf is None:
+            nf = ops.constrained_kernel(store.p[self.name + '/kernel'], self.strength)
         y, c4 = ops.cconv3(x, nf, pad_mode=1, want_f32=not c4_only, want_c4=c4_only)
         return (c4 if c4_only else y), nf
 
diff --git a/neural-imaging_amd/models/tfmodel.py b/neural-imaging_amd/models/tfmodel.py
--- a/neural-imaging_amd/models/tfmodel.py
+++ b/neural-imaging_amd/models/tfmodel.py
@@ -57,6 +57,18 @@
             step = self.step
         ops.adam_step(self.flat, self.flat_grad, self.m, self.v, lr, step, grad_scale=grad_scale, skip_flag=skip_flag,
                       lr_t_dev=lr_t_dev if lr_t_dev is not None else self.lr_t_dev)
+
+    @staticmethod
+    def adam_many(stores, lr, step, grad_scale=1.0, skip_flag=None, lr_t_dev=None):
+        if len(stores) < 2 or any(st.lr_t_dev is not None for st in stores):
+            for st in stores:
+                st.adam(lr, step, grad_scale, skip_flag=skip_flag, lr_t_dev=lr_t_dev)
+            return
+        for st in stores:
+            st.ensure_adam()
+            st.grads_pending = False
+        ops.adam_step_table([(st.flat, st.flat_grad, st.m, st.v) for st in stores], lr, step, grad_scale=grad_scale,
+                            skip_flag=skip_flag, lr_t_dev=lr_t_dev)
 
 
 def glorot_uniform_(t, fan_in, fan_out, gen):
diff --git a/neural-imaging_amd/ops.py b/neural-imaging_amd/ops.py
--- a/neural-imaging_amd/ops.py
+++ b/neural-imaging_amd/ops.py
@@ -22,12 +22,16 @@
 
 
 _WB_REGISTRY = {}
+_NF_REGISTRY = {}
+_NF_FLIP = {}
+NF_FLIP_OFFSET = 256
 
 
 class WeightImages(object):
 
     def __init__(self, weights, device):
         lib = _lib.load()
+        self.device = device
         self.entries, sizes = [], []
         for w in weights:
             kh, kw, cin, cout = w.shape
@@ -44,7 +48,10 @@
             if _WB_REGISTRY.get(w.data_ptr(), {}).get('shape') != tuple(w.shape):
                 _WB_REGISTRY[w.data_ptr()] = {'shape': tuple(w.shape)}
             _WB_REGISTRY[w.data_ptr()][mode] = view
+        self._table_host = table
         self.table = torch.from_numpy(table).to(device)
+        self.fresh = False
+        self._nf_bufs = []
         import weakref
         keys = [(w.data_ptr(), tuple(w.shape)) for w in weights]
         weakref.finalize(self, WeightImages._forget, keys, self.buf.data_ptr(), self.buf.numel())
@@ -57,9 +64,75 @@
                     all(base <= reg[m].data_ptr() < base + size for m in (0, 1) if m in reg):
                 del _WB_REGISTRY[ptr]
 
+    @staticmethod
+    def _forget_nf(kptr, nfptr):
+        reg = _NF_REGISTRY.get(kptr)
+        if reg is not None and reg[1].data_ptr() == nfptr:
+            del _NF_REGISTRY[kptr]
+            _NF_FLIP.pop(nfptr, None)
+
+    def add_constrained(self, kernel, strength):
+        ks, _, c, c2 = kernel.shape
+        if c != c2 or c > 16 or ks * ks * c * c > NF_FLIP_OFFSET:
+            raise ValueError('add_constrained: a (ks,ks,c,c) kernel of at most {} elements expected'.format(NF_FLIP_OFFSET))
+        buf = torch.zeros(2 * NF_FLIP_OFFSET, dtype=torch.float32, device=self.device)
+        n = ks * ks * c * c
+        nf, flip = buf[:n].view(ks, ks, c, c), buf[NF_FLIP_OFFSET:NF_FLIP_OFFSET + n].view(ks, ks, c, c)
+        sbits = int(np.float32(strength).view(np.uint32))
+        word3 = (sbits << 32) | c
+        row = np.array([[kernel.data_ptr(), buf.data_ptr(), ((ks * ks) << 32) | 2, word3 - (1 << 64) if word3 >> 63 else word3]], np.int64)
+        self._table_host = np.concatenate([self._table_host, row])
+        self.table = torch.from_numpy(self._table_host).to(self.device)
+        self._nf_bufs.append(buf)
+        _NF_REGISTRY[kernel.data_ptr()] = (float(np.float32(strength)), nf, flip, buf)
+        _NF_FLIP[nf.data_ptr()] = flip
+        import weakref
+        weakref.finalize(self, WeightImages._forget_nf, kernel.data_ptr(), nf.data_ptr())
+
     def refresh(self):
-        if COMPUTE == 'bf16' and len(self.entries):
-            _lib.call('nimg_conv_weights_bf16_batch', _p(self.table), len(self.entries), _stream())
+        if self.fresh:
+            self.fresh = False
+            return
+        if COMPUTE == 'bf16' and len(self._table_host):
+            _lib.call('nimg_conv_weights_bf16_batch', _p(self.table), len(self._table_host), _stream())
+
+    _MERGED = {}
+
+    @staticmethod
+    def refresh_many(images):
+        images = [im for im in images if im is not None and len(im._table_host)]
+        if COMPUTE != 'bf16' or not images:
+            return
+        if len(images) == 1:
+            images[0].fresh = False
+            images[0].refresh()
+            images[0].fresh = True
+            return
+        key = tuple(im.table.data_ptr() for im in images)
+        merged = WeightImages._MERGED.get(key)
+        if merged is None or any(a() is not b for a, b in zip(merged[1], images)):
+            import weakref
+            host = np.concatenate([im._table_host for im in images])
+            merged = (torch.from_numpy(host).to(images[0].device), [weakref.ref(im) for im in images], len(host))
+            if len(WeightImages._MERGED) > 16:
+                WeightImages._MERGED.clear()
+            WeightImages._MERGED[key] = merged
+        _lib.call('nimg_conv_weights_bf16_batch', _p(pin(merged[0])), merged[2], _stream())
+        for im in images:
+            im.fresh = True
+
+    @staticmethod
+    def clear_fresh(images):
+        for im in images:
+            if im is not None:
+                im.fresh = False
+
+
+def constrained_kernel_prebuilt(kernel, strength):
+    reg = _NF_REGISTRY.get(kernel.data_ptr())
+    if COMPUTE != 'bf16' or reg is None or reg[0] != float(np.float32(strength)) or tuple(reg[1].shape) != tuple(kernel.shape):
+        return None
+    return reg[1]
 
 
 def weights_bf16(w, mode):
@@ -779,8 +852,39 @@
     return conv2d(dy, w, None, stride=2, pads=(0, 0), out_hw=(h2 // 2, w2 // 2), act_mask=act_mask, out_bf16=out_bf16)
 
 
-def convt2x2_wgrad(x, dy, dw=None, side=False):
-    return conv2d_wgrad(dy, x, 2, stride=2, pads=(0, 0), dw=dw, side=side)
+def convt2x2_wgrad(x, dy, dw=None, side=False, db=None):
+    cout, cin = dy.shape[3], x.shape[3]
+    fused = db is not None and COMPUTE == 'bf16' and cout % 4 == 0 and cin % 4 == 0 and cout >= 8 and _reduce_carrier() is None and \
+        (not _is_bf16(dy) or cout % 8 == 0) and (not _is_bf16(x) or cin % 8 == 0) and \
+        dy.shape[1] == 2 * x.shape[1] and dy.shape[2] == 2 * x.shape[2]
+    if not fused:
+        dw = conv2d_wgrad(dy, x, 2, stride=2, pads=(0, 0), dw=dw, side=side)
+        if db is not None:
+            bias_grad(dy, db=db, side=side)
+        return dw
+    if side and _SIDE['enabled'] and dw is not None:
+        ctx = _on_side_stream(dy, x, key=dw.data_ptr())
+        with ctx:
+            if CHAIN_REDUCE:
+                _flush_chain_here(ctx.k)
+            _flush_deferred(ctx.k, on_its_stream=False)
+            return _convt2x2_wgrad_bias(x, dy, dw, db)
+    return _convt2x2_wgrad_bias(x, dy, dw, db)
+
+
+def _convt2x2_wgrad_bias(x, dy, dw, db):
+    _f32(dw, db)
+    _fb(x, dy)
+    n, ho, wo, cin = x.shape
+    cout = dy.shape[3]
+    if dw is None:
+        dw = torch.empty((2, 2, cout, cin), dtype=torch.float32, device=x.device)
+    need = _lib.load().nimg_conv2d_wgrad_bf16_isum_workspace_bytes(cout, cin, 2, 2, n, ho, wo)
+    ws = _ws_current(x.device).get(need, x.device)
+    flags = (BF16_IN if _is_bf16(dy) else 0) | (BF16_DZ if _is_bf16(x) else 0)
+    _lib.call('nimg_convt2x2_wgrad_bias_bf16', _p(dy), cout, _p(x), cin, _p(dw), _p(db), n, ho, wo, 0, _p(ws), ws.numel(), flags,
+              _stream())
+    return dw
 
 
 def maxpool2(x):
@@ -1256,6 +1360,47 @@
     _lib.call('nimg_nan_flag', _p(g), g.numel(), _p(flag), _stream())
 
 
+class RangeTables(object):
+    _CACHE = {}
+
+    @staticmethod
+    def get(kind, columns):
+        key = (kind, str(columns[0][0].device)) + tuple(t.data_ptr() for col in columns for t in col) + tuple(col[0].numel() for col in columns)
+        hit = RangeTables._CACHE.get(key)
+        if hit is None:
+            for col in columns:
+                _f32(*col)
+                if any(t.numel() != col[0].numel() for t in col):
+                    raise ValueError('the buffers of one range must have one length')
+            rows = np.array([[t.data_ptr() for t in col] + [col[0].numel()] for col in columns], np.int64)
+            if len(RangeTables._CACHE) > 64:
+                RangeTables._CACHE.clear()
+            hit = RangeTables._CACHE[key] = (torch.from_numpy(rows).to(columns[0][0].device), len(columns),
+                                             max(col[0].numel() for col in columns))
+        pin(hit[0])
+        return hit
+
+
+def nan_flag_table(grads, flag, seen=None):
+    join_side_stream()
+    grads = [g for g in grads if g.numel() > 0]
+    if not grads:
+        return
+    table, n, max_count = RangeTables.get('nan', [(g,) for g in grads])
+    _lib.call('nimg_nan_flag_table', _p(table), n, max_count, _p(flag), _p(seen), _stream())
+
+
+def adam_step_table(stores, lr, step, beta1=0.9, beta2=0.999, eps=1e-7, grad_scale=1.0, skip_flag=None, lr_t_dev=None):
+    join_side_stream()
+    stores = [c for c in stores if c[0].numel() > 0]
+    if not stores:
+        return
+    _f32(lr_t_dev)
+    table, n, max_count = RangeTables.get('adam', [tuple(c) for c in stores])
+    _lib.call('nimg_adam_step_table', _p(table), n, max_count, float(lr), float(beta1), float(beta2), float(eps), int(step),
+              float(grad_scale), _p(skip_flag), _p(lr_t_dev), _stream())
+
+
 def constrained_kernel(kernel, strength=100.0):
     _f32(kernel)
     nf = torch.empty_like(kernel)
@@ -1343,11 +1488,14 @@
 def cconv3_dgrad(dy, nf):
     _f32(dy, nf)
     n, h, wd, _ = dy.shape
+    flip = _NF_FLIP.get(nf.data_ptr())
+    if flip is None:
+        flip = flip_weights(nf)
     if COMPUTE == 'bf16' and wd % 64 == 0 and CCONV_DGRAD_MFMA:
         dx = torch.empty_like(dy)
-        _lib.call('nimg_conv5c3_bf16', _p(dy), _p(flip_weights(nf)), _p(dx), n, h, wd, _stream())
+        _lib.call('nimg_conv5c3_bf16', _p(dy), _p(flip), _p(dx), n, h, wd, _stream())
     else:
-        dx, _ = cconv3(dy, flip_weights(nf), pad_mode=0)
+        dx, _ = cconv3(dy, flip, pad_mode=0)
     _lib.call('nimg_cconv3_dgrad_border', _p(dy), _p(nf), _p(dx), n, h, wd, _stream())
     return dx
 
diff --git a/neural-imaging_amd/workflows/manipulation_classification.py b/neural-imaging_amd/workflows/manipulation_classification.py
--- a/neural-imaging_amd/workflows/manipulation_classification.py
+++ b/neural-imaging_amd/workflows/manipulation_classification.py
@@ -248,18 +248,24 @@
 
         self._launch_pending_fan()
 
-        m = None
-        if getattr(self.nip, 'writes_into', False):
-            b = x.shape[0]
-            m = torch.empty((self.n_classes * b, 2 * x.shape[1], 2 * x.shape[2], 3), dtype=torch.float32, device=x.device)
-            Y, nctx = self.nip.forward(x, training=train_nip, out=m[:b])
-        else:
-            Y, nctx = self.nip.forward(x, training=train_nip)
-        m, mctxs = self._manipulations(Y, augment, training=train_nip, m=m)
-        c = self._downsampling(m)
-        C, entropy, cctx = self._codec_forward(c, training=need_upstream)
-        self._finish_pending_fan()
-        _, fctx = self.fan.forward(C, self._device_labels(b), training=True)
+        images = [getattr(getattr(mdl, '_model', None), 'images', None)
+                  for mdl in (self.nip, self.codec, None if self._pending_fan is not None else self.fan)]
+        ops.WeightImages.refresh_many(images)
+        try:
+            m = None
+            if getattr(self.nip, 'writes_into', False):
+                b = x.shape[0]
+                m = torch.empty((self.n_classes * b, 2 * x.shape[1], 2 * x.shape[2], 3), dtype=torch.float32, device=x.device)
+                Y, nctx = self.nip.forward(x, training=train_nip, out=m[:b])
+            else:
+                Y, nctx = self.nip.forward(x, training=train_nip)
+            m, mctxs = self._manipulations(Y, augment, training=train_nip, m=m)
+            c = self._downsampling(m)
+            C, entropy, cctx = self._codec_forward(c, training=need_upstream)
+            self._finish_pending_fan()
+            _, fctx = self.fan.forward(C, self._device_labels(b), training=True)
+        finally:
+            ops.WeightImages.clear_fresh(images)
 
         ops.int_fill(self._nan_flag, 0)
         late_fan = forensics.LATE_PARAMS and need_upstream and not parallel.is_distributed() and \
@@ -269,9 +275,17 @@
         deferred = [] if pipelined else None
         if pipelined:
             late_fan = True
+        single = not parallel.is_distributed()
+        checked = []
+
+        def check(g):
+            if single:
+                checked.append(g)
+            else:
+                ops.nan_flag(g, self._nan_flag)
         loss_ce, dC = self.fan.backward(fctx, need_input_grad=need_upstream, join=not late_fan, defer=deferred)
         if not late_fan:
-            ops.nan_flag(self.fan._model.flat_grad, self._nan_flag)
+            check(self.fan._model.flat_grad)
             self._bucket.launch(self.fan._model.flat_grad)
         loss_dcn = None
         dc = None
@@ -292,7 +306,7 @@
                 if train_nip and dc_direct is not None:
                     ops.add(dc, dc_direct, out=dc)
                 if train_dcn:
-                    ops.nan_flag(self.codec._model.flat_grad, self._nan_flag)
+                    check(self.codec._model.flat_grad)
                     self._bucket.launch(self.codec._model.flat_grad)
             else:
                 dc_direct = None
@@ -307,7 +321,7 @@
                 if dc_direct is not None:
                     ops.add(dc, dc_direct, out=dc)
                 if train_dcn:
-                    ops.nan_flag(self.codec._model.flat_grad, self._nan_flag)
+                    check(self.codec._model.flat_grad)
                     self._bucket.launch(self.codec._model.flat_grad)
         if train_nip:
             dm = self._downsampling_bwd(dc)
@@ -333,15 +347,18 @@
                 self._bucket.launch(enc)
             else:
                 self.nip.backward(nctx, dY, **nip_kw)
-                ops.nan_flag(self.nip._model.flat_grad, self._nan_flag)
+                check(self.nip._model.flat_grad)
                 self._bucket.launch(self.nip._model.flat_grad)
         else:
             loss_nip, _ = self.nip._loss_fn(Y, target)
         if late_fan and not pipelined:
-            ops.nan_flag(self.fan._model.flat_grad, self._nan_flag)
+            check(self.fan._model.flat_grad)
             self._bucket.launch(self.fan._model.flat_grad)
-        parallel.all_reduce_flag(self._nan_flag)
-        ops.int_max_(self._nan_seen, self._nan_flag)
+        if single:
+            ops.nan_flag_table(checked, self._nan_flag, seen=self._nan_seen)
+        else:
+            parallel.all_reduce_flag(self._nan_flag)
+            ops.int_max_(self._nan_seen, self._nan_flag)
         if self._nan_check == 'eager' and int(self._nan_flag.item()) != 0:
             self._nan_seen.zero_()
             self._bucket.wait()
@@ -353,12 +370,9 @@
         rate = self._lr_t_dev
         if pipelined:
             self._pending_fan = (deferred, learning_rate, self._step, gscale)
-        else:
-            self.fan._model.adam(learning_rate, self._step, gscale, skip_flag=self._nan_flag, lr_t_dev=rate)
-        if train_nip:
-            self.nip._model.adam(learning_rate, self._step, gscale, skip_flag=self._nan_flag, lr_t_dev=rate)
-        if train_dcn:
-            self.codec._model.adam(learning_rate, self._step, gscale, skip_flag=self._nan_flag, lr_t_dev=rate)
+        stores = ([] if pipelined else [self.fan._model]) + ([self.nip._model] if train_nip else []) + \
+            ([self.codec._model] if train_dcn else [])
+        self.fan._model.adam_many(stores, learning_rate, self._step, gscale, skip_flag=self._nan_flag, lr_t_dev=rate)
 
         dcn_value = np.nan
         if loss_dcn is not None and loss_dcn[1] is None:
```

Measured after the change: 8389 patches/s (median of 4 runs). No clear change (+1.8%).
